# jackroos/VL-BERT

Measured on AMD Instinct MI355X. Metric: samples/sec VL-BERT-base pretrain (seq 64+36 regions) at 1/2/4/8 MI355X, higher is better.
Workload: dtype bf16; 1 GPU; VL-BERT-base 12-layer pretrain step (fwd+bwd+clip+AdamW), 64 text + 36 regions, precomputed 2048-d region features, dropout on; global_batch=256, per_gpu_batch=256, per_gpu_caption_samples=256, per_gpu_text_only_samples=0, module=ResNetVLBERTForPretraining, seq_len=101, parallelism=dp1, hipgraph=False, arch=gfx950:sramecc+:xnack-, cus=256, forced_exchange=False, ranks=1

## Files before the change

include/vlbert_hip.h:

```cpp
#ifndef VLBERT_HIP_H
#define VLBERT_HIP_H

#include <stdint.h>

#ifdef __cplusplus
extern "C" {
#endif

typedef struct ihipStream_t* vlb_stream_t;

const char* vlb_last_error(void);
int vlb_version(void);
int vlb_act_dtype(void);
int vlb_device_info(int device, char* name, int cap);

int vlb_gemm_nt_bf16(const void* A, long lda, const void* B, long ldb, void* C, long ldc, int M, int N, int K,
                     const float* bias, int act, const void* aux, long ldaux, void* pre, long ldpre,
                     const void* res, long ldres, float drop_p, const uint32_t* seed, uint32_t tag,
                     int out_mode, int splitk, vlb_stream_t stream);
int vlb_gemm_nt_bf16_ex(const void* A, long lda, const void* B, long ldb, void* C, long ldc, int M, int N, int K,
                        const float* bias, int act, const void* aux, long ldaux, void* pre, long ldpre,
                        const void* res, long ldres, const float* res_stats, const float* res_gamma, const float* res_beta,
                        int out_f16, float drop_p, const uint32_t* seed, uint32_t tag, int out_mode, int splitk,
                        vlb_stream_t stream);


int vlb_gemm_nt_bf16_splitk(const void* A, long lda, const void* B, long ldb, void* C, long ldc, int M, int N, int K,
                            float* workspace, long workspace_floats, vlb_stream_t stream);
int vlb_gemm_set_option(const char* name, int value);



long vlb_wgrad_workspace_floats(int M, int N, int K);
int vlb_wgrad_nt_bf16(const void* A, long lda, const void* B, long ldb, float* C, long ldc, int M, int N, int K,
                      float* workspace, long workspace_floats, vlb_stream_t stream);

int vlb_wgrad_tn_bf16(const void* A, long lda, const void* B, long ldb, float* C, long ldc, int R, int Mo, int No,
                      float* colsum, float* workspace, long workspace_floats, int accumulate, vlb_stream_t stream);

int vlb_transpose_bf16(const void* in, long ldi, void* out, long ldo, int R, int C, float* colsum, vlb_stream_t stream);
int vlb_transpose_batched_bf16(const int64_t* desc, const int32_t* tile_start, int n, int total_tiles, vlb_stream_t stream);

int vlb_nonfinite_status(int reset);
int vlb_layernorm_fwd(const void* x, long ldx, const float* gamma, const float* beta, void* y, long ldy, float* stats,
                      int rows, int H, float eps, int x_f16, vlb_stream_t stream);
int vlb_layernorm_bwd(const void* dy, long lddy, int dy_f32, const void* x, long ldx, const float* stats,
                      const float* gamma, void* dx, long lddx, void* dx_drop, long lddd, float drop_p,
                      const uint32_t* seed, uint32_t tag, float* dx_acc, long ldacc, float* dgamma, float* dbeta,
                      float* workspace, int rows, int H, int x_f16, vlb_stream_t stream);
long vlb_layernorm_bwd_workspace_floats(int H);
int vlb_layernorm_bwd_deferred(const void* dy, long lddy, int dy_f32, const void* x, long ldx, const float* stats,
                               const float* gamma, void* dx, long lddx, void* dx_drop, long lddd, float drop_p,
                               const uint32_t* seed, uint32_t tag, float* dx_acc, long ldacc, float* dgamma, float* dbeta,
                               float* workspace, int rows, int H, int x_f16, vlb_stream_t stream);
int vlb_layernorm_bwd_slabs(int rows);
int vlb_ln_param_finalize_batch(int n, const float* const* ws, const int* nslab, float* const* dgamma, float* const* dbeta, int H,
                                vlb_stream_t stream);

int vlb_attention_fwd(const void* qkv, const float* mask, void* ctx, float* lse, int B, int S, int H, int nh,
                      float drop_p, const uint32_t* seed, uint32_t tag, vlb_stream_t stream);
int vlb_attention_bwd(const void* qkv, const float* mask, const void* ctx, const float* lse, const void* dctx,
                      void* dqkv, int B, int S, int H, int nh, float drop_p, const uint32_t* seed, uint32_t tag,
                      vlb_stream_t stream);
int vlb_attention_probs(const void* qkv, const float* mask, const float* lse, float* probs, int B, int S, int H, int nh, int n,
                        int ldp, float drop_p, const uint32_t* seed, uint32_t tag, vlb_stream_t stream);

int vlb_seq_layout(const uint8_t* text_mask, const uint8_t* obj_mask, int B, int T, int R, int S, int32_t* code,
                   int32_t* text_len, int32_t* nobj, int32_t* text_rows, int32_t* obj_rows, float* attn_mask,
                   vlb_stream_t stream);
int vlb_obj_prep_fwd(const float* boxes, long ldbox, const float* im_info, long ldinfo, const int64_t* mvrc_ops,
                     const float* mask_emb, void* out, int B, int R, float drop_p, const uint32_t* seed, uint32_t tag,
                     vlb_stream_t stream);
int vlb_zero_padded_rows_bf16(void* x, long ld, const float* boxes, long ldbox, int rows, int H, vlb_stream_t stream);
int vlb_masked_colsum(const void* src, long lds, const int64_t* sel, int rows, int C, float* dst, float drop_p,
                      const uint32_t* seed, uint32_t tag, uint32_t row_elems, uint32_t col_off, vlb_stream_t stream);
int vlb_embed_fwd(const int32_t* code, const int32_t* text_len, const int64_t* text_ids, const int64_t* text_type,
                  const void* word_emb, const void* pos_emb, const void* type_emb, const void* end_emb,
                  const void* text_vis, long tv_sb, long tv_st, const void* obj_vis, long ov_sb, long ov_sr,
                  const void* obj_ling, long ol_sb, long ol_sr, const int64_t* obj_ling_idx, const float* gamma,
                  const float* beta, void* pre, float* stats, void* out, int B, int T, int R, int S, int H, int V,
                  int P, float eps, float drop_p, const uint32_t* seed, uint32_t tag, vlb_stream_t stream);
int vlb_embed_bwd(const void* dy, const void* pre, const float* stats, const float* gamma, const int32_t* code,
                  const int32_t* text_len, const int64_t* text_ids, const int64_t* text_type,
                  const int64_t* obj_ling_idx, float* d_word, float* d_pos, float* d_type, float* d_end,
                  float* d_gamma, float* d_beta, float* d_text_vis, long dtv_sb, long dtv_st, float* d_obj_vis,
                  long dov_sb, long dov_sr, float* d_obj_ling, long dol_sb, long dol_sr, int B, int T, int R, int S,
                  int H, int V, int P, float drop_p, const uint32_t* seed, uint32_t tag, int text_vis_zeroed,
                  vlb_stream_t stream);
int vlb_gather_rows(const void* src, const int32_t* idx, void* out, int n, int H, vlb_stream_t stream);
int vlb_scatter_rows(const void* src, const int32_t* idx, void* out, int n, int H, vlb_stream_t stream);
int vlb_mlm_compact(const int64_t* labels, const int32_t* src_rows, int n, int n_split, int V, int cap, int32_t* sel_pos,
                    int32_t* sel_src, int64_t* labels_c, float* count0, float* count1, int32_t* overflow, vlb_stream_t stream);
int vlb_ce_fwd_bwd_compact(void* logits, long ld, int rows, int V, const int64_t* labels_c, const float* count0, const float* count1,
                           float gscale, float* loss_out0, float* loss_out1, vlb_stream_t stream);
int vlb_head_grad_combine(const void* d_text, const void* d_obj, const int32_t* code, void* dx, int B, int T, int R,
                          int S, int H, vlb_stream_t stream);
int vlb_relu_bwd_cast(const float* g, const void* y, void* out, long n, vlb_stream_t stream);
int vlb_dgelu_mul(const void* dg, const void* u, void* out, long n, vlb_stream_t stream);
int vlb_mul_bf16(const void* a, const void* b, void* out, long n, vlb_stream_t stream);
int vlb_tanh_bwd(const void* dy, const void* y, void* out, long n, vlb_stream_t stream);

int vlb_ce_fwd_bwd(void* logits, long ld, int rows, int V, const int64_t* labels, float* counts, float gscale,
                   float* loss_out, void* logits_copy, long ldcopy, vlb_stream_t stream);
int vlb_soft_ce_fwd_bwd(void* logits, long ld, int rows, int C, const float* target, long ldt, float* tsum,
                        float* counts, float gscale, float* loss_out, void* logits_copy, long ldcopy,
                        vlb_stream_t stream);

int vlb_ce_eval(const void* logits, long ld, int rows, int V, const int64_t* labels, const float* count0, const float* count1,
                float* loss_out0, float* loss_out1, int64_t* acc0, int64_t* acc1, int32_t* pred, vlb_stream_t stream);
int vlb_soft_ce_eval(const void* logits, long ld, int rows, int C, const float* target, long ldt, float* loss_out, int64_t* acc,
                     vlb_stream_t stream);

int vlb_argmax_eval(const float* logits, long ld, int rows, int C, int mode, const void* label, long ldl, int32_t* pred, float* score,
                    float* probs, long ldp, void* sum, int64_t* count, vlb_stream_t stream);
int vlb_binary_cls_eval(const float* logits, long ld, const float* label, long ldl, int rows, int N, int64_t* acc, vlb_stream_t stream);
int vlb_joint_hits(const int32_t* pred_a, const int64_t* label_a, const int32_t* pred_r, const int64_t* label_r, int rows, int64_t* acc,
                   vlb_stream_t stream);

int vlb_bce_logits_fwd_bwd(void* logits, long ld, int rows, int A, const float* label, long ldl, float gscale, float pos_weight,
                           float* loss_out, void* logits_copy, long ldcopy, vlb_stream_t stream);
int vlb_dropout_bf16(const void* x, void* y, long n, float drop_p, const uint32_t* seed, uint32_t tag, vlb_stream_t stream);

int vlb_ground_score_fwd(const void* g, long ldg, int H, const float* w2, const float* b2, float* logits, long ldo, int B, int max_len,
                         int origin_len, float drop_p, const uint32_t* seed, uint32_t tag, vlb_stream_t stream);
int vlb_ground_bce(const float* logits, long ldo, const float* boxes, long sbb, long sbr, const float* label, long ldl, int B, int max_len,
                   float* loss_out, float* dlogit, vlb_stream_t stream);
int vlb_ground_score_bwd(const float* gscale, const float* dlogit, int rows, const void* g, long ldg, const void* dgelu, long ldd, int H,
                         const float* w2, void* du, long lddu, float* dw2, float* db2, float drop_p, const uint32_t* seed, uint32_t tag,
                         vlb_stream_t stream);
int vlb_ground_pick_box(const float* logits, long ldo, int B, int origin_len, const float* boxes, long sbb, long sbr, const float* im_info,
                        long ldi, float* pred_boxes, int64_t* idx, vlb_stream_t stream);

int vlb_scale_f32(float* x, long n, float alpha, vlb_stream_t stream);
int vlb_zero_ranges_f32(float* base, const int64_t* ranges, const int32_t* block_start, int n, int total_blocks, vlb_stream_t stream);
int vlb_copy_ranges_f32(const float* src, float* dst, const int64_t* ranges, const int32_t* block_start, int n, int total_blocks,
                        vlb_stream_t stream);

int vlb_sumsq_f32(const float* g, long n, float* out, vlb_stream_t stream);
int vlb_sumsq_f32_det(const float* g, long n, float* partials, int partials_len, float* out, vlb_stream_t stream);
int vlb_adamw_step(float* p, const float* g, float* m, float* v, void* p_bf16, long n, float* state, float grad_scale,
                   vlb_stream_t stream);
int vlb_sumsq_bf16_det(const void* g_bf16, long n, float* partials, int partials_len, float* out, vlb_stream_t stream);
int vlb_adamw_step_gbf16(float* p, const void* g_bf16, float* m, float* v, void* p_bf16, long n, float* state, float grad_scale,
                         vlb_stream_t stream);
int vlb_sumsq_ranges_det(const void* g, int g_is_bf16, const int64_t* ranges, const int32_t* block_start, int n, int total_blocks, int chunk,
                         float* partials, int partials_len, float* out, vlb_stream_t stream);
int vlb_adamw_step_ranges(float* p, const void* g, int g_is_bf16, float* m, float* v, void* p_bf16_compact, const int64_t* ranges,
                          const int32_t* block_start, int n, int total_blocks, int chunk, float* state, float grad_scale, vlb_stream_t stream);
int vlb_sgd_momentum_step(float* p, const float* g, float* momentum_buf, void* p_bf16, long n, float lr, float momentum,
                          float weight_decay, const float* sumsq, float max_norm, float grad_scale, vlb_stream_t stream);
int vlb_lr_schedule_step(float* state, int kind, float base_lr, float warmup_steps, float t_total, vlb_stream_t stream);

#define VLB_SCALER_FLOATS 9
#define VLB_SCALER_SCALE 0
#define VLB_SCALER_GROWTH_FACTOR 1
#define VLB_SCALER_BACKOFF_FACTOR 2
#define VLB_SCALER_GROWTH_INTERVAL 3
#define VLB_SCALER_UNSKIPPED 4
#define VLB_SCALER_SKIPPED_TOTAL 5
#define VLB_SCALER_SKIPPED_IN_A_ROW 6
#define VLB_SCALER_MIN_SCALE 7
#define VLB_SCALER_MAX_SCALE 8
int vlb_adamw_step_scaled(float* p, const void* g, int g_is_bf16, float* m, float* v, void* p_bf16, long n, float* state, float* scaler,
                          int update_scaler, float grad_scale, vlb_stream_t stream);
int vlb_adamw_step_ranges_scaled(float* p, const void* g, int g_is_bf16, float* m, float* v, void* p_bf16_compact, const int64_t* ranges,
                                 const int32_t* block_start, int n, int total_blocks, int chunk, float* state, float* scaler,
                                 float grad_scale, vlb_stream_t stream);
int vlb_sgd_momentum_step_scaled(float* p, const float* g, float* momentum_buf, void* p_bf16, long n, float lr, float momentum,
                                 float weight_decay, const float* sumsq, float max_norm, float grad_scale, float* scaler, int update_scaler,
                                 vlb_stream_t stream);
int vlb_lr_schedule_step_scaled(float* state, const float* scaler, int kind, float base_lr, float warmup_steps, float t_total,
                                vlb_stream_t stream);
int vlb_ce_fwd_bwd_ds(void* logits, long ld, int rows, int V, const int64_t* labels, float* counts, float gscale, const float* dscale,
                      float* loss_out, void* logits_copy, long ldcopy, vlb_stream_t stream);
int vlb_ce_fwd_bwd_compact_ds(void* logits, long ld, int rows, int V, const int64_t* labels_c, const float* count0, const float* count1,
// ... 98 lines not shown
```

vl-bert_amd/_lib.py:

```python
import ctypes
import os

_HERE = os.path.dirname(os.path.abspath(__file__))
PRECISION = os.environ.get("VLB_PRECISION", "bf16").lower()
if PRECISION in ("fp16", "half", "float16"):
    PRECISION = "f16"
if PRECISION not in ("bf16", "f16"):
    raise ValueError("VLB_PRECISION must be bf16 or f16 (got %r)" % PRECISION)


def _default_path(precision):
    return os.path.join(_HERE, "libvlbert_hip.so" if precision == "bf16" else "libvlbert_hip_f16.so")


LIB_PATH = os.environ.get("VLB_LIB_PATH") or _default_path(PRECISION)

_P, _L, _I, _F, _U = ctypes.c_void_p, ctypes.c_long, ctypes.c_int, ctypes.c_float, ctypes.c_uint32

_SIGS = {
    "vlb_gemm_nt_bf16": "plplpliiipiplplplfpuiis",
    "vlb_transpose_batched_bf16": "ppiis",
    "vlb_gemm_nt_bf16_splitk": "plplpliiipls",
    "vlb_transpose_bf16": "plpliips",
    "vlb_wgrad_nt_bf16": "plplpliiipls",
    "vlb_wgrad_tn_bf16": "plplpliiipplis",
    "vlb_wgrad_tn_group_bf16": "ippppppipppplis",
    "vlb_wgrad_tn_table_launch": "piis",
    "vlb_tn8_set_stamps": "p",
    "vlb_wgrad_tn_table_pack": "i" + "p" * 11 + "ipl",
    "vlb_zero_ranges_f32": "pppiis",
    "vlb_copy_ranges_f32": "ppppiis",
    "vlb_layernorm_fwd": "plppplpiifis",
    "vlb_layernorm_bwd": "pliplppplplfpuplpppiiis",
    "vlb_layernorm_bwd_deferred": "pliplppplplfpuplpppiiis",
    "vlb_ln_param_finalize_batch": "ippppis",
    "vlb_gemm_nt_bf16_ex": "plplpliiipiplplplpppifpuiis",
    "vlb_attention_fwd": "ppppiiiifpus",
    "vlb_attention_bwd": "ppppppiiiifpus",
    "vlb_attention_probs": "ppppiiiiiifpus",
    "vlb_seq_layout": "ppiiiipppppps",
    "vlb_obj_prep_fwd": "plplpppiifpus",
    "vlb_masked_colsum": "plpiipfpuuus",
    "vlb_embed_fwd": "pppp" "pppp" "pll" "pll" "pll" "p" "pp" "ppp" "iiiiiii" "f" "fpu" "s",
    "vlb_embed_bwd": "pppp" "ppppp" "pppppp" "pll" "pll" "pll" "iiiiiii" "fpu" "i" "s",
    "vlb_gather_rows": "pppiis",
    "vlb_scatter_rows": "pppiis",
    "vlb_mlm_compact": "ppiiiipppppps",
    "vlb_ce_fwd_bwd_compact": "pliipppfpps",
    "vlb_head_grad_combine": "ppppiiiiis",
    "vlb_relu_bwd_cast": "pppls",
    "vlb_dgelu_mul": "pppls",
    "vlb_mul_bf16": "pppls",
    "vlb_tanh_bwd": "pppls",
    "vlb_ce_fwd_bwd": "pliippfppls",
    "vlb_soft_ce_fwd_bwd": "pliiplppfppls",
    "vlb_ce_eval": "plii" + "p" * 8 + "s",
    "vlb_soft_ce_eval": "pliiplpps",
    "vlb_argmax_eval": "pliiiplppplpps",
    "vlb_binary_cls_eval": "plpliips",
    "vlb_joint_hits": "ppppips",
    "vlb_sumsq_f32": "plps",
    "vlb_zero_padded_rows_bf16": "plpliis",
    "vlb_bce_logits_fwd_bwd": "pliiplffppls",
    "vlb_dropout_bf16": "pplfpus",
    "vlb_sumsq_f32_det": "plpips",
    "vlb_adamw_step": "ppppplpfs",
    "vlb_adamw_step_gbf16": "ppppplpfs",
    "vlb_sgd_momentum_step": "pppplfffpffs",
    "vlb_sumsq_bf16_det": "plpips",
    "vlb_sumsq_ranges_det": "pippiiipips",
    "vlb_adamw_step_ranges": "ppipppppiiipfs",
    "vlb_lr_schedule_step": "pifffs",
    "vlb_adamw_step_scaled": "ppippplppifs",
    "vlb_adamw_step_ranges_scaled": "ppipppppiiippfs",
    "vlb_sgd_momentum_step_scaled": "pppplfffpffpis",
    "vlb_lr_schedule_step_scaled": "ppifffs",
    "vlb_ce_fwd_bwd_ds": "pliippfpppls",
    "vlb_ce_fwd_bwd_compact_ds": "pliipppfppps",
    "vlb_soft_ce_fwd_bwd_ds": "pliiplppfpppls",
    "vlb_bce_logits_fwd_bwd_ds": "pliiplfpfppls",
    "vlb_conv_weight_prepare": "pppppfppppiiiis",
    "vlb_conv_weight_prepare_batched": "ppiifs",
    "vlb_conv_wgrad_finalize": "pppiiiis",
    "vlb_conv3x3_nhwc_bf16": "piiiiiplplipiplps",
    "vlb_conv3x3_wgrad_tn_bf16": "plpiiiiiplipplis",
    "vlb_wgrad_tn_rowscale_bf16": "plplpliiipplis",
    "vlb_im2col_nhwc_bf16": "ppliiiiiiiiis",
    "vlb_im2col_image_f32": "ppiiiiiiiiis",
    "vlb_mask_image_boxes_f32": "piiiiplips",
    "vlb_maxpool3x3s2_nhwc": "ppiiiis",
    "vlb_subsample2_nhwc": "ppiiiis",
    "vlb_upsample2_zero_nhwc": "ppiiiis",
    "vlb_roi_align_nhwc_fwd": "pplipiiiiiifis",
    "vlb_roi_align_nhwc_bwd": "pplipiiiiiiifis",
    "vlb_roi_align_nhwc_bwd_gather": "pplippppliiiiiifis",
    "vlb_relu_mask_cast": "pppls",
    "vlb_avgpool_rows_fwd": "ppliiiiips",
    "vlb_avgpool_rows_bwd": "plpplpiiifpuuups",
    "vlb_gemm_nt_f32": "plplpliiiiillllllplfiplplplfpuiis",
    "vlb_gemm_tn_f32": "plplpliiiiillllllfiips",
    "vlb_transpose_f32": "plpliiiiillllps",
    "vlb_layernorm_f32_fwd": "plppplpiifs",
    "vlb_layernorm_f32_bwd": "plplppplplfpuppiis",
# ... 117 lines not shown
```

vl-bert_amd/csrc/gemm.hip:

```cpp
#include <math.h>
#include <stdlib.h>

#include <type_traits>

#include "vlb_common.h"

#include "gemm_params.h"


struct EpiStage {
  char* lds;
  int m0, n0;
  int row_l, col_l;
  int tid, nthreads, bn;
};

__device__ __forceinline__ void epi_stage_put(const EpiStage& st, int i, int j, const float (&v)[4]) {
  const int row = st.row_l + i * 16, colb = (st.col_l + j * 16) * 2;
  const int pitch = st.bn * 2, mask = (st.bn >> 3) - 1;
  *(uint2*)(st.lds + row * pitch + ((((colb >> 4) ^ (row & mask)) << 4) | (colb & 15))) =
      make_uint2(pack2bf(v[0], v[1]), pack2bf(v[2], v[3]));
}

__device__ __forceinline__ void epi_copy_out(const EpiStage& st, bf16_t* C, long ldc) {
// ... 145 lines not shown
            for (int r = 0; r < 4 && n + r < p.N; ++r) v[r] += fmaf((h2f(q[r]) - ms.x) * ms.y, p.res_gamma[n + r], p.res_beta[n + r]);
          }
        } else if (full) {
          const uint2 w = *(const uint2*)q;
          v[0] += bflo(w.x); v[1] += bfhi(w.x); v[2] += bflo(w.y); v[3] += bfhi(w.y);
        } else {
          for (int r = 0; r < 4 && n + r < p.N; ++r) v[r] += bf2f(q[r]);
        }
      }
      if (ACT == 7) {
#pragma unroll
        for (int r = 0; r < 4; ++r) v[r] = fmaxf(v[r], 0.f);
      } else if (ACT == 8) {
        const bf16_t* q = aux_row + j * 16;
        if (full) {
          const uint2 w = *(const uint2*)q;
          v[0] = bflo(w.x) > 0.f ? v[0] : 0.f; v[1] = bfhi(w.x) > 0.f ? v[1] : 0.f;
          v[2] = bflo(w.y) > 0.f ? v[2] : 0.f; v[3] = bfhi(w.y) > 0.f ? v[3] : 0.f;
        } else {
          for (int r = 0; r < 4 && n + r < p.N; ++r) v[r] = bf2f(q[r]) > 0.f ? v[r] : 0.f;
        }
      }
      if (OUT == 0) {
        if (STAGED) {
          epi_stage_put(st, i, j, v);
        } else {
          bf16_t* c = (bf16_t*)p.C + offc + j * 16;
          if (full) *(uint2*)c = make_uint2(pack2o(v[0], v[1], f16out), pack2o(v[2], v[3], f16out));
          else for (int r = 0; r < 4 && n + r < p.N; ++r) c[r] = f16out ? f2h(v[r]) : f2bf(v[r]);
        }
      } else if (OUT == 1) {
        float* c = (float*)p.C + offc + j * 16;
        if (full) *(float4*)c = make_float4(v[0], v[1], v[2], v[3]);
        else for (int r = 0; r < 4 && n + r < p.N; ++r) c[r] = v[r];
      } else if (OUT == 2) {
        float* c = (float*)p.C + offc + j * 16;
        for (int r = 0; r < 4 && (INTERIOR || n + r < p.N); ++r) atomicAdd(c + r, v[r]);
      } else {
        float* c = (float*)p.C + offc + j * 16;
        if (full) {
          const float4 o = *(const float4*)c;
          *(float4*)c = make_float4(o.x + v[0], o.y + v[1], o.z + v[2], o.w + v[3]);
        } else {
          for (int r = 0; r < 4 && n + r < p.N; ++r) c[r] += v[r];
        }
      }
    }
  }
  if (STAGED) epi_copy_out(st, (bf16_t*)p.C, p.ldc);
}

template <bool INTERIOR, int FM, int FN>
__device__ __forceinline__ void gemm_epilogue_dispatch(const GemmParams& p, f32x4 (&acc)[FM][FN], int mb, int nb, const EpiStage& st) {
  if (p.out_f32 == 3) gemm_epilogue<0, false, false, 3, INTERIOR, FM, FN, true>(p, acc, mb, nb, st);
  else if (p.out_f32 == 2) gemm_epilogue<0, false, false, 2, INTERIOR, FM, FN, true>(p, acc, mb, nb, st);
  else if (p.out_f32 == 1) gemm_epilogue<0, false, false, 1, INTERIOR, FM, FN, true>(p, acc, mb, nb, st);
  else if (p.act == 1) gemm_epilogue<1, false, false, 0, INTERIOR, FM, FN, true>(p, acc, mb, nb, st);
  else if (p.act == 2) gemm_epilogue<2, false, false, 0, INTERIOR, FM, FN, true>(p, acc, mb, nb, st);
  else if (p.act == 3) gemm_epilogue<3, false, false, 0, INTERIOR, FM, FN, true>(p, acc, mb, nb, st);
  else if (p.act == 4) gemm_epilogue<4, false, false, 0, INTERIOR, FM, FN, true>(p, acc, mb, nb, st);
  else if (p.act == 5) gemm_epilogue<5, false, false, 0, INTERIOR, FM, FN, true>(p, acc, mb, nb, st);
  else if (p.act == 6) gemm_epilogue<6, false, false, 0, INTERIOR, FM, FN, true>(p, acc, mb, nb, st);
  else if (p.act == 7) gemm_epilogue<7, false, true, 0, INTERIOR, FM, FN, true>(p, acc, mb, nb, st);
  else if (p.act == 8) {
    if (p.res) gemm_epilogue<8, false, true, 0, INTERIOR, FM, FN, true>(p, acc, mb, nb, st);
    else gemm_epilogue<8, false, false, 0, INTERIOR, FM, FN, true>(p, acc, mb, nb, st);
  } else if (p.res) {
    if (p.drop_thr) gemm_epilogue<0, true, true, 0, INTERIOR, FM, FN, true>(p, acc, mb, nb, st);
    else gemm_epilogue<0, false, true, 0, INTERIOR, FM, FN, true>(p, acc, mb, nb, st);
  } else if (p.drop_thr) gemm_epilogue<0, true, false, 0, INTERIOR, FM, FN, true>(p, acc, mb, nb, st);
  else gemm_epilogue<0, false, false, 0, INTERIOR, FM, FN, true>(p, acc, mb, nb, st);
}

template <int EPI, bool INTERIOR, int FM, int FN>
__device__ __forceinline__ void gemm_epilogue_select(const GemmParams& p, f32x4 (&acc)[FM][FN], int mb, int nb, const EpiStage& st) {
  if constexpr (EPI < 0) {
    gemm_epilogue_dispatch<INTERIOR, FM, FN>(p, acc, mb, nb, st);
  } else {
    constexpr int ACT = EPI == 1 ? 4 : EPI == 2 ? 5 : EPI == 5 ? 2 : EPI == 6 ? 7 : (EPI == 7 || EPI == 8) ? 8 : 0;
    gemm_epilogue<ACT, EPI == 3, EPI == 3 || EPI == 4 || EPI == 6 || EPI == 7, 0, INTERIOR, FM, FN>(p, acc, mb, nb, st);
  }
}

template <int BM, int BN, int WGM, int WGN, int EPI, bool CONV = false>
__global__ __launch_bounds__(64 * WGM * WGN, (WGM * WGN >= 8) ? 4 : 2) void gemm_nt_bf16_kernel(const GemmParams p) {
  constexpr int BK = 64;
  constexpr int NT = 64 * WGM * WGN;
  constexpr int WM = BM / WGM, WN = BN / WGN;
  constexpr int FM = WM / 16, FN = WN / 16;
  constexpr int NA = BM * 8 / NT, NB = BN * 8 / NT;
  constexpr int A_BYTES = BM * BK * 2, B_BYTES = BN * BK * 2, STAGE = A_BYTES + B_BYTES;
  extern __shared__ __attribute__((aligned(16))) char smem[];

  const int tid = threadIdx.x;
  const int lane = tid & 63;
  const int wave = __builtin_amdgcn_readfirstlane(tid >> 6);
  const int wm = wave / WGN, wn = wave % WGN;
  const int nt = p.ntm * p.ntn;
  const int k_begin = blockIdx.y * p.k_per_split;
  const int k_end = min(p.K, k_begin + p.k_per_split);
  const int ntk = (k_end - k_begin) / BK;
  if ((int)blockIdx.x >= nt || ntk <= 0) return;
  auto tile_of = [&](int w, int& m0, int& n0) {
    int tile_m, tile_n;
    vlb_tile_of(vlb_xcd_order(w, nt), p.ntm, p.ntn, p.tile_group, tile_m, tile_n);
    m0 = tile_m * BM;
    n0 = tile_n * BN;
  };
  auto setup = [&](const bf16_t* (&a_src)[NA], uint32_t (&a_msk)[NA], const bf16_t* (&b_src)[NB], int m0, int n0) {
#pragma unroll
    for (int it = 0; it < NA; ++it) {
      const int P = it * NT + tid, r = P >> 3, kc = (P & 7) ^ ((r >> 1) & 7);
      const int m = min(m0 + r, p.M - 1);
      a_src[it] = p.A + (long)m * p.lda + k_begin + kc * 8;
      if constexpr (CONV) {
        const int ox = m % p.conv_W, oy = (m / p.conv_W) % p.conv_H;
        uint32_t msk = 0;
#pragma unroll
        for (int t = 0; t < 9; ++t) {
          const int iy = oy + (t / 3 - 1) * p.conv_dil, ix = ox + (t % 3 - 1) * p.conv_dil;
          msk |= (uint32_t)(iy >= 0 && iy < p.conv_H && ix >= 0 && ix < p.conv_W) << t;
        }
        a_msk[it] = msk;
      }
    }
#pragma unroll
    for (int it = 0; it < NB; ++it) {
      const int P = it * NT + tid, r = P >> 3, kc = (P & 7) ^ ((r >> 1) & 7);
      b_src[it] = p.B + (long)min(n0 + r, p.N - 1) * p.ldb + k_begin + kc * 8;
    }
  };
  const int conv_cpt = CONV ? p.conv_C / BK : 1;
  auto stage = [&](const bf16_t* (&a_src)[NA], uint32_t (&a_msk)[NA], const bf16_t* (&b_src)[NB], int buf, int kt) {
    char* sa = smem + buf * STAGE;
    char* sb = sa + A_BYTES;
    const int koff = kt * BK;
    if constexpr (CONV) {
      const int t = kt / conv_cpt, cb = kt - t * conv_cpt;
      const long aoff = ((long)(t / 3 - 1) * p.conv_W + (t % 3 - 1)) * p.conv_dil * p.conv_C + cb * BK;
#pragma unroll
      for (int it = 0; it < NA; ++it) {
        const bf16_t* src = ((a_msk[it] >> t) & 1u) ? a_src[it] + aoff : p.zero;
        __builtin_amdgcn_global_load_lds(GLDS_PTR(src), LDS_PTR(sa + (it * NT + wave * 64) * 16), 16, 0, 0);
      }
    } else {
#pragma unroll
      for (int it = 0; it < NA; ++it)
        __builtin_amdgcn_global_load_lds(GLDS_PTR(a_src[it] + koff), LDS_PTR(sa + (it * NT + wave * 64) * 16), 16, 0, 0);
    }
#pragma unroll
    for (int it = 0; it < NB; ++it)
      __builtin_amdgcn_global_load_lds(GLDS_PTR(b_src[it] + koff), LDS_PTR(sb + (it * NT + wave * 64) * 16), 16, 0, 0);
  };

  f32x4 acc[FM][FN];
#pragma unroll
  for (int i = 0; i < FM; ++i)
#pragma unroll
    for (int j = 0; j < FN; ++j) acc[i][j] = (f32x4){0.f, 0.f, 0.f, 0.f};

  const int frow = lane & 15;
  const int c0 = (((lane >> 4) ^ (frow >> 1)) << 4);
  const int a_off = (wm * WM + frow) * 128 + c0;
  const int b_off = (wn * WN + frow) * 128 + c0;

  const bf16_t* a_src[NA];
  const bf16_t* b_src[NB];
  uint32_t a_msk[NA];
  int w = blockIdx.x, m0, n0, buf = 0;
  if (!CONV && p.stagger > 0 && ((blockIdx.x >> 3) & 63) >= 32) {
    for (int i = 0; i < p.stagger; ++i) __builtin_amdgcn_s_sleep(127);
  }
  tile_of(w, m0, n0);
  setup(a_src, a_msk, b_src, m0, n0);
  stage(a_src, a_msk, b_src, 0, 0);
  __syncthreads();
  for (;;) {
    const int w_next = w + gridDim.x;
    const bool has_next = w_next < nt;
    int m0n = 0, n0n = 0;
    const bf16_t* a_nx[NA];
    const bf16_t* b_nx[NB];
    uint32_t m_nx[NA];
    for (int kt = 0; kt < ntk; ++kt) {
      if (kt + 1 < ntk) {
        stage(a_src, a_msk, b_src, buf ^ 1, kt + 1);
      } else if (has_next) {
        tile_of(w_next, m0n, n0n);
// ... 604 lines not shown
                                               float* __restrict__ colsum, int vec, int r0, int c0) {
  __shared__ __attribute__((aligned(16))) bf16_t tile[64 * 64];
  __shared__ float csum[4][64];
  const int tid = threadIdx.x, sub = tid & 7, grp = tid >> 3;
  float cs[8];
#pragma unroll
  for (int k = 0; k < 8; ++k) cs[k] = 0.f;
#pragma unroll
  for (int it = 0; it < 2; ++it) {
    const int rl = grp + 32 * it, r = r0 + rl, c = c0 + sub * 8;
    uint4 v = make_uint4(0, 0, 0, 0);
    if (r < R) {
      if (vec && c + 8 <= C) {
        v = *(const uint4*)(in + (long)r * ldi + c);
      } else {
        bf16_t e[8];
#pragma unroll
        for (int k = 0; k < 8; ++k) e[k] = (c + k < C) ? in[(long)r * ldi + c + k] : (bf16_t)0;
        v = make_uint4(e[0] | (uint32_t)e[1] << 16, e[2] | (uint32_t)e[3] << 16, e[4] | (uint32_t)e[5] << 16, e[6] | (uint32_t)e[7] << 16);
      }
    }
    *(uint4*)(tile + rl * 64 + ((sub ^ (rl >> 3)) << 3)) = v;
    if (colsum) {
      cs[0] += bflo(v.x); cs[1] += bfhi(v.x); cs[2] += bflo(v.y); cs[3] += bfhi(v.y);
      cs[4] += bflo(v.z); cs[5] += bfhi(v.z); cs[6] += bflo(v.w); cs[7] += bfhi(v.w);
    }
  }
  if (colsum) {
#pragma unroll
    for (int k = 0; k < 8; ++k) {
      cs[k] += __shfl_xor(cs[k], 8, 64);
      cs[k] += __shfl_xor(cs[k], 16, 64);
      cs[k] += __shfl_xor(cs[k], 32, 64);
    }
    if ((tid & 63) < 8) {
#pragma unroll
      for (int k = 0; k < 8; ++k) csum[tid >> 6][sub * 8 + k] = cs[k];
    }
  }
  __syncthreads();
#pragma unroll
  for (int it = 0; it < 2; ++it) {
    const int cl = grp + 32 * it, c = c0 + cl, rb = sub * 8;
    bf16_t e[8];
#pragma unroll
    for (int k = 0; k < 8; ++k) e[k] = tile[(rb + k) * 64 + (((cl >> 3) ^ sub) << 3) + (cl & 7)];
    if (c < C) {
      const int r = r0 + rb;
      bf16_t* o = out + (long)c * ldo + r;
      if (vec && r + 8 <= R) {
        *(uint4*)o = make_uint4(e[0] | (uint32_t)e[1] << 16, e[2] | (uint32_t)e[3] << 16, e[4] | (uint32_t)e[5] << 16,
                                e[6] | (uint32_t)e[7] << 16);
      } else {
#pragma unroll
        for (int k = 0; k < 8; ++k)
          if (r + k < R) o[k] = e[k];
      }
    }
  }
  if (colsum && tid < 64 && c0 + tid < C) atomicAdd(colsum + c0 + tid, csum[0][tid] + csum[1][tid] + csum[2][tid] + csum[3][tid]);
}

__global__ __launch_bounds__(256) void transpose_bf16_kernel(const bf16_t* __restrict__ in, long ldi, bf16_t* __restrict__ out,
                                                             long ldo, int R, int C, float* __restrict__ colsum, int vec) {
  transpose_tile(in, ldi, out, ldo, R, C, colsum, vec, blockIdx.y * 64, blockIdx.x * 64);
}

__global__ __launch_bounds__(256) void transpose_batched_kernel(const long* __restrict__ desc, const int* __restrict__ tile_start, int n) {
  int lo = 0, hi = n;
  while (hi - lo > 1) {
    const int mid = (lo + hi) >> 1;
    if ((int)blockIdx.x >= tile_start[mid]) lo = mid; else hi = mid;
  }
  const long* d = desc + 6 * lo;
  const bf16_t* in = (const bf16_t*)d[0];
  bf16_t* out = (bf16_t*)d[2];
  const long ldi = d[1], ldo = d[3];
  const int R = (int)d[4], C = (int)d[5];
  const int t = blockIdx.x - tile_start[lo], tx = (C + 63) >> 6;
  const int vec = ((ldi % 8) == 0 && (ldo % 8) == 0 && ((uintptr_t)in % 16) == 0 && ((uintptr_t)out % 16) == 0) ? 1 : 0;
  transpose_tile(in, ldi, out, ldo, R, C, nullptr, vec, (t / tx) * 64, (t % tx) * 64);
}

template <int BM, int BN, int WGM, int WGN, int EPI>
static int launch_gemm_cfg(GemmParams& p, int splits, hipStream_t stream) {
  int cap = vlb_opt(VLB_OPT_RESIDENT) / splits;
  if (cap < 8) cap = 8;
  return launch_persistent<gemm_nt_bf16_kernel<BM, BN, WGM, WGN, EPI>>(2 * (BM + BN) * 64 * 2, 64 * WGM * WGN, BM, BN, cap & ~7,
                                                                       vlb_opt(VLB_OPT_TILE_GROUP), p, splits, stream, "vlb_gemm_nt_bf16");
}

static int epi_class(const GemmParams& p) {
  if (!vlb_opt(VLB_OPT_EPI_SPECIALISE) || p.out_f32 != 0 || p.res_stats || p.c_f16) return -1;
  if (p.act == 0) return p.res ? (p.drop_thr ? 3 : 4) : (p.drop_thr ? -1 : 0);
  if (p.act == 4) return 1;
  if (p.act == 5) return 2;
  if (p.act == 2) return 5;
  if (p.act == 7) return 6;
  if (p.act == 8) return p.res ? 7 : 8;
  return -1;
}

template <int BM, int BN, int WGM, int WGN>
static int launch_gemm_epi(GemmParams& p, int splits, hipStream_t stream) {
  return dispatch_epi(epi_class(p), std::integer_sequence<int, -1, 0, 1, 2, 3, 4, 5, 6, 7, 8>{}, VLB_ERR_ARG, [&](auto epi) {
    return launch_gemm_cfg<BM, BN, WGM, WGN, decltype(epi)::value>(p, splits, stream);
  });
}

template <int BM, int BN, int WGM, int WGN, int NS>
static int launch_ring_epi(GemmParams& p, hipStream_t stream) {
  constexpr int smem = NS * (BM + BN) * 128;
  return dispatch_epi(epi_class(p), std::integer_sequence<int, -1, 0, 1, 2, 3, 4, 5>{}, 1, [&](auto epi) {
    return launch_persistent<gemm_nt_ring_kernel<BM, BN, WGM, WGN, decltype(epi)::value, NS>>(
        smem, 64 * WGM * WGN, BM, BN, 256 * (163840 / smem), vlb_opt(VLB_OPT_TILE_GROUP), p, 1, stream, "vlb_gemm_nt_bf16(ring)");
  });
}

static int gemm_ring_try(GemmParams& p, int splits, hipStream_t stream) {
  const int ring = vlb_opt(VLB_OPT_NT_RING);
  if (!ring || splits != 1 || p.c_split_stride != 0 || p.k_per_split < p.K) return 1;
  if (ring == 1 && !(p.N <= 1024 && p.M <= 8192 && p.M >= 1024 && p.K >= 512)) return 1;
  const bool narrow = ring == 3 || ring == 1;
  if (narrow) return launch_ring_epi<128, 64, 2, 2, 3>(p, stream);
  return launch_ring_epi<128, 128, 2, 4, 4>(p, stream);
}


template <int BM, int BN>
static int launch_gemm(GemmParams& p, int splits, hipStream_t stream) {
  if (BN == 128) return launch_gemm_epi<BM, 128, 2, 4>(p, splits, stream);
  return launch_gemm_epi<BM, BN, 2, 2>(p, splits, stream);
}

static int gemm_nt_impl(const void* A, long lda, const void* B, long ldb, void* C, long ldc, int M, int N, int K,
                        const float* bias, int act, const void* aux, long ldaux, void* pre, long ldpre,
                        const void* res, long ldres, const float* res_stats, const float* res_gamma, const float* res_beta, int out_f16,
                        float drop_p, const uint32_t* seed, uint32_t tag, int out_mode, int splitk, hipStream_t stream) {
  if (M <= 0 || N <= 0) return VLB_OK;
  VLB_CHECK_ARG(!res_stats || (res && res_gamma && res_beta && act == 0 && out_mode == 0),
                "vlb_gemm_nt_bf16_ex: the LayerNorm residual needs res (fp16 pre-LN rows), gamma, beta, act 0 and a 16-bit output");
  VLB_CHECK_ARG(!out_f16 || out_mode == 0, "vlb_gemm_nt_bf16_ex: out_f16 applies to the 16-bit output mode");
  VLB_CHECK_ARG(K > 0 && (K % 64) == 0, "vlb_gemm_nt_bf16: K=%d must be a positive multiple of 64", K);
  VLB_CHECK_ARG(A && B && C, "vlb_gemm_nt_bf16: null operand");
  VLB_CHECK_ARG((lda % 8) == 0 && (ldb % 8) == 0, "vlb_gemm_nt_bf16: lda/ldb must be multiples of 8 elements");
  VLB_CHECK_ARG((ldc % 4) == 0, "vlb_gemm_nt_bf16: ldc must be a multiple of 4");
  VLB_CHECK_ARG(out_mode >= 0 && out_mode <= 3, "vlb_gemm_nt_bf16: bad out_mode %d", out_mode);
  VLB_CHECK_ARG(act >= 0 && act <= 8, "vlb_gemm_nt_bf16: bad act %d", act);
  VLB_CHECK_ARG((act != 3 && act != 5 && act != 8) || aux, "vlb_gemm_nt_bf16: act=3/5/8 needs aux");
  VLB_CHECK_ARG(act != 7 || res, "vlb_gemm_nt_bf16: act=7 (relu after residual) needs res");
  VLB_CHECK_ARG(act == 0 || act >= 7 || (!(drop_p > 0.f) && !res), "vlb_gemm_nt_bf16: an activation cannot be combined with dropout/residual");
  VLB_CHECK_ARG(act < 7 || !(drop_p > 0.f), "vlb_gemm_nt_bf16: act=7/8 cannot be combined with dropout");
  VLB_CHECK_ARG(out_mode == 0 || (act == 0 && !(drop_p > 0.f) && !res), "vlb_gemm_nt_bf16: fp32 outputs take bias only");
  VLB_CHECK_ARG(!(drop_p > 0.f) || seed, "vlb_gemm_nt_bf16: dropout needs a device seed pointer");
  VLB_CHECK_ARG((long)M * (long)N < (1L << 32) || !(drop_p > 0.f), "vlb_gemm_nt_bf16: dropout index overflow");
  GemmParams p = {};
  p.A = (const bf16_t*)A; p.lda = lda; p.B = (const bf16_t*)B; p.ldb = ldb;
  p.M = M; p.N = N; p.K = K;
  p.bias = bias; p.act = act; p.aux = (const bf16_t*)aux; p.ldaux = ldaux; p.pre = (bf16_t*)pre; p.ldpre = ldpre;
  p.res = (const bf16_t*)res; p.ldres = ldres;
  p.res_stats = res_stats; p.res_gamma = res_gamma; p.res_beta = res_beta; p.c_f16 = out_f16 ? 1 : 0;
  p.drop_thr = vlb_drop_thr(drop_p); p.drop_scale = vlb_drop_scale(p.drop_thr); p.seed = seed; p.tag = tag;
  p.C = C; p.ldc = ldc; p.out_f32 = out_mode; p.c_split_stride = 0;
  p.stagger = vlb_opt(VLB_OPT_NT_STAGGER);
  int splits = 1;
  const int ktiles = K / 64;
  if (out_mode == 2) {
    splits = splitk > 0 ? splitk : 1;
    if (splitk <= 0) {
      const long tiles = (long)vlb_cdiv(M, 128) * vlb_cdiv(N, 128);
      const long slots = 512;
      double best = -1.0;
      for (int sp = 1; sp <= 32 && sp <= ktiles; ++sp) {
        const long blocks = tiles * sp;
        const long rounds = (blocks + slots - 1) / slots;
        const double eff = (double)blocks / (double)(rounds * slots);
        if (eff > best + 0.04) { best = eff; splits = sp; }
      }
    }
    if (splits > ktiles) splits = ktiles;
    if (splits < 1) splits = 1;
  }
  const int per = vlb_cdiv(ktiles, splits);
  splits = vlb_cdiv(ktiles, per);
  p.k_per_split = per * 64;
  if (splits == 1 && out_mode == 0) {
    const int took = vlb_gemm_p8_try(p, stream);
    if (took != 0) return took < 0 ? took : VLB_OK;
  }
  const int use256 = vlb_opt(VLB_OPT_NT_256);
  const long tiles256 = (long)vlb_cdiv(M, 256) * vlb_cdiv(N, 256);
  const bool big_b = (long)N * K * 2 >= (24L << 20) && tiles256 >= 512;
  if (use256 && out_mode == 0 && splits == 1 && act == 0 && !res && !p.drop_thr &&
      (use256 == 1 ? big_b : tiles256 >= use256)) {
    return launch_persistent<gemm_nt_256_kernel>(3 * (256 + 256) * 64, 512, 256, 256, 256, vlb_opt(VLB_OPT_NT_256_GROUP), p, 1, stream,
                                                 "vlb_gemm_nt_bf16(256)");
  }
  const long tiles128 = (long)vlb_cdiv(M, 128) * vlb_cdiv(N, 128) * splits;
  const bool narrow = tiles128 < 384 || N <= 64;
  {
    const int took = gemm_ring_try(p, splits, stream);
    if (took <= 0) return took;
  }
  if (narrow) return launch_gemm<128, 64>(p, splits, stream);
  return launch_gemm<128, 128>(p, splits, stream);
}

extern "C" int vlb_gemm_nt_bf16(const void* A, long lda, const void* B, long ldb, void* C, long ldc, int M, int N, int K,
                                const float* bias, int act, const void* aux, long ldaux, void* pre, long ldpre,
                                const void* res, long ldres, float drop_p, const uint32_t* seed, uint32_t tag,
                                int out_mode, int splitk, hipStream_t stream) {
  return gemm_nt_impl(A, lda, B, ldb, C, ldc, M, N, K, bias, act, aux, ldaux, pre, ldpre, res, ldres, nullptr, nullptr, nullptr, 0,
                      drop_p, seed, tag, out_mode, splitk, stream);
}

extern "C" int vlb_gemm_nt_bf16_ex(const void* A, long lda, const void* B, long ldb, void* C, long ldc, int M, int N, int K,
                                   const float* bias, int act, const void* aux, long ldaux, void* pre, long ldpre,
                                   const void* res, long ldres, const float* res_stats, const float* res_gamma, const float* res_beta,
                                   int out_f16, float drop_p, const uint32_t* seed, uint32_t tag, int out_mode, int splitk,
                                   hipStream_t stream) {
  return gemm_nt_impl(A, lda, B, ldb, C, ldc, M, N, K, bias, act, aux, ldaux, pre, ldpre, res, ldres, res_stats, res_gamma, res_beta,
                      out_f16, drop_p, seed, tag, out_mode, splitk, stream);
}

template <int BN, int WGN>
static int launch_conv(GemmParams& p, hipStream_t stream) {
  return dispatch_epi(p.act == 0 ? 0 : p.act == 2 ? 5 : 8, std::integer_sequence<int, 0, 5, 8>{}, VLB_ERR_ARG, [&](auto epi) {
    return launch_persistent<gemm_nt_bf16_kernel<128, BN, 2, WGN, decltype(epi)::value, true>>(
        2 * (128 + BN) * 64 * 2, 64 * 2 * WGN, 128, BN, 512, vlb_opt(VLB_OPT_TILE_GROUP), p, 1, stream, "vlb_conv3x3_nhwc_bf16");
  });
}

extern "C" int vlb_conv3x3_nhwc_bf16(const void* x, int N, int H, int W, int C, int dil, const void* w, long ldw, void* y, long ldy,
                                     int O, const float* bias, int act, const void* aux, long ldaux, const void* zero16,
                                     hipStream_t stream) {
  if (N <= 0 || O <= 0) return VLB_OK;
  VLB_CHECK_ARG(x && w && y && zero16, "vlb_conv3x3_nhwc_bf16: null argument");
  VLB_CHECK_ARG(C > 0 && (C % 64) == 0, "vlb_conv3x3_nhwc_bf16: C=%d must be a multiple of 64", C);
  VLB_CHECK_ARG(H > 0 && W > 0 && dil >= 1, "vlb_conv3x3_nhwc_bf16: bad geometry");
  VLB_CHECK_ARG((ldw % 8) == 0 && ldw >= 9L * C && (ldy % 4) == 0, "vlb_conv3x3_nhwc_bf16: bad leading dimensions");
  VLB_CHECK_ARG(act == 0 || act == 2 || (act == 8 && aux), "vlb_conv3x3_nhwc_bf16: act must be 0, 2 or 8 (with aux)");
  VLB_CHECK_ARG((long)N * H * W < (1L << 31), "vlb_conv3x3_nhwc_bf16: too many rows");
  GemmParams p = {};
  p.A = (const bf16_t*)x; p.lda = C; p.B = (const bf16_t*)w; p.ldb = ldw;
  p.M = N * H * W; p.N = O; p.K = 9 * C; p.k_per_split = 9 * C;
  p.bias = bias; p.act = act; p.aux = (const bf16_t*)aux; p.ldaux = ldaux; p.pre = nullptr; p.ldpre = 0; p.res = nullptr; p.ldres = 0;
  p.drop_thr = 0; p.drop_scale = 1.f; p.seed = nullptr; p.tag = 0;
  p.C = y; p.ldc = ldy; p.out_f32 = 0; p.c_split_stride = 0;
  p.conv_C = C; p.conv_H = H; p.conv_W = W; p.conv_dil = dil; p.zero = (const bf16_t*)zero16;
  const long tiles128 = (long)vlb_cdiv(p.M, 128) * vlb_cdiv(O, 128);
  const bool narrow = tiles128 < 384 || O <= 64;
  return narrow ? launch_conv<64, 2>(p, stream) : launch_conv<128, 4>(p, stream);
}

__global__ __launch_bounds__(256) void splitk_reduce_kernel(const float* __restrict__ slabs, long slab_stride, int splits,
                                                            float* __restrict__ C, long ldc, int M, int N, int ldw,
                                                            bf16_t* __restrict__ Cb, long ldcb, int accumulate,
                                                            const float* __restrict__ rowscale = nullptr) {
  const int n4 = ldw >> 2;
  const long total = (long)M * n4;
  for (long i = (long)blockIdx.x * 256 + threadIdx.x; i < total; i += (long)gridDim.x * 256) {
    const int m = (int)(i / n4), n = (int)(i % n4) * 4;
    const float* src = slabs + (long)m * ldw + n;
    float4 a = *(const float4*)src;
    for (int sp = 1; sp < splits; ++sp) {
      const float4 b = *(const float4*)(src + sp * slab_stride);
      a.x += b.x; a.y += b.y; a.z += b.z; a.w += b.w;
    }
    if (rowscale) {
      const float sc = rowscale[m];
      a.x *= sc; a.y *= sc; a.z *= sc; a.w *= sc;
    }
    if (Cb) {
      bf16_t* c = Cb + (long)m * ldcb + n;
      if (n + 3 < N) {
        *(uint2*)c = make_uint2(pack2bf(a.x, a.y), pack2bf(a.z, a.w));
      } else {
        const float av[4] = {a.x, a.y, a.z, a.w};
        for (int r = 0; r < 4 && n + r < N; ++r) c[r] = f2bf(av[r]);
      }
      continue;
    }
    float* c = C + (long)m * ldc + n;
    if (n + 3 < N) {
      if (accumulate) {
        const float4 o = *(const float4*)c;
        a.x += o.x; a.y += o.y; a.z += o.z; a.w += o.w;
      }
      *(float4*)c = a;
    } else {
      const float av[4] = {a.x, a.y, a.z, a.w};
      for (int r = 0; r < 4 && n + r < N; ++r) c[r] = accumulate ? c[r] + av[r] : av[r];
    }
  }
}

static int launch_splitk_reduce(const float* workspace, long slab_stride, int splits, float* C, long ldc, int Mo, int No, long ldw,
                                int accumulate, const float* rowscale, hipStream_t stream, const char* name, bf16_t* Cb = nullptr) {
  long blocks = ((long)Mo * (ldw / 4) + 255) / 256;
  if (blocks > 2048) blocks = 2048;
  hipLaunchKernelGGL(splitk_reduce_kernel, dim3((int)blocks), dim3(256), 0, stream, workspace, slab_stride, splits, C, ldc, Mo, No, (int)ldw,
                     Cb, ldc, accumulate, rowscale);
  VLB_CHECK_LAUNCH(name);
  return VLB_OK;
}

static int wgrad_pick_splits(int M, int N, int K, long workspace_floats) {
  const int ktiles = K / 64;
  const long tiles = (long)vlb_cdiv(M, 128) * vlb_cdiv(N, 128);
  const long ldw = (N + 3) / 4 * 4;
  const double t_k = 1.15, t_fix = 4.0, bw = 4.0e6;
  int best = 1;
  double best_t = 1e30;
  for (int sp = 1; sp <= 32 && sp <= ktiles; ++sp) {
    if (sp > 1 && (long)sp * M * ldw > workspace_floats) break;
    const long rounds = (tiles * sp + 511) / 512;
    const double t = rounds * (vlb_cdiv(ktiles, sp) * t_k + t_fix) + (sp > 1 ? 2.0 * sp * M * ldw * 4.0 / bw : 0.0);
    if (t < best_t * 0.97) { best_t = t; best = sp; }
  }
  return best;
}

extern "C" long vlb_wgrad_workspace_floats(int M, int N, int K) {
  if (M <= 0 || N <= 0 || K <= 0) return 0;
  int sp = wgrad_pick_splits(M, N, K, 1L << 40);
  if (K >= 256 && (K % 128) == 0) {
    const int sp8 = vlb_tn8_pick_splits(M, N, K);
    if (sp8 > sp) sp = sp8;
  }
  return sp > 1 ? (long)sp * M * ((N + 3) / 4 * 4) : 0;
}

extern "C" int vlb_wgrad_nt_bf16(const void* A, long lda, const void* B, long ldb, float* C, long ldc, int M, int N, int K,
                                 float* workspace, long workspace_floats, hipStream_t stream) {
  if (M <= 0 || N <= 0) return VLB_OK;
  VLB_CHECK_ARG(K > 0 && (K % 64) == 0, "vlb_wgrad_nt_bf16: K=%d must be a positive multiple of 64", K);
  VLB_CHECK_ARG(A && B && C, "vlb_wgrad_nt_bf16: null operand");
  VLB_CHECK_ARG((lda % 8) == 0 && (ldb % 8) == 0 && (ldc % 4) == 0, "vlb_wgrad_nt_bf16: bad leading dimensions");
  const int splits = wgrad_pick_splits(M, N, K, workspace ? workspace_floats : 0);
  const int ktiles = K / 64;
  const int per = vlb_cdiv(ktiles, splits);
  const int nsp = vlb_cdiv(ktiles, per);
  const long ldw = (N + 3) / 4 * 4;
  GemmParams p = {};
  p.A = (const bf16_t*)A; p.lda = lda; p.B = (const bf16_t*)B; p.ldb = ldb;
  p.M = M; p.N = N; p.K = K; p.k_per_split = per * 64;
  p.bias = nullptr; p.act = 0; p.aux = nullptr; p.ldaux = 0; p.pre = nullptr; p.ldpre = 0; p.res = nullptr; p.ldres = 0;
  p.drop_thr = 0; p.drop_scale = 1.f; p.seed = nullptr; p.tag = 0;
  if (nsp == 1) {
    p.C = C; p.ldc = ldc; p.out_f32 = 3; p.c_split_stride = 0;
  } else {
    p.C = workspace; p.ldc = ldw; p.out_f32 = 1; p.c_split_stride = (long)M * ldw;
  }
  int rc = launch_gemm<128, 128>(p, nsp, stream);
  if (rc) return rc;
  if (nsp > 1) return launch_splitk_reduce(workspace, (long)M * ldw, nsp, C, ldc, M, N, ldw, 1, nullptr, stream, "vlb_wgrad_nt_bf16(reduce)");
  return VLB_OK;
}

extern "C" int vlb_gemm_nt_bf16_splitk(const void* A, long lda, const void* B, long ldb, void* C, long ldc, int M, int N, int K,
                                       float* workspace, long workspace_floats, hipStream_t stream) {
  if (M <= 0 || N <= 0) return VLB_OK;
  VLB_CHECK_ARG(K > 0 && (K % 64) == 0, "vlb_gemm_nt_bf16_splitk: K=%d must be a positive multiple of 64", K);
  VLB_CHECK_ARG(A && B && C, "vlb_gemm_nt_bf16_splitk: null operand");
  VLB_CHECK_ARG((lda % 8) == 0 && (ldb % 8) == 0 && (ldc % 4) == 0, "vlb_gemm_nt_bf16_splitk: bad leading dimensions");
  const int splits = wgrad_pick_splits(M, N, K, workspace ? workspace_floats : 0);
  const int ktiles = K / 64;
  const int per = vlb_cdiv(ktiles, splits);
  const int nsp = vlb_cdiv(ktiles, per);
  if (nsp <= 1)
    return vlb_gemm_nt_bf16(A, lda, B, ldb, C, ldc, M, N, K, nullptr, 0, nullptr, 0, nullptr, 0, nullptr, 0, 0.f, nullptr, 0, 0, 0, stream);
  const long ldw = (N + 3) / 4 * 4;
  GemmParams p = {};
  p.A = (const bf16_t*)A; p.lda = lda; p.B = (const bf16_t*)B; p.ldb = ldb;
  p.M = M; p.N = N; p.K = K; p.k_per_split = per * 64;
  p.bias = nullptr; p.act = 0; p.aux = nullptr; p.ldaux = 0; p.pre = nullptr; p.ldpre = 0; p.res = nullptr; p.ldres = 0;
  p.drop_thr = 0; p.drop_scale = 1.f; p.seed = nullptr; p.tag = 0;
  p.C = workspace; p.ldc = ldw; p.out_f32 = 1; p.c_split_stride = (long)M * ldw;
  int rc = launch_gemm<128, 128>(p, nsp, stream);
  if (rc) return rc;
  return launch_splitk_reduce(workspace, (long)M * ldw, nsp, nullptr, ldc, M, N, ldw, 0, nullptr, stream, "vlb_gemm_nt_bf16_splitk(reduce)",
                              (bf16_t*)C);
}

struct SplitkReduceGroup {
  const float* slabs[4];
  long slab_stride[4];
  float* C[4];
  long ldc[4];
  int splits[4], M[4], N[4], ldw[4];
};

__global__ __launch_bounds__(256) void splitk_reduce_group_kernel(const SplitkReduceGroup g, int accumulate) {
  const int e = blockIdx.y;
  const float* slabs = g.slabs[e];
  const long slab_stride = g.slab_stride[e], ldc = g.ldc[e];
  float* C = g.C[e];
  const int splits = g.splits[e], M = g.M[e], N = g.N[e], ldw = g.ldw[e];
  const int n4 = ldw >> 2;
  const long total = (long)M * n4;
  for (long i = (long)blockIdx.x * 256 + threadIdx.x; i < total; i += (long)gridDim.x * 256) {
    const int m = (int)(i / n4), n = (int)(i % n4) * 4;
    const float* src = slabs + (long)m * ldw + n;
    float4 a = *(const float4*)src;
    for (int sp = 1; sp < splits; ++sp) {
      const float4 b = *(const float4*)(src + sp * slab_stride);
      a.x += b.x; a.y += b.y; a.z += b.z; a.w += b.w;
    }
    float* c = C + (long)m * ldc + n;
    if (n + 3 < N) {
      if (accumulate) {
        const float4 o = *(const float4*)c;
        a.x += o.x; a.y += o.y; a.z += o.z; a.w += o.w;
      }
      vlb_store_nt((float4*)c, a);
    } else {
      const float av[4] = {a.x, a.y, a.z, a.w};
      for (int r = 0; r < 4 && n + r < N; ++r) c[r] = accumulate ? c[r] + av[r] : av[r];
    }
  }
}

template <auto KERNEL>
static void tn128_launch_kernel(dim3 grid, int block, const GemmParams& p, float* colsum, hipStream_t stream) {
  constexpr int smem = 2 * 2 * 64 * 128 * 2;
  static bool attr_set = false;
  if (!attr_set) {
    (void)hipFuncSetAttribute((const void*)KERNEL, hipFuncAttributeMaxDynamicSharedMemorySize, smem);
    attr_set = true;
  }
  hipLaunchKernelGGL(KERNEL, grid, dim3(block), smem, stream, p, colsum);
}

template <bool CONV>
static int tn128_launch(GemmParams& p, float* C, long ldc, int R, int Mo, int No, float* colsum, const float* rowscale, float* workspace,
                        long workspace_floats, int accumulate, hipStream_t stream, const char* name) {
  const int Rp = vlb_cdiv(R, 64) * 64;
  const int splits = wgrad_pick_splits(Mo, No, Rp, workspace ? workspace_floats : 0);
  const int ktiles = Rp / 64;
  const int per = vlb_cdiv(ktiles, splits);
  const int nsp = vlb_cdiv(ktiles, per);
  const long ldw = (No + 3) / 4 * 4;
  const bool slab = nsp > 1 || rowscale != nullptr;
  VLB_CHECK_ARG(!rowscale || (workspace && workspace_floats >= (long)nsp * Mo * ldw), "%s: rowscale needs a workspace of %ld floats", name,
                (long)nsp * Mo * ldw);
  p.M = Mo; p.N = No; p.K = R; p.k_per_split = per * 64;
  p.drop_scale = 1.f;
  if (!slab) {
    p.C = C; p.ldc = ldc; p.out_f32 = accumulate ? 3 : 1; p.c_split_stride = 0;
  } else {
    p.C = workspace; p.ldc = ldw; p.out_f32 = 1; p.c_split_stride = (long)Mo * ldw;
  }
  p.ntm = vlb_cdiv(Mo, 128); p.ntn = vlb_cdiv(No, 128);
  const dim3 grid(p.ntm * p.ntn, nsp);
  if (p.out_f32 == 3) tn128_launch_kernel<gemm_tn_bf16_kernel<4, 3, CONV>>(grid, 512, p, colsum, stream);
  else tn128_launch_kernel<gemm_tn_bf16_kernel<4, 1, CONV>>(grid, 512, p, colsum, stream);
  VLB_CHECK_LAUNCH(name);
  if (slab) return launch_splitk_reduce(workspace, (long)Mo * ldw, nsp, C, ldc, Mo, No, ldw, accumulate, rowscale, stream, name);
  return VLB_OK;
}

static int wgrad_tn_impl(const void* A, long lda, const void* B, long ldb, float* C, long ldc, int R, int Mo, int No, float* colsum,
                         const float* rowscale, float* workspace, long workspace_floats, int accumulate, hipStream_t stream) {
  if (Mo <= 0 || No <= 0 || R <= 0) return VLB_OK;
  VLB_CHECK_ARG(A && B && C, "vlb_wgrad_tn_bf16: null operand");
  VLB_CHECK_ARG((lda % 8) == 0 && (ldb % 8) == 0 && (ldc % 4) == 0 && lda >= 8 && ldb >= 8, "vlb_wgrad_tn_bf16: bad leading dimensions");
  VLB_CHECK_ARG(((uintptr_t)A % 16) == 0 && ((uintptr_t)B % 16) == 0, "vlb_wgrad_tn_bf16: operands must be 16-byte aligned");
  {
    GemmParams q = {};
    q.A = (const bf16_t*)A; q.lda = lda; q.B = (const bf16_t*)B; q.ldb = ldb;
    q.M = Mo; q.N = No; q.K = R;
    const int used = vlb_gemm_tn8_try(q, C, ldc, colsum, workspace, workspace_floats, accumulate, rowscale != nullptr, stream);
    if (used < 0) return used;
    if (used > 0) {
      const long ldw8 = (No + 3) / 4 * 4;
      if (used > 1 || rowscale)
        return launch_splitk_reduce(workspace, (long)Mo * ldw8, used, C, ldc, Mo, No, ldw8, accumulate, rowscale, stream,
                                    "vlb_wgrad_tn_bf16(tn8 reduce)");
      return VLB_OK;
    }
  }
  GemmParams p = {};
  p.A = (const bf16_t*)A; p.lda = lda; p.B = (const bf16_t*)B; p.ldb = ldb;
  const int ntm = vlb_cdiv(Mo, 128), ntn = vlb_cdiv(No, 128), tn_group = vlb_opt(VLB_OPT_TN_GROUP);
  p.tile_group = tn_group > 0 ? (tn_group < ntm ? tn_group : ntm) : vlb_square_tile_group(ntm, ntn);
  return tn128_launch<false>(p, C, ldc, R, Mo, No, colsum, rowscale, workspace, workspace_floats, accumulate, stream, "vlb_wgrad_tn_bf16");
}

extern "C" int vlb_wgrad_tn_bf16(const void* A, long lda, const void* B, long ldb, float* C, long ldc, int R, int Mo, int No,
                                 float* colsum, float* workspace, long workspace_floats, int accumulate, hipStream_t stream) {
  return wgrad_tn_impl(A, lda, B, ldb, C, ldc, R, Mo, No, colsum, nullptr, workspace, workspace_floats, accumulate, stream);
}

extern "C" int vlb_wgrad_tn_group_bf16(int n, const void* const* A, const long* lda, const void* const* B, const long* ldb,
                                       float* const* C, const long* ldc, int R, const int* Mo, const int* No, float* const* colsum,
                                       float* workspace, long workspace_floats, int accumulate, hipStream_t stream) {
  VLB_CHECK_ARG(n >= 1 && n <= 4 && A && lda && B && ldb && C && ldc && Mo && No, "vlb_wgrad_tn_group_bf16: bad arguments (1 <= n <= 4)");
  for (int i = 0; i < n; ++i) VLB_CHECK_ARG(A[i] && B[i] && C[i], "vlb_wgrad_tn_group_bf16: null operand %d", i);
  int slices[4];
  long ws_off[4];
  const int took = vlb_gemm_tn8_group(n, A, lda, B, ldb, C, ldc, R, Mo, No, colsum, workspace, workspace_floats, accumulate, slices, ws_off,
                                      stream);
  if (took < 0) return took;
  if (took == 0) {
    for (int i = 0; i < n; ++i) {
      const int rc = wgrad_tn_impl(A[i], lda[i], B[i], ldb[i], C[i], ldc[i], R, Mo[i], No[i], colsum ? colsum[i] : nullptr, nullptr,
                                   workspace, workspace_floats, accumulate, stream);
      if (rc) return rc;
    }
    return VLB_OK;
  }
  SplitkReduceGroup rg;
  int nr = 0;
  long max_blocks = 1;
  for (int i = 0; i < n; ++i) {
    if (slices[i] <= 1) continue;
    const long ldw = (No[i] + 3) / 4 * 4;
    long blocks = ((long)Mo[i] * (ldw / 4) + 255) / 256;
    if (blocks > 2048) blocks = 2048;
    if (blocks > max_blocks) max_blocks = blocks;
    rg.slabs[nr] = workspace + ws_off[i]; rg.slab_stride[nr] = (long)Mo[i] * ldw; rg.splits[nr] = slices[i];
    rg.C[nr] = C[i]; rg.ldc[nr] = ldc[i]; rg.M[nr] = Mo[i]; rg.N[nr] = No[i]; rg.ldw[nr] = (int)ldw;
    ++nr;
  }
  if (nr) {
    hipLaunchKernelGGL(splitk_reduce_group_kernel, dim3((int)max_blocks, nr), dim3(256), 0, stream, rg, accumulate);
    VLB_CHECK_LAUNCH("vlb_wgrad_tn_group_bf16(reduce)");
  }
  return VLB_OK;
}

extern "C" int vlb_wgrad_tn_rowscale_bf16(const void* A, long lda, const void* B, long ldb, float* C, long ldc, int R, int Mo, int No,
                                          const float* rowscale, float* workspace, long workspace_floats, int accumulate,
                                          hipStream_t stream) {
  VLB_CHECK_ARG(rowscale, "vlb_wgrad_tn_rowscale_bf16: null rowscale");
  return wgrad_tn_impl(A, lda, B, ldb, C, ldc, R, Mo, No, nullptr, rowscale, workspace, workspace_floats, accumulate, stream);
}

extern "C" int vlb_conv3x3_wgrad_tn_bf16(const void* dy, long lddy, const void* x, int N, int H, int W, int C, int dil, float* dW,
                                         long lddw, int O, const float* rowscale, float* workspace, long workspace_floats, int accumulate,
                                         hipStream_t stream) {
  if (N <= 0 || O <= 0) return VLB_OK;
  VLB_CHECK_ARG(dy && x && dW, "vlb_conv3x3_wgrad_tn_bf16: null operand");
  VLB_CHECK_ARG(C > 0 && (C % 128) == 0, "vlb_conv3x3_wgrad_tn_bf16: C=%d must be a multiple of 128", C);
  VLB_CHECK_ARG((lddy % 8) == 0 && lddy >= O && (lddw % 4) == 0 && lddw >= 9L * C, "vlb_conv3x3_wgrad_tn_bf16: bad leading dimensions");
  VLB_CHECK_ARG(H > 0 && W > 0 && dil >= 1 && (long)N * H * W < (1L << 24), "vlb_conv3x3_wgrad_tn_bf16: bad geometry (rows must be < 2^24)");
  const int R = N * H * W, No = 9 * C;
  GemmParams p = {};
  p.A = (const bf16_t*)dy; p.lda = lddy; p.B = (const bf16_t*)x; p.ldb = C;
  p.conv_C = C; p.conv_H = H; p.conv_W = W; p.conv_dil = dil; p.zero = nullptr;
  p.tile_group = vlb_square_tile_group(vlb_cdiv(O, 128), No / 128);
  return tn128_launch<true>(p, dW, lddw, R, O, No, nullptr, rowscale, workspace, workspace_floats, accumulate, stream,
                            "vlb_conv3x3_wgrad_tn_bf16");
}

extern "C" int vlb_transpose_bf16(const void* in, long ldi, void* out, long ldo, int R, int C, float* colsum,
                                  hipStream_t stream) {
  if (R <= 0 || C <= 0) return VLB_OK;
  VLB_CHECK_ARG(in && out && ldo >= R && ldi >= C, "vlb_transpose_bf16: bad arguments");
  dim3 grid(vlb_cdiv(C, 64), vlb_cdiv(R, 64));
  const int vec = ((ldi % 8) == 0 && (ldo % 8) == 0 && ((uintptr_t)in % 16) == 0 && ((uintptr_t)out % 16) == 0) ? 1 : 0;
  hipLaunchKernelGGL(transpose_bf16_kernel, grid, dim3(256), 0, stream, (const bf16_t*)in, ldi, (bf16_t*)out, ldo, R, C,
                     colsum, vec);
  VLB_CHECK_LAUNCH("vlb_transpose_bf16");
  return VLB_OK;
}

extern "C" int vlb_transpose_batched_bf16(const int64_t* desc, const int32_t* tile_start, int n, int total_tiles, hipStream_t stream) {
  if (n <= 0 || total_tiles <= 0) return VLB_OK;
  VLB_CHECK_ARG(desc && tile_start, "vlb_transpose_batched_bf16: null descriptor table");
  hipLaunchKernelGGL(transpose_batched_kernel, dim3(total_tiles), dim3(256), 0, stream, (const long*)desc, (const int*)tile_start, n);
  VLB_CHECK_LAUNCH("vlb_transpose_batched_bf16");
  return VLB_OK;
}
// ... 1 lines not shown
```

vl-bert_amd/csrc/gemm_p8.hip:

```cpp
#include <math.h>
#include <stdlib.h>
#include <string.h>

#include <type_traits>

#include "gemm_params.h"

#ifndef VLB_P8_LN_SB
#define VLB_P8_LN_SB 2
#endif
#ifndef VLB_P8_SIDE_DEPTH
#define VLB_P8_SIDE_DEPTH 1
#endif
#ifndef VLB_P8_WDRAIN
#define VLB_P8_WDRAIN 1
#endif

namespace {

template <int OFF>
__device__ __forceinline__ void p8_lds_read(bf16x8& dst, uint32_t vaddr) {
  asm volatile("ds_read_b128 %0, %1 offset:%2" : "=v"(dst) : "v"(vaddr), "n"(OFF));
}

// ... 303 lines not shown
  auto consts = [&]() {
    if (p.bias && full8) {
      const float4 b0 = *(const float4*)(p.bias + n), b1 = *(const float4*)(p.bias + n + 4);
      b8[0] = b0.x; b8[1] = b0.y; b8[2] = b0.z; b8[3] = b0.w; b8[4] = b1.x; b8[5] = b1.y; b8[6] = b1.z; b8[7] = b1.w;
    }
    if constexpr (LNRES) {
#pragma unroll
      for (int e = 0; e < 8; ++e) g8[e] = be8[e] = 0.f;
      if (full8) {
        const float4 a0 = *(const float4*)(p.res_gamma + n), a1 = *(const float4*)(p.res_gamma + n + 4);
        const float4 c0 = *(const float4*)(p.res_beta + n), c1 = *(const float4*)(p.res_beta + n + 4);
        g8[0] = a0.x; g8[1] = a0.y; g8[2] = a0.z; g8[3] = a0.w; g8[4] = a1.x; g8[5] = a1.y; g8[6] = a1.z; g8[7] = a1.w;
        be8[0] = c0.x; be8[1] = c0.y; be8[2] = c0.z; be8[3] = c0.w; be8[4] = c1.x; be8[5] = c1.y; be8[6] = c1.z; be8[7] = c1.w;
      }
    }
  };
  auto load_side = [&](int u, uint4& sd, float2& ms) {
    if constexpr (SIDE) {
      if (!EDGE || (mw + uoff(u) < p.M && full8)) {
        const uint4* src = (const uint4*)(Sl + uoff(u) * lds_);
        if (EPI == 2 || EPI == 10) sd = vlb_load_nt(src);
        else sd = *src;
        if constexpr (LNRES) ms = *(const float2*)(Ml + 2 * uoff(u));
      }
    }
  };
  auto put = [&](auto u_c) {
    constexpr int u = decltype(u_c)::value, R = u >> 1, hf = u & 1;
    if (upper == (hf != 0)) {
      p8_lds_write_f4<0>(wr[0], acc[R][0]);
      p8_lds_write_f4<0>(wr[1], acc[R][1]);
      p8_lds_write_f4<0>(wr[2], acc[R][2]);
      p8_lds_write_f4<0>(wr[3], acc[R][3]);
    }
  };
  auto finish = [&](int u, const f32x4& x0, const f32x4& x1, const uint4& sd, const float2& ms) {
    const int m = mw + uoff(u);
    if (!EDGE || (m < p.M && n < p.N)) {
      float v[8] = {x0[0], x0[1], x0[2], x0[3], x1[0], x1[1], x1[2], x1[3]};
      if (full8) {
        if constexpr (LNRES) p8_epilogue8<EPI>(p, v, b8, m, n, seed, sd, ms, g8, be8);
        else p8_epilogue8<EPI>(p, v, b8, m, n, seed, sd);
        uint4 o4;
        if (f16out) {
          asm volatile("" ::: "memory");
          o4 = make_uint4(pack2h(v[0], v[1]), pack2h(v[2], v[3]), pack2h(v[4], v[5]), pack2h(v[6], v[7]));
        } else {
          o4 = make_uint4(pack2bf(v[0], v[1]), pack2bf(v[2], v[3]), pack2bf(v[4], v[5]), pack2bf(v[6], v[7]));
        }
        *(uint4*)(Cl + (p.ablate != 2 ? uoff(u) * (long)p.ldc : 0L)) = o4;
      } else {
        for (int e = 0; e < 8 && n + e < p.N; ++e) {
          const float o = p8_epilogue1<EPI>(p, v[e], m, n + e, seed);
          Cl[uoff(u) * (long)p.ldc + e] = f16out ? f2h(o) : f2bf(o);
        }
      }
    }
  };
  constexpr int DEPTH = (EPI == 2 || EPI == 10) ? VLB_P8_SIDE_DEPTH : 1, RING = DEPTH + 1;
  uint4 side[RING];
  float2 mst[RING];
#pragma unroll
  for (int d = 0; d < RING; ++d) {
    side[d] = make_uint4(0, 0, 0, 0);
    mst[d] = make_float2(0.f, 0.f);
  }
  consts();
  p8_static_for<0, (DEPTH < NU ? DEPTH : NU)>([&](auto d_c) {
    constexpr int d = decltype(d_c)::value;
    load_side(d, side[d % RING], mst[d % RING]);
  });
  put(std::integral_constant<int, 0>{});
  p8_static_for<0, NU>([&](auto u_c) {
    constexpr int u = decltype(u_c)::value;
    f32x4 x0, x1;
    p8_stage_read<0>(x0, x1, rd0, rd1);
    if constexpr (u + DEPTH < NU) load_side(u + DEPTH, side[(u + DEPTH) % RING], mst[(u + DEPTH) % RING]);
    if constexpr (u + 1 < NU) put(std::integral_constant<int, u + 1>{});
    finish(u, x0, x1, side[u % RING], mst[u % RING]);
  });
  asm volatile("" ::"v"(b8[0]), "v"(b8[4]));
}

template <int FMH, int EPI, bool KEEPB>
__global__ __launch_bounds__(512, 2) void gemm_nt_p8_kernel(const GemmParams p) {
  constexpr int AH = 32 * FMH;
  constexpr int BM = 2 * AH, BN = 256;
  constexpr int AHB = AH * 128, BHB = 128 * 128;
  constexpr int OFF_A0 = 0, OFF_A1 = AHB, OFF_B0 = 2 * AHB, OFF_B1 = 2 * AHB + BHB;
  constexpr int BUF = 2 * AHB + 2 * BHB;
  constexpr int STG = 2 * BUF;
  constexpr int SR = (163840 - STG) / 1024 >= 32 ? 32 : (163840 - STG) / 1024;
  constexpr int NLA = (AH * 8 + 511) / 512;
  constexpr int VM_AHEAD = (AH * 8) / 512 + 2;
  static_assert(SR == 32 || SR == 16, "staging slab");
  extern __shared__ __attribute__((aligned(16))) char smem[];

  const int tid = threadIdx.x, lane = tid & 63;
  const int wave = __builtin_amdgcn_readfirstlane(tid >> 6);
  const int wm = wave >> 2, wn = wave & 3;
  const int nt = p.ntm * p.ntn;
  const int nk = p.K >> 6;
  if ((int)blockIdx.x >= nt) return;
  unsigned long long* const stamps = (unsigned long long*)(EPI == 1 ? (void*)p.aux : (void*)p.pre);
  const bool stamp = (p.ablate == 4) && stamps;
  unsigned long long t_main = 0, t_epi = 0, t_mark = 0;
  if (stamp && tid == 0) {
    unsigned long long* t = stamps + 8 * blockIdx.x;
    t[0] = __builtin_readcyclecounter();
    t[1] = __builtin_amdgcn_s_memrealtime();
  }

  auto tile_of = [&](int w, int& m0, int& n0) {
    int tile_m, tile_n;
    vlb_tile_of(vlb_xcd_order(w, nt), p.ntm, p.ntn, p.tile_group, tile_m, tile_n);
    m0 = tile_m * BM;
    n0 = tile_n * BN;
  };

  const __amdgpu_buffer_rsrc_t rsA = __builtin_amdgcn_make_buffer_rsrc((void*)p.A, 0, 0x7FFFFFFF, 0x00020000);
  const __amdgpu_buffer_rsrc_t rsB = __builtin_amdgcn_make_buffer_rsrc((void*)p.B, 0, 0x7FFFFFFF, 0x00020000);
  const int ldaB = (int)p.lda * 2, ldbB = (int)p.ldb * 2;
  const int kcb = (((tid & 7) ^ ((tid >> 4) & 7)) << 4);
  const int rowA = (tid >> 3) * ldaB + kcb, maxA = (p.M - 1) * ldaB + kcb;
#if VLB_P8_WDRAIN
  const int rowB = ((tid >> 8) * 64 + ((tid >> 3) & 31)) * ldbB + kcb, maxB = (p.N - 1) * ldbB + kcb;
#else
  const int rowB = (tid >> 3) * ldbB + kcb, maxB = (p.N - 1) * ldbB + kcb;
#endif
  int w_p = blockIdx.x, kt_p = 0, pm0 = 0, pn0 = 0;
  auto setup = [&](int w) { tile_of(w, pm0, pn0); };
  auto stage = [&](auto which_c, auto buf_c) {
    constexpr int WHICH = decltype(which_c)::value, B_ = decltype(buf_c)::value;
    const int koff = kt_p * 128;
    if constexpr (WHICH < 2) {
      char* dst = smem + B_ * BUF + (WHICH == 0 ? OFF_A0 : OFF_A1);
#pragma unroll
      for (int it = 0; it < NLA; ++it) {
        if (it * 512 + 511 < AH * 8 || wave < (AH * 8 - it * 512) / 64) {
          const int vo = min((pm0 + WHICH * AH + it * 64) * ldaB + rowA, maxA);
          __builtin_amdgcn_raw_ptr_buffer_load_lds(rsA, LDS_PTR(dst + (it * 512 + wave * 64) * 16), 16, vo, koff, 0, 0);
        }
      }
    } else {
      char* dst = smem + B_ * BUF + (WHICH == 2 ? OFF_B0 : OFF_B1);
#pragma unroll
      for (int it = 0; it < 2; ++it) {
#if VLB_P8_WDRAIN
        const int vo = min((pn0 + (WHICH - 2) * 32 + it * 128) * ldbB + rowB, maxB);
#else
        const int vo = min((pn0 + (WHICH - 2) * 128 + it * 64) * ldbB + rowB, maxB);
#endif
        __builtin_amdgcn_raw_ptr_buffer_load_lds(rsB, LDS_PTR(dst + (it * 512 + wave * 64) * 16), 16, vo, koff, 0, 0);
      }
    }
  };
  auto advance = [&]() {
    if (++kt_p == nk) {
      if (w_p + (int)gridDim.x < nt) {
        kt_p = 0;
        w_p += gridDim.x;
        setup(w_p);
      } else {
        kt_p = nk - 1;
      }
    }
  };
  constexpr int ORD1 = KEEPB ? 2 : 3, ORD2 = KEEPB ? 3 : 1, ORD3 = KEEPB ? 1 : 2;
  using I0 = std::integral_constant<int, 0>;
  using I1 = std::integral_constant<int, 1>;
  using W0 = std::integral_constant<int, 0>;
  using W1 = std::integral_constant<int, ORD1>;
  using W2 = std::integral_constant<int, ORD2>;
  using W3 = std::integral_constant<int, ORD3>;

  f32x4 acc[2 * FMH][4];
  bf16x8 af[FMH][2], bfr[2][2], bkeep[2][2];
  const int frow = lane & 15;
  const uint32_t c0 = (uint32_t)((((lane >> 4) ^ (frow >> 1)) << 4));
  const uint32_t lds0 = (uint32_t)(uintptr_t)LDS_PTR(smem);
  const uint32_t a_rd = lds0 + (uint32_t)((wm * FMH * 16 + frow) * 128) + c0;
  const uint32_t b_rd = lds0 + (uint32_t)(OFF_B0 + (wn * 32 + frow) * 128) + c0;

  auto read_a = [&](auto buf_c, auto half_c) {
    constexpr int B_ = decltype(buf_c)::value, H_ = decltype(half_c)::value;
    const uint32_t v0 = a_rd + B_ * BUF, v1 = v0 ^ 64u;
    constexpr int O = H_ * AHB;
    p8_lds_read<O + 0 * 2048>(af[0][0], v0); p8_lds_read<O + 0 * 2048>(af[0][1], v1);
    p8_lds_read<O + 1 * 2048>(af[1][0], v0); p8_lds_read<O + 1 * 2048>(af[1][1], v1);
    p8_lds_read<O + 2 * 2048>(af[2][0], v0); p8_lds_read<O + 2 * 2048>(af[2][1], v1);
    if constexpr (FMH >= 4) {
      p8_lds_read<O + 3 * 2048>(af[3][0], v0); p8_lds_read<O + 3 * 2048>(af[3][1], v1);
    }
    if constexpr (FMH == 5) {
      p8_lds_read<O + 4 * 2048>(af[4][0], v0); p8_lds_read<O + 4 * 2048>(af[4][1], v1);
    }
  };
  auto read_b = [&](auto buf_c, auto half_c, bf16x8 (&dst)[2][2]) {
// ... 59 lines not shown
      read_b(I0{}, I1{}, bfr);
      stage(W3{}, I1{});
      p8_barrier();
      compute(I0{}, I1{}, bfr);
      p8_barrier();
      read_a(I0{}, I1{});
      advance();
      stage(W0{}, I0{});
      p8_barrier();
      compute(I1{}, I1{}, bfr);
      p8_barrier();
      if constexpr (!KEEPB) read_b(I0{}, I0{}, bfr);
      stage(W1{}, I0{});
      __builtin_amdgcn_s_waitcnt(0x0F70 | VM_AHEAD);
      p8_barrier();
      if constexpr (KEEPB) compute(I1{}, I0{}, bkeep); else compute(I1{}, I0{}, bfr);
      p8_barrier();
      if constexpr (KEEPB) read_b(I1{}, I0{}, bkeep); else read_b(I1{}, I0{}, bfr);
      __builtin_amdgcn_sched_barrier(0);
      read_a(I1{}, I0{});
      stage(W2{}, I0{});
      p8_barrier();
      if constexpr (KEEPB) compute(I0{}, I0{}, bkeep); else compute(I0{}, I0{}, bfr);
      p8_barrier();
      read_b(I1{}, I1{}, bfr);
      stage(W3{}, I0{});
      p8_barrier();
      compute(I0{}, I1{}, bfr);
      p8_barrier();
      read_a(I1{}, I1{});
      advance();
      stage(W0{}, I1{});
      p8_barrier();
      compute(I1{}, I1{}, bfr);
      p8_barrier();
      if constexpr (!KEEPB) read_b(I1{}, I0{}, bfr);
      stage(W1{}, I1{});
      __builtin_amdgcn_s_waitcnt(0x0F70 | VM_AHEAD);
      p8_barrier();
      if constexpr (KEEPB) compute(I1{}, I0{}, bkeep); else compute(I1{}, I0{}, bfr);
      p8_barrier();
    }
    if (wm == 0) p8_barrier();
    if (stamp) {
      const unsigned long long now = __builtin_readcyclecounter();
      t_main += now - t_mark;
      t_mark = now;
    }

    int m0, n0;
    tile_of(w, m0, n0);
    if (p.ablate == 1) {
#if VLB_P8_WDRAIN
    } else if ((w + (int)gridDim.x < nt || EPI == 0 || (p.p8_flags & 2)) && !(FMH == 5 && (EPI == 6 || EPI == 7))) {
      if (m0 + BM <= p.M && n0 + BN <= p.N) p8_drain_w<FMH, EPI, false>(p, acc, lds0 + STG, m0, n0, wm, wn, tid, seed);
      else p8_drain_w<FMH, EPI, true>(p, acc, lds0 + STG, m0, n0, wm, wn, tid, seed);
#endif
    } else if (w + (int)gridDim.x >= nt) {
      __builtin_amdgcn_s_waitcnt(0x0F70);
      p8_barrier();
      p8_drain<FMH, EPI, (STG >= 131072 ? 4 : 3)>(p, acc, lds0, m0, n0, wm, wn, lane, tid, seed);
    } else {
      p8_drain<FMH, EPI, (SR == 32 ? 1 : 0)>(p, acc, lds0 + STG, m0, n0, wm, wn, lane, tid, seed);
    }
    if (p.p8_flags & 1) __builtin_amdgcn_s_waitcnt(0x0F70);
    p8_barrier();
    if (wm == 1 && w + (int)gridDim.x < nt) p8_barrier();
    if (stamp) t_epi += __builtin_readcyclecounter() - t_mark;
  }
  __builtin_amdgcn_s_waitcnt(0x0F70);
  if (stamp && tid == 0) {
    unsigned long long* t = stamps + 8 * blockIdx.x;
    t[2] = __builtin_readcyclecounter();
    t[3] = __builtin_amdgcn_s_memrealtime();
    t[4] = t_main;
    t[5] = t_epi;
    t[6] = (unsigned long long)((nt - (int)blockIdx.x + (int)gridDim.x - 1) / (int)gridDim.x);
  }
}

template <int FMH, bool KEEPB>
int p8_launch_epi(GemmParams& p, int epi, hipStream_t stream) {
  const int wgs = vlb_opt(VLB_OPT_P8_WGS);
  const int rc = dispatch_epi(epi, std::integer_sequence<int, 0, 1, 2, 3, 4, 5, 6, 7, 8, 10>{}, VLB_ERR_ARG, [&](auto e) {
    return launch_persistent<gemm_nt_p8_kernel<FMH, decltype(e)::value, KEEPB>>(163840, 512, 64 * FMH, 256, (wgs >= 8 && wgs <= 256) ? (wgs & ~7) : 256,
                                                                                vlb_opt(VLB_OPT_P8_GROUP), p, 1, stream, "vlb_gemm_nt_bf16(p8)", true);
  });
  return rc < 0 ? rc : 1;
}

inline bool aligned16(const void* q) { return ((uintptr_t)q & 15) == 0; }

}

int vlb_gemm_p8_try(GemmParams& p, hipStream_t stream) {
  const int mode = vlb_opt(VLB_OPT_P8_MODE), min_tiles = vlb_opt(VLB_OPT_P8_MIN_TILES);
  if (!mode || p.out_f32 != 0 || p.c_split_stride != 0) return 0;
  if ((p.K % 128) != 0 || p.k_per_split < p.K) return 0;
  int epi;
  if (p.act == 0 && p.res && p.res_stats) epi = p.drop_thr ? 6 : 7;
  else if (p.act == 0) epi = p.res ? (p.drop_thr ? 3 : 4) : (p.drop_thr ? -1 : 0);
  else if (p.act == 4) epi = 1;
  else if (p.act == 5) epi = 2;
  else if (p.act == 2) epi = 5;
  else if (p.act == 7 && p.res && !p.drop_thr) epi = 8;
  else if (p.act == 8 && !p.res && !p.drop_thr) epi = 10;
  else epi = -1;
  if (epi < 0) return 0;
  if ((p.ldc % 8) || !aligned16(p.C) || (p.lda % 8) || (p.ldb % 8) || !aligned16(p.A) || !aligned16(p.B)) return 0;
  if (p.res && ((p.ldres % 8) || !aligned16(p.res))) return 0;
  if ((epi == 2 || epi == 10) && ((p.ldaux % 8) || !aligned16(p.aux))) return 0;
  if (epi == 1 && p.pre && ((p.ldpre % 8) || !aligned16(p.pre))) return 0;
  if (p.bias && ((uintptr_t)p.bias & 15)) return 0;
  if (p.res_stats && (((uintptr_t)p.res_gamma & 15) || ((uintptr_t)p.res_beta & 15) || ((uintptr_t)p.res_stats & 7))) return 0;
  if ((long)p.M * p.lda * 2 >= (1L << 31) || (long)p.N * p.ldb * 2 >= (1L << 31)) return 0;
  const long nn = vlb_cdiv(p.N, 256);
  const long t3 = (long)vlb_cdiv(p.M, 192) * nn, t4 = (long)vlb_cdiv(p.M, 256) * nn, t5 = (long)vlb_cdiv(p.M, 320) * nn;
  const double c3 = (double)((t3 + 255) / 256) * 192.0 * 1.15, c4 = (double)((t4 + 255) / 256) * 256.0, c5 = (double)((t5 + 255) / 256) * 320.0;
  const bool ok3 = t3 >= min_tiles, ok4 = t4 >= min_tiles || (t4 >= 128 && p.K >= 1536), ok5 = t5 >= min_tiles;
  int fmh = 0;
  double best = 1e30;
  if (ok4) { fmh = 4; best = c4; }
  if (ok5 && c5 < 0.97 * best) { fmh = 5; best = c5; }
  if (ok3 && vlb_opt(VLB_OPT_P8_TILE192) && c3 < 0.97 * best) { fmh = 3; best = c3; }
  if (mode == 3 || mode == 4 || mode == 5) fmh = mode;
  if (!fmh) return 0;
  p.ablate = vlb_opt(VLB_OPT_P8_ABLATE);
  p.p8_flags = (vlb_opt(VLB_OPT_P8_DRAIN) & 1) | (vlb_opt(VLB_OPT_P8_LASTW) ? 2 : 0);
  if (fmh == 3) return p8_launch_epi<3, true>(p, epi, stream);
  if (fmh == 5) return p8_launch_epi<5, false>(p, epi, stream);
  return vlb_opt(VLB_OPT_P8_KEEPB) ? p8_launch_epi<4, true>(p, epi, stream) : p8_launch_epi<4, false>(p, epi, stream);
}
```

vl-bert_amd/csrc/gemm_params.h:

```cpp
#pragma once
#include <utility>

#include "options.h"
#include "tile_order.h"
#include "vlb_common.h"

struct GemmParams {
  const bf16_t* A; long lda;
  const bf16_t* B; long ldb;
  int M, N, K;
  int k_per_split;
  const float* bias;
  int act;
  const bf16_t* aux; long ldaux;
  bf16_t* pre; long ldpre;
  const bf16_t* res; long ldres;
  const float* res_stats; const float* res_gamma; const float* res_beta;
  int c_f16;
  int ablate;
  int p8_flags;
  int stagger;
  uint32_t drop_thr; float drop_scale; const uint32_t* seed; uint32_t tag;
  void* C; long ldc;
  long c_split_stride;
  int out_f32;
  int ntm, ntn;
  int tile_group;
  int conv_C, conv_H, conv_W, conv_dil;
  const bf16_t* zero;
};

#define GLDS_PTR(p) ((const __attribute__((address_space(1))) void*)(p))
#define LDS_PTR(p) ((__attribute__((address_space(3))) void*)(p))

int vlb_gemm_p8_try(GemmParams& p, hipStream_t stream);

int vlb_gemm_tn8_try(GemmParams& p, float* C, long ldc, float* colsum, float* workspace, long workspace_floats, int accumulate,
                     bool force_slab, hipStream_t stream);
int vlb_tn8_pick_splits(int Mo, int No, int R);
int vlb_gemm_tn8_group(int n, const void* const* A, const long* lda, const void* const* B, const long* ldb, float* const* C,
                       const long* ldc, int R, const int* Mo, const int* No, float* const* colsum, float* workspace,
                       long workspace_floats, int accumulate, int* slices, long* ws_off, hipStream_t stream);

template <auto KERNEL>
static int launch_persistent(int smem, int block, int bm, int bn, int grid_cap, int tile_group, GemmParams& p, int splits,
                             hipStream_t stream, const char* name, bool lds_required = false) {
  static bool attr_set = false;
  if (!attr_set) {
    const hipError_t e = hipFuncSetAttribute((const void*)KERNEL, hipFuncAttributeMaxDynamicSharedMemorySize, smem);
    if (e != hipSuccess && lds_required) {
      vlb_set_error("%s: cannot reserve %d bytes of LDS: %s", name, smem, hipGetErrorString(e));
      return VLB_ERR_HIP;
    }
    attr_set = true;
  }
  p.ntm = vlb_cdiv(p.M, bm);
  p.ntn = vlb_cdiv(p.N, bn);
  p.tile_group = tile_group < 1 ? 1 : tile_group;
  int gx = p.ntm * p.ntn;
  if (gx > grid_cap) gx = grid_cap;
  hipLaunchKernelGGL(KERNEL, dim3(gx, splits), dim3(block), smem, stream, p);
  VLB_CHECK_LAUNCH(name);
  return VLB_OK;
}

template <int... E, typename F>
static int dispatch_epi(int cls, std::integer_sequence<int, E...>, int other, F&& f) {
  int rc = other;
  (void)((cls == E && (rc = f(std::integral_constant<int, E>{}), true)) || ...);
  return rc;
}
```

vl-bert_amd/csrc/gemm_tn8.hip:

```cpp
#include <math.h>
#include <stdlib.h>

#include <type_traits>

#include "gemm_params.h"

namespace {

typedef __attribute__((ext_vector_type(4))) short s16x4;
typedef __attribute__((ext_vector_type(2))) vlb_h16 bf16x2_t;
#ifdef VLB_ACT_F16
#define VLB_FDOT2 __builtin_amdgcn_fdot2
#else
#define VLB_FDOT2 __builtin_amdgcn_fdot2_f32_bf16
#endif

template <int OFF>
__device__ __forceinline__ void tn8_tr_read(s16x4& dst, uint32_t vaddr) {
  asm volatile("ds_read_b64_tr_b16 %0, %1 offset:%2" : "=v"(dst) : "v"(vaddr), "n"(OFF));
}

__device__ __forceinline__ void tn8_barrier() {
  asm volatile("" ::: "memory");
  __builtin_amdgcn_s_barrier();
  asm volatile("" ::: "memory");
}

__device__ __forceinline__ bf16x8 tn8_frag(s16x4 lo, s16x4 hi) {
  typedef __attribute__((ext_vector_type(8))) short s16x8;
  const s16x8 v = __builtin_shufflevector(lo, hi, 0, 1, 2, 3, 4, 5, 6, 7);
  return __builtin_bit_cast(bf16x8, v);
}

struct Tn8Desc {
  const bf16_t* A; const bf16_t* B;
  float* C;
  float* colsum;
  long c_split_stride;
  int lda, ldb, ldc;
  int Mo, No, R;
  int ntm, ntn, tile_group;
  int nsplit, kt_per_split;
  int item0, nitems;
  int accumulate;
  const float* rowscale;
};
constexpr int TN8_MAX_GROUP = 4;
struct Tn8Group {
  Tn8Desc d[TN8_MAX_GROUP];
  int n, nitems;
  unsigned long long* stamps;
};

template <bool TABLE, int ABL = 0>
__global__ __launch_bounds__(512, 2) void gemm_tn8_kernel(const Tn8Group grp, const Tn8Desc* __restrict__ tab) {
  auto D = [&](int gi) -> Tn8Desc {
    if constexpr (TABLE) return tab[gi];
    else return grp.d[gi];
  };
  constexpr int HB = 64 * 256;
  constexpr int OFF_A0 = 0, OFF_A1 = HB, OFF_B0 = 2 * HB, OFF_B1 = 3 * HB;
  constexpr int BUF = 4 * HB;
  extern __shared__ __attribute__((aligned(16))) char smem[];

  const int tid = threadIdx.x, lane = tid & 63;
  const int wave = __builtin_amdgcn_readfirstlane(tid >> 6);
  const int wm = wave >> 2, wn = wave & 3;
  const int nitems = grp.nitems;
  if ((int)blockIdx.x >= nitems) return;
  if (grp.stamps && tid == 0) {
    unsigned long long* t = grp.stamps + 4 * blockIdx.x;
    t[0] = __builtin_readcyclecounter();
    t[1] = __builtin_amdgcn_s_memrealtime();
  }

  auto item_of = [&](int w, int& gi, int& m0, int& n0, int& kt0, int& nk) {
    gi = 0;
    w = vlb_xcd_order(w, nitems);
    if constexpr (TABLE) {
      int lo = 0, hi = grp.n;
      while (hi - lo > 1) {
        const int mid = (lo + hi) >> 1;
        if (w >= tab[mid].item0) lo = mid; else hi = mid;
      }
      gi = lo;
    } else {
#pragma unroll
      for (int q = 1; q < TN8_MAX_GROUP; ++q)
        if (q < grp.n && w >= grp.d[q].item0) gi = q;
    }
    const Tn8Desc d = D(gi);
    const int wl = w - d.item0, ntile = d.ntm * d.ntn;
    const int sp = wl / ntile, t = wl - sp * ntile;
    int tile_m, tile_n;
    vlb_tile_of(t, d.ntm, d.ntn, d.tile_group, tile_m, tile_n);
    m0 = tile_m * 256;
    n0 = tile_n * 256;
    kt0 = sp * d.kt_per_split;
    nk = min((d.R >> 6) - kt0, d.kt_per_split);
  };
  const int step = (int)gridDim.x;

  const int srow = tid >> 4, sc = tid & 15;
  const int sf = (srow & 3) | (((srow >> 3) & 1) << 2);
  const int lc = ((((sc >> 1) ^ sf) << 1) | (sc & 1)) * 8;
  __amdgpu_buffer_rsrc_t rsA, rsB;
  int ldaB = 0, ldbB = 0, clampA = 0, clampB = 0, rowA = 0, rowB = 0;
  int w_p = blockIdx.x, kt_p = 0, nk_p = 0, kt0_p = 0, pm0 = 0, pn0 = 0;
  auto setup = [&](int w) {
    int gi;
    item_of(w, gi, pm0, pn0, kt0_p, nk_p);
    if constexpr ((ABL & 8) != 0) { gi = 0; pm0 = 0; pn0 = 0; kt0_p = 0; }
    const Tn8Desc d = D(gi);
    rsA = __builtin_amdgcn_make_buffer_rsrc((void*)d.A, 0, 0x7FFFFFFF, 0x00020000);
    rsB = __builtin_amdgcn_make_buffer_rsrc((void*)d.B, 0, 0x7FFFFFFF, 0x00020000);
    ldaB = d.lda * 2; ldbB = d.ldb * 2;
    clampA = d.lda - 8; clampB = d.ldb - 8;
    rowA = srow * ldaB; rowB = srow * ldbB;
  };
  auto stage = [&](auto which_c, auto buf_c) {
    constexpr int WHICH = decltype(which_c)::value, B_ = decltype(buf_c)::value;
    if constexpr ((ABL & 1) != 0) return;
    const int kt = kt0_p + kt_p;
    if constexpr (WHICH < 2) {
      char* dst = smem + B_ * BUF + (WHICH == 0 ? OFF_A0 : OFF_A1);
      const int vo = rowA + 2 * min(pm0 + WHICH * 128 + lc, clampA);
#pragma unroll
      for (int it = 0; it < 2; ++it)
        __builtin_amdgcn_raw_ptr_buffer_load_lds(rsA, LDS_PTR(dst + (it * 512 + wave * 64) * 16), 16, vo, (kt * 64 + it * 32) * ldaB, 0, 0);
    } else {
      char* dst = smem + B_ * BUF + (WHICH == 2 ? OFF_B0 : OFF_B1);
      const int vo = rowB + 2 * min(pn0 + (WHICH - 2) * 128 + lc, clampB);
#pragma unroll
      for (int it = 0; it < 2; ++it)
        __builtin_amdgcn_raw_ptr_buffer_load_lds(rsB, LDS_PTR(dst + (it * 512 + wave * 64) * 16), 16, vo, (kt * 64 + it * 32) * ldbB, 0, 0);
    }
  };
  auto advance = [&]() {
    if (++kt_p == nk_p) {
      const int w_next = w_p + step;
      if (w_next < nitems) {
        kt_p = 0;
        w_p = w_next;
        setup(w_p);
      } else {
        kt_p = nk_p - 1;
      }
    }
  };
  using I0 = std::integral_constant<int, 0>;
  using I1 = std::integral_constant<int, 1>;
  using W0 = std::integral_constant<int, 0>;
  using W1 = std::integral_constant<int, 3>;
  using W2 = std::integral_constant<int, 1>;
  using W3 = std::integral_constant<int, 2>;

  constexpr int NI = 4, NJ = 2, KS = 2, KROWS = 32;
  f32x4 acc[2 * NI][2 * NJ];
  s16x4 alo[NI * KS], ahi[NI * KS], blo[NJ * KS], bhi[NJ * KS];
  float csum[2 * NI];
  const int L = lane & 15, g = lane >> 4;
  const int fl = (L >> 2) | ((g & 1) << 2);
  const uint32_t lds0 = (uint32_t)(uintptr_t)LDS_PTR(smem);
  const uint32_t lane_off = lds0 + (uint32_t)((8 * g + (L >> 2)) * 256 + (L & 3) * 8);
  uint32_t a_fo[NI], b_fo[NJ];
#pragma unroll
  for (int i = 0; i < NI; ++i)
    a_fo[i] = lane_off + (uint32_t)(((wm * 4 + i) ^ fl) << 5);
#pragma unroll
  for (int j = 0; j < NJ; ++j)
    b_fo[j] = lane_off + (uint32_t)(OFF_B0 + (((wn * 2 + j) ^ fl) << 5));

  auto read_a = [&](auto buf_c, auto half_c) {
    if constexpr ((ABL & 2) != 0) return;
    constexpr int O = decltype(buf_c)::value * BUF + decltype(half_c)::value * HB;
#pragma unroll
    for (int i = 0; i < NI; ++i) {
      const uint32_t v = a_fo[i] + (uint32_t)O;
      tn8_tr_read<0>(alo[i * KS + 0], v);
      tn8_tr_read<4 * 256>(ahi[i * KS + 0], v);
      tn8_tr_read<KROWS * 256>(alo[i * KS + 1], v);
      tn8_tr_read<KROWS * 256 + 4 * 256>(ahi[i * KS + 1], v);
// ... 188 lines not shown

static unsigned long long* g_tn8_stamps = nullptr;
extern "C" int vlb_tn8_set_stamps(void* dev) {
  g_tn8_stamps = (unsigned long long*)dev;
  return VLB_OK;
}

int vlb_tn8_pick_splits(int Mo, int No, int R) {
  const long tiles = (long)vlb_cdiv(Mo, 256) * vlb_cdiv(No, 256);
  const int pairs = R / 128;
  const long ldw = (No + 3) / 4 * 4;
  double best = -1.0;
  int best_sp = 1;
  for (int sp = 1; sp <= pairs && sp <= 64; ++sp) {
    const long items = tiles * sp;
    const long rounds = (items + 255) / 256;
    const int per = vlb_cdiv(pairs, sp);
    if ((long)vlb_cdiv(pairs, per) != sp) continue;
    const double t = (double)rounds * (per * 2 * 1.6 + 6.0) + (sp > 1 ? 2.0 * sp * Mo * (double)ldw * 4.0 / 4.0e6 : 0.0);
    if (best < 0 || t < best) { best = t; best_sp = sp; }
  }
  return best_sp;
}

static int tile_group_for(int ntm, int ntn) {
  const int group = vlb_opt(VLB_OPT_TN8_GROUP);
  return group > 0 ? (group < ntm ? group : ntm) : vlb_square_tile_group(ntm, ntn);
}

template <bool TABLE, int ABL>
static int tn8_launch_k(Tn8Group& grp, const Tn8Desc* tab, int gx, hipStream_t stream) {
  constexpr int smem = 131072;
  static bool attr_set = false;
  if (!attr_set) {
    hipError_t e = hipFuncSetAttribute((const void*)gemm_tn8_kernel<TABLE, ABL>, hipFuncAttributeMaxDynamicSharedMemorySize, smem);
    if (e != hipSuccess) {
      vlb_set_error("gemm_tn8: cannot reserve %d bytes of LDS: %s", smem, hipGetErrorString(e));
      return VLB_ERR_HIP;
    }
    attr_set = true;
  }
  hipLaunchKernelGGL((gemm_tn8_kernel<TABLE, ABL>), dim3(gx), dim3(512), smem, stream, grp, tab);
  VLB_CHECK_LAUNCH("vlb_wgrad_tn_bf16(tn8)");
  return VLB_OK;
}

template <bool TABLE>
static int tn8_launch_t(Tn8Group& grp, const Tn8Desc* tab, hipStream_t stream) {
  const int wgs = vlb_opt(VLB_OPT_TN8_WGS);
  const int cap = (wgs >= 8 && wgs <= 256) ? wgs : 256;
  const int gx = grp.nitems > cap ? cap : grp.nitems;
  grp.stamps = g_tn8_stamps;
#ifdef VLB_TN8_PROBE
  if (const int ablate = vlb_opt(VLB_OPT_TN8_ABLATE); !TABLE && ablate) {
#define TN8_ABL(A) \
  if ((ablate & 15) == A) return tn8_launch_k<false, A>(grp, tab, gx, stream);
    TN8_ABL(1) TN8_ABL(2) TN8_ABL(3) TN8_ABL(4) TN8_ABL(5) TN8_ABL(6) TN8_ABL(8) TN8_ABL(12) TN8_ABL(14)
#undef TN8_ABL
  }
#endif
  return tn8_launch_k<TABLE, 0>(grp, tab, gx, stream);
}

static int tn8_launch(Tn8Group& grp, hipStream_t stream) { return tn8_launch_t<false>(grp, nullptr, stream); }

static bool tn8_shape_ok(long lda, long ldb, long ldc, int R) {
  if ((R % 128) != 0 || R < 256) return false;
  if ((lda % 8) || (ldb % 8) || lda < 8 || ldb < 8 || (ldc % 4)) return false;
  if ((long)R * lda * 2 >= (1L << 31) || (long)R * ldb * 2 >= (1L << 31)) return false;
  return true;
}

int vlb_gemm_tn8_try(GemmParams& p, float* C, long ldc, float* colsum, float* workspace, long workspace_floats, int accumulate,
                     bool force_slab, hipStream_t stream) {
  if (!vlb_opt(VLB_OPT_TN8_MODE)) return 0;
  const int R = p.K, Mo = p.M, No = p.N;
  if (!tn8_shape_ok(p.lda, p.ldb, ldc, R)) return 0;
  const int ntm = vlb_cdiv(Mo, 256), ntn = vlb_cdiv(No, 256);
  const long tiles = (long)ntm * ntn;
  const int pairs = R / 128;
  const long ldw = (No + 3) / 4 * 4;
  int splits = vlb_tn8_pick_splits(Mo, No, R);
  if (tiles * splits < 128) return 0;
  const int per = vlb_cdiv(pairs, splits);
  splits = vlb_cdiv(pairs, per);
  const bool slab = splits > 1 || force_slab;
  if (slab && (!workspace || workspace_floats < (long)splits * Mo * ldw)) return 0;
  Tn8Group grp = {};
  Tn8Desc& d = grp.d[0];
  d.A = p.A; d.B = p.B; d.colsum = colsum;
  d.lda = (int)p.lda; d.ldb = (int)p.ldb; d.Mo = Mo; d.No = No; d.R = R;
  d.ntm = ntm; d.ntn = ntn; d.tile_group = tile_group_for(ntm, ntn);
  d.nsplit = splits; d.kt_per_split = per * 2; d.item0 = 0; d.nitems = (int)(tiles * splits);
  if (slab) { d.C = workspace; d.ldc = (int)ldw; d.c_split_stride = (long)Mo * ldw; d.accumulate = 0; }
  else { d.C = C; d.ldc = (int)ldc; d.c_split_stride = 0; d.accumulate = accumulate ? 1 : 0; }
  grp.n = 1; grp.nitems = d.nitems;
  const int rc = tn8_launch(grp, stream);
  return rc < 0 ? rc : splits;
}

int vlb_gemm_tn8_group(int n, const void* const* A, const long* lda, const void* const* B, const long* ldb, float* const* C,
                       const long* ldc, int R, const int* Mo, const int* No, float* const* colsum, float* workspace,
                       long workspace_floats, int accumulate, int* slices, long* ws_off, hipStream_t stream) {
  if (!vlb_opt(VLB_OPT_TN8_MODE) || n < 1 || n > TN8_MAX_GROUP) return 0;
  long tiles = 0;
  for (int i = 0; i < n; ++i) {
    if (!tn8_shape_ok(lda[i], ldb[i], ldc[i], R)) return 0;
    tiles += (long)vlb_cdiv(Mo[i], 256) * vlb_cdiv(No[i], 256);
  }
  const int pairs = R / 128;
  int splits = (int)(256 / tiles);
  if (splits < 1) splits = 1;
  if (splits > pairs) splits = pairs;
  if (tiles * splits < 128) return 0;
  const int per = vlb_cdiv(pairs, splits);
  splits = vlb_cdiv(pairs, per);
  Tn8Group grp = {};
  long off = 0;
  int item = 0;
  for (int i = 0; i < n; ++i) {
    Tn8Desc& d = grp.d[i];
    const long ldw = (No[i] + 3) / 4 * 4;
    d.A = (const bf16_t*)A[i]; d.B = (const bf16_t*)B[i]; d.colsum = colsum ? colsum[i] : nullptr;
    d.lda = (int)lda[i]; d.ldb = (int)ldb[i]; d.Mo = Mo[i]; d.No = No[i]; d.R = R;
    d.ntm = vlb_cdiv(Mo[i], 256); d.ntn = vlb_cdiv(No[i], 256); d.tile_group = tile_group_for(d.ntm, d.ntn);
    d.nsplit = splits; d.kt_per_split = per * 2;
    d.item0 = item; d.nitems = d.ntm * d.ntn * splits;
    item += d.nitems;
    if (splits > 1) {
      d.C = workspace + off; d.ldc = (int)ldw; d.c_split_stride = (long)Mo[i] * ldw; d.accumulate = 0;
      ws_off[i] = off;
      off += (long)splits * Mo[i] * ldw;
    } else {
      d.C = C[i]; d.ldc = (int)ldc[i]; d.c_split_stride = 0; d.accumulate = accumulate ? 1 : 0;
      ws_off[i] = 0;
    }
    slices[i] = splits;
  }
  if (splits > 1 && (!workspace || off > workspace_floats)) return 0;
  grp.n = n; grp.nitems = item;
  const int rc = tn8_launch(grp, stream);
  return rc < 0 ? rc : 1;
}


extern "C" long vlb_wgrad_tn_table_desc_bytes(void) { return (long)sizeof(Tn8Desc); }

extern "C" int vlb_wgrad_tn_table_pack(int n, const void* const* A, const long* lda, const void* const* B, const long* ldb, float* const* C,
                                       const long* ldc, const int* R, const int* Mo, const int* No, float* const* colsum,
                                       const float* const* rowscale, int accumulate, void* host_out, long host_bytes) {
  VLB_CHECK_ARG(n >= 1 && A && B && C && lda && ldb && ldc && R && Mo && No && host_out, "vlb_wgrad_tn_table_pack: null argument");
  VLB_CHECK_ARG(host_bytes >= (long)n * (long)sizeof(Tn8Desc), "vlb_wgrad_tn_table_pack: output buffer too small");
  Tn8Desc* out = (Tn8Desc*)host_out;
  int item = 0;
  for (int i = 0; i < n; ++i) {
    if (!A[i] || !B[i] || !C[i] || Mo[i] < 1 || No[i] < 1) {
      vlb_set_error("vlb_wgrad_tn_table_pack: bad product %d", i);
      return VLB_ERR_ARG;
    }
    if (!tn8_shape_ok(lda[i], ldb[i], ldc[i], R[i])) return 0;
    Tn8Desc d = {};
    d.A = (const bf16_t*)A[i]; d.B = (const bf16_t*)B[i]; d.C = C[i]; d.colsum = colsum ? colsum[i] : nullptr;
    d.rowscale = rowscale ? rowscale[i] : nullptr;
    d.lda = (int)lda[i]; d.ldb = (int)ldb[i]; d.ldc = (int)ldc[i]; d.Mo = Mo[i]; d.No = No[i]; d.R = R[i];
    d.ntm = vlb_cdiv(Mo[i], 256); d.ntn = vlb_cdiv(No[i], 256); d.tile_group = tile_group_for(d.ntm, d.ntn);
    d.nsplit = 1; d.kt_per_split = R[i] / 64; d.c_split_stride = 0; d.accumulate = accumulate ? 1 : 0;
    d.item0 = item; d.nitems = d.ntm * d.ntn;
    item += d.nitems;
    out[i] = d;
  }
  return item;
}

extern "C" int vlb_wgrad_tn_table_launch(const void* desc_dev, int n, int nitems, hipStream_t stream) {
  VLB_CHECK_ARG(desc_dev && n >= 1 && nitems >= 1, "vlb_wgrad_tn_table_launch: bad argument");
  Tn8Group grp = {};
  grp.n = n; grp.nitems = nitems;
  return tn8_launch_t<true>(grp, (const Tn8Desc*)desc_dev, stream);
}
// ... 1 lines not shown
```

vl-bert_amd/csrc/loss.hip:

```cpp
#include "vlb_common.h"

__device__ __forceinline__ void online_merge(float& m, float& s, float m2, float s2) {
  const float mn = fmaxf(m, m2);
  if (mn == -INFINITY) return;
  s = s * __expf(m - mn) + s2 * __expf(m2 - mn);
  m = mn;
}

__device__ __forceinline__ void block_online_reduce(float& m, float& s, float* sh) {
#pragma unroll
  for (int o = 32; o > 0; o >>= 1) {
    const float m2 = __shfl_xor(m, o, 64), s2 = __shfl_xor(s, o, 64);
    online_merge(m, s, m2, s2);
  }
  const int wave = threadIdx.x >> 6, lane = threadIdx.x & 63;
  __syncthreads();
  if (lane == 0) {
    sh[wave * 2] = m;
    sh[wave * 2 + 1] = s;
  }
  __syncthreads();
  m = sh[0];
  s = sh[1];
#pragma unroll
// ... 2 lines not shown

__device__ __forceinline__ float block_sum(float v, float* sh) {
  v = wave_sum(v);
  const int wave = threadIdx.x >> 6, lane = threadIdx.x & 63;
  __syncthreads();
  if (lane == 0) sh[wave] = v;
  __syncthreads();
  return sh[0] + sh[1] + sh[2] + sh[3];
}

__global__ void count_labels_kernel(const int64_t* __restrict__ labels, int n, float* __restrict__ counts) {
  int c = 0;
  for (int i = blockIdx.x * 256 + threadIdx.x; i < n; i += gridDim.x * 256) c += (labels[i] >= 0);
  float f = wave_sum((float)c);
  if ((threadIdx.x & 63) == 0 && f != 0.f) atomicAdd(counts, f);
}

template <bool DS = false>
__global__ __launch_bounds__(256) void ce_fwd_bwd_kernel(bf16_t* __restrict__ logits, long ld, int V, const int64_t* __restrict__ labels,
                                                         const float* __restrict__ n_valid, float gscale, float* __restrict__ loss_out,
                                                         bf16_t* __restrict__ logits_copy, long ldcopy,
                                                         const float* __restrict__ n_valid2 = nullptr, float* __restrict__ loss_out2 = nullptr,
                                                         const float* __restrict__ dscale = nullptr) {
  if (DS) gscale = __fmul_rn(gscale, *dscale);
  __shared__ float sh[16];
  const int row = blockIdx.x;
  if (n_valid2 && (float)row >= *n_valid) {
    n_valid = n_valid2;
    loss_out = loss_out2;
  }
  bf16_t* x = logits + (long)row * ld;
  const long label = labels[row];
  const int ldv = (int)ld;
  if (logits_copy) {
    bf16_t* cp = logits_copy + (long)row * ldcopy;
    for (int c = threadIdx.x * 8; c < V; c += 2048) {
      if (c + 8 <= V) *(uint4*)(cp + c) = *(const uint4*)(x + c);
      else for (int k = c; k < V; ++k) cp[k] = x[k];
    }
  }
  if (label < 0 || label >= V) {
    for (int c = threadIdx.x * 8; c < ldv; c += 2048) *(uint4*)(x + c) = make_uint4(0, 0, 0, 0);
    return;
  }
  float m = -INFINITY, s = 0.f;
  for (int c = threadIdx.x * 8; c < V; c += 2048) {
    const uint4 w = *(const uint4*)(x + c);
    const uint32_t ww[4] = {w.x, w.y, w.z, w.w};
#pragma unroll
    for (int k = 0; k < 4; ++k) {
      const float a = bflo(ww[k]), b = bfhi(ww[k]);
      if (c + 2 * k < V) online_merge(m, s, a, 1.f);
      if (c + 2 * k + 1 < V) online_merge(m, s, b, 1.f);
    }
  }
  block_online_reduce(m, s, sh);
  const float lse = m + __logf(s);
  const float nv = fmaxf(*n_valid, 1.f);
  if (threadIdx.x == 0) atomicAdd(loss_out, (lse - bf2f(x[label])) / nv);
  const float sc = gscale / nv;
  __syncthreads();
  for (int c = threadIdx.x * 8; c < ldv; c += 2048) {
    const uint4 w = *(const uint4*)(x + c);
    const uint32_t ww[4] = {w.x, w.y, w.z, w.w};
    uint32_t o[4];
#pragma unroll
    for (int k = 0; k < 4; ++k) {
      const int c0 = c + 2 * k, c1 = c0 + 1;
      float g0 = (c0 < V) ? __expf(bflo(ww[k]) - lse) : 0.f;
      float g1 = (c1 < V) ? __expf(bfhi(ww[k]) - lse) : 0.f;
      if (c0 == label) g0 -= 1.f;
      if (c1 == label) g1 -= 1.f;
      o[k] = pack2bf(g0 * sc, g1 * sc);
    }
    *(uint4*)(x + c) = make_uint4(o[0], o[1], o[2], o[3]);
  }
}

#define MLM_TILE_CHUNKS 16
__global__ __launch_bounds__(1024) void mlm_compact_kernel(const int64_t* __restrict__ labels, const int32_t* __restrict__ src_rows, int n,
                                                           int n_split, int V, int cap, int32_t* __restrict__ sel_pos,
                                                           int32_t* __restrict__ sel_src, int64_t* __restrict__ labels_c,
                                                           float* __restrict__ count0, float* __restrict__ count1,
                                                           int32_t* __restrict__ overflow) {
  __shared__ int wsum[16], wsum0[16];
  const int tid = threadIdx.x, lane = tid & 63, wave = tid >> 6;
  const unsigned long long below = (1ull << lane) - 1ull;
  int total = 0, n0 = 0;
  for (int tile0 = 0; tile0 < n; tile0 += 1024 * MLM_TILE_CHUNKS) {
    const int first = tile0 + wave * MLM_TILE_CHUNKS * 64;
    int lab[MLM_TILE_CHUNKS];
    unsigned long long bal[MLM_TILE_CHUNKS];
    int wtot = 0, wtot0 = 0;
#pragma unroll
    for (int i = 0; i < MLM_TILE_CHUNKS; ++i) {
      const int idx = first + i * 64 + lane;
      const int64_t l = (idx < n) ? labels[idx] : (int64_t)-1;
      lab[i] = (int)l;
      bal[i] = __ballot(l >= 0 && l < V);
    }
#pragma unroll
    for (int i = 0; i < MLM_TILE_CHUNKS; ++i) {
      const int d = n_split - (first + i * 64);
      const unsigned long long front = d <= 0 ? 0ull : (d >= 64 ? ~0ull : (1ull << d) - 1ull);
      wtot += __popcll(bal[i]);
      wtot0 += __popcll(bal[i] & front);
    }
    __syncthreads();
    if (lane == 0) {
      wsum[wave] = wtot;
      wsum0[wave] = wtot0;
    }
    __syncthreads();
    int k = total;
#pragma unroll
    for (int w = 0; w < 16; ++w) {
      if (w < wave) k += wsum[w];
      total += wsum[w];
      n0 += wsum0[w];
    }
#pragma unroll
    for (int i = 0; i < MLM_TILE_CHUNKS; ++i) {
      if ((bal[i] >> lane) & 1ull) {
        const int kk = k + __popcll(bal[i] & below), idx = first + i * 64 + lane;
        if (kk < cap) {
          sel_pos[kk] = idx;
          sel_src[kk] = src_rows[idx];
          labels_c[kk] = (int64_t)lab[i];
        }
      }
      k += __popcll(bal[i]);
    }
  }
  for (int q = total + tid; q < cap; q += 1024) {
    sel_pos[q] = -1;
    sel_src[q] = -1;
    labels_c[q] = -1;
  }
  if (tid == 0) {
    const int kept = min(total, cap);
    n0 = min(n0, kept);
    *count0 = (float)n0;
    *count1 = (float)(kept - n0);
    if (total > cap) *overflow = 1;
  }
}

extern "C" int vlb_mlm_compact(const int64_t* labels, const int32_t* src_rows, int n, int n_split, int V, int cap, int32_t* sel_pos,
                               int32_t* sel_src, int64_t* labels_c, float* count0, float* count1, int32_t* overflow, hipStream_t stream) {
  VLB_CHECK_ARG(labels && src_rows && sel_pos && sel_src && labels_c && count0 && count1 && overflow, "vlb_mlm_compact: null argument");
  VLB_CHECK_ARG(n > 0 && cap > 0 && n_split >= 0 && n_split <= n, "vlb_mlm_compact: bad sizes");
  hipLaunchKernelGGL(mlm_compact_kernel, dim3(1), dim3(1024), 0, stream, labels, src_rows, n, n_split, V, cap, sel_pos, sel_src, labels_c,
                     count0, count1, overflow);
  VLB_CHECK_LAUNCH("vlb_mlm_compact");
  return VLB_OK;
}

static int ce_fwd_bwd_compact(void* logits, long ld, int rows, int V, const int64_t* labels_c, const float* count0, const float* count1,
                              float gscale, const float* dscale, float* loss_out0, float* loss_out1, hipStream_t stream) {
  if (rows <= 0) return VLB_OK;
  VLB_CHECK_ARG(logits && labels_c && count0 && count1 && loss_out0 && loss_out1, "vlb_ce_fwd_bwd_compact: null argument");
  VLB_CHECK_ARG(ld >= V && (ld % 8) == 0, "vlb_ce_fwd_bwd_compact: ld=%ld must be >= V=%d and a multiple of 8", ld, V);
  if (dscale)
    hipLaunchKernelGGL(ce_fwd_bwd_kernel<true>, dim3(rows), dim3(256), 0, stream, (bf16_t*)logits, ld, V, labels_c, count0, gscale, loss_out0,
                       (bf16_t*)nullptr, 0L, count1, loss_out1, dscale);
  else
    hipLaunchKernelGGL(ce_fwd_bwd_kernel<false>, dim3(rows), dim3(256), 0, stream, (bf16_t*)logits, ld, V, labels_c, count0, gscale, loss_out0,
                       (bf16_t*)nullptr, 0L, count1, loss_out1, (const float*)nullptr);
  VLB_CHECK_LAUNCH("vlb_ce_fwd_bwd_compact");
  return VLB_OK;
}

extern "C" int vlb_ce_fwd_bwd_compact(void* logits, long ld, int rows, int V, const int64_t* labels_c, const float* count0,
                                      const float* count1, float gscale, float* loss_out0, float* loss_out1, hipStream_t stream) {
  return ce_fwd_bwd_compact(logits, ld, rows, V, labels_c, count0, count1, gscale, nullptr, loss_out0, loss_out1, stream);
}

extern "C" int vlb_ce_fwd_bwd_compact_ds(void* logits, long ld, int rows, int V, const int64_t* labels_c, const float* count0,
                                         const float* count1, float gscale, const float* dscale, float* loss_out0, float* loss_out1,
                                         hipStream_t stream) {
  return ce_fwd_bwd_compact(logits, ld, rows, V, labels_c, count0, count1, gscale, dscale, loss_out0, loss_out1, stream);
}

__global__ __launch_bounds__(256) void soft_valid_kernel(const float* __restrict__ target, long ldt, int C, int rows, float* __restrict__ tsum,
                                                         float* __restrict__ counts) {
  const int row = blockIdx.x * 4 + (threadIdx.x >> 6), lane = threadIdx.x & 63;
  if (row >= rows) return;
  const float* t = target + (long)row * ldt;
  float s = 0.f;
  for (int c = lane; c < C; c += 512) {
    float v[8];
#pragma unroll
    for (int u = 0; u < 8; ++u) v[u] = (c + 64 * u < C) ? t[c + 64 * u] : 0.f;
#pragma unroll
    for (int u = 0; u < 8; ++u)
      if (c + 64 * u < C) s += v[u];
  }
  s = wave_sum(s);
  if (lane == 0) {
    tsum[row] = s;
    if (fabsf(s - 1.f) < 0.1f) atomicAdd(counts, 1.f);
  }
}

template <bool DS = false>
__global__ __launch_bounds__(256) void soft_ce_fwd_bwd_kernel(bf16_t* __restrict__ logits, long ld, int C, const float* __restrict__ target,
                                                              long ldt, const float* __restrict__ tsum, const float* __restrict__ n_valid,
                                                              float gscale, float* __restrict__ loss_out, bf16_t* __restrict__ logits_copy,
                                                              long ldcopy, const float* __restrict__ dscale = nullptr) {
  __shared__ float sh[16];
  if (DS) gscale = __fmul_rn(gscale, *dscale);
  const int row = blockIdx.x;
  bf16_t* x = logits + (long)row * ld;
  const float* t = target + (long)row * ldt;
  const int ldv = (int)ld;
  if (logits_copy) {
    bf16_t* cp = logits_copy + (long)row * ldcopy;
    for (int c = threadIdx.x; c < C; c += 256) cp[c] = x[c];
  }
  const float ts = tsum[row];
  if (!(fabsf(ts - 1.f) < 0.1f)) {
    for (int c = threadIdx.x; c < ldv; c += 256) x[c] = 0;
    return;
  }
  float m = -INFINITY, s = 0.f, dot = 0.f;
  for (int c = threadIdx.x; c < C; c += 256) {
    const float v = bf2f(x[c]);
    online_merge(m, s, v, 1.f);
    dot += t[c] * v;
  }
  block_online_reduce(m, s, sh);
  dot = block_sum(dot, sh + 8);
  const float lse = m + __logf(s);
  const float nv = fmaxf(*n_valid, 1.f);
  if (threadIdx.x == 0) atomicAdd(loss_out, (lse * ts - dot) / nv);
  const float sc = gscale / nv;
  for (int c = threadIdx.x; c < ldv; c += 256) {
    float g = 0.f;
// ... 140 lines not shown
```

vl-bert_amd/csrc/options.h:

```cpp
#pragma once

#define VLB_OPTIONS(X)                                                                                                                  \
                                                                                 \
                                \
  X(P8_MODE, "p8_mode", "VLB_GEMM_P8", 1)                                                                                               \
                         \
  X(P8_KEEPB, "p8_keepb", "VLB_GEMM_P8_KEEPB", 1)                                                                                       \
                                                                                             \
  X(P8_GROUP, "p8_group", "VLB_GEMM_P8_GROUP", 2)                                                                                       \
                       \
  X(P8_MIN_TILES, "p8_min_tiles", "VLB_GEMM_P8_MIN_TILES", 160)                                                                         \
              \
  X(P8_WGS, "p8_wgs", "VLB_GEMM_P8_WGS", 256)                                                                                           \
                                         \
  X(P8_ABLATE, "p8_ablate", nullptr, 0)                                                                                                 \
                                                                                       \
  X(P8_TILE192, "p8_tile192", "VLB_GEMM_P8_192", 1)                                                                                     \
                                                    \
  X(P8_DRAIN, "p8_drain", "VLB_GEMM_P8_DRAIN", 0)                                                                                       \
                                         \
  X(P8_LASTW, "p8_lastw", "VLB_GEMM_P8_LASTW", 0)                                                                                       \
                                                                                                    \
                                                                   \
  X(NT_RING, "nt_ring", "VLB_GEMM_NT_RING", 1)                                                                                          \
                                                         \
  X(NT_STAGGER, "nt_stagger", "VLB_GEMM_NT_STAGGER", 0)                                                                                 \
                                                     \
  X(TILE_GROUP, "tile_group", "VLB_GEMM_TILE_GROUP", 4)                                                                                 \
                 \
  X(RESIDENT, "resident", "VLB_GEMM_RESIDENT", 512)                                                                                     \
               \
  X(EPI_SPECIALISE, "epi_specialise", "VLB_GEMM_EPI_SPECIALISE", 1)                                                                     \
   \
  X(NT_256, "nt_256", "VLB_GEMM_256", 1)                                                                                                \
                                                                                      \
  X(NT_256_GROUP, "nt_256_group", "VLB_GEMM_256_GROUP", 2)                                                                              \
                                                                           \
                                                                \
  X(TN_GROUP, "tn_group", "VLB_GEMM_TN_GROUP", -1)                                                                                      \
                                                                           \
                                                                                                     \
  X(TN8_MODE, "tn8_mode", "VLB_GEMM_TN8", 1)                                                                                            \
                                                                  \
  X(TN8_WGS, "tn8_wgs", "VLB_GEMM_TN8_WGS", 256)                                                                                        \
                                                         \
  X(TN8_ABLATE, "tn8_ablate", nullptr, 0)                                                                                               \
                                                                \
  X(TN8_GROUP, "tn8_group", "VLB_GEMM_TN8_GROUP", 0)                                                                                    \
                                                                     \
                        \
  X(LN_FWD_ROWS, "ln_fwd_rows", "VLB_LN_FWD_ROWS", 0)                                                                                   \
                    \
  X(LN_BWD4, "ln_bwd4", "VLB_LN_BWD4", 1)

enum VlbOpt {
#define VLB_OPT_ID(id, name, env, dflt) VLB_OPT_##id,
  VLB_OPTIONS(VLB_OPT_ID)
#undef VLB_OPT_ID
  VLB_OPT_COUNT
};

int vlb_opt(VlbOpt o);
bool vlb_opt_set(const char* name, int value);
```

vl-bert_amd/engine.py:

```python
import math
import os
from collections import OrderedDict
from dataclasses import dataclass
from types import SimpleNamespace

import torch

from . import ops
from .side_streams import SideStreams

F32 = torch.float32
MAX_SEQ = 512
VIS_DIM = 2048
TAG_EMBED, TAG_DOWNSAMPLE = 1000, 1001


def _ru(x, m):
    return (x + m - 1) // m * m


@dataclass
class ModelConfig:
    hidden_size: int = 768
    num_hidden_layers: int = 12
# ... 200 lines not shown
        self.wT["vlbert.mlm_head.predictions.transform.dense.weight"] = zb(H, H)
        self.wT["vlbert.word_embeddings.weight"] = zb(H, self.Vp)
        self.wT["vlbert.mvrc_head.transform.dense.weight"] = zb(H, H)
        self.wT["vlbert.mvrc_head.region_cls_pred.weight"] = zb(H, self.Cp)
        self.wT["image_feature_extractor.obj_downsample.1.weight"] = zb(2 * VIS_DIM, H)
        if cfg.with_pooler:
            self.wT["vlbert.pooler.dense.weight"] = zb(H, H)
        if cfg.with_rel_loss:
            self.wT["vlbert.relationsip_head.caption_image_relationship.weight"] = zb(H, 64)

        self.layer = [self._layer_record(l) for l in range(L)]

        self.seed = torch.tensor([((seed * 2 + 1) & 0x7FFFFFFF)], dtype=torch.int32, device=d)
        self._seed_prev = torch.zeros_like(self.seed)
        self._last_p_a, self._seed_moved = None, False
        self.adam = torch.tensor([lr, betas[0], betas[1], eps, weight_decay, 0.0, max_grad_norm, 0.0], dtype=F32, device=d)
        self.hyper = dict(betas=(float(betas[0]), float(betas[1])), eps=float(eps), weight_decay=float(weight_decay))
        if self._scaler_spec is not None:
            self.scaler = LS.LossScaler(self._scaler_spec, d)
        self.sumsq_ws = zf(2048)
        self.losses = zf(4)
        self.counts = zf(4)
        self.metric_acc = torch.zeros((4, 2), dtype=torch.int64, device=d)

        self.in_boxes = zf(B, R, 4 + VIS_DIM)
        self.in_im_info = zf(B, 5)
        Bt = self.Bt
        self.in_text = torch.zeros((Bt, T), dtype=torch.int64, device=d)
        self.in_mlm_labels = torch.full((Bt, T), -1, dtype=torch.int64, device=d)
        self.in_mvrc_ops = torch.zeros((B, R), dtype=torch.int64, device=d)
        self.in_mvrc_labels = zf(B, R, C)
        self.in_rel_label = torch.zeros((B,), dtype=torch.int64, device=d)
        self.text_mask = torch.zeros((Bt, T), dtype=torch.uint8, device=d)
        self.box_mask = torch.zeros((Bt, R), dtype=torch.uint8, device=d)
        i32 = lambda *s: torch.zeros(s, dtype=torch.int32, device=d)
        self.lay = dict(code=i32(Bt, self.S), text_len=i32(Bt), nobj=i32(Bt), text_rows=i32(Bt, T), obj_rows=i32(Bt, R),
                        attn_mask=zf(Bt, self.S))

        M, BT, BR, S, nh = self.M, self.BT, self.BR, self.S, cfg.num_attention_heads
        self.Mp128 = _ru(M, 128)
        self._row_padded = {}

        def zbm(cols):
            full = zb(self.Mp128, cols)
            view = full[:M]
            self._row_padded[view.data_ptr()] = full
            return view
        self.a_ds = zb(BR, 2 * VIS_DIM)
        self.obj_reps = zb(BR, H)
        self.objvis, self.st_objvis = zb(BR, H), zf(BR, 2)
        self.textvis, self.st_textvis = zb(Bt, H), zf(Bt, 2)
        self.emb_pre, self.st_emb = zb(M, H), zf(M, 2)
        self.X = [zbm(H) for _ in range(L + 1)]
        self.QKV = [zb(M, 3 * H) for _ in range(L)]
        self.CTX = [zbm(H) for _ in range(L)]
        self.LSE = [zf(Bt, nh, S) for _ in range(L)]
        self.hp_res = os.environ.get("VLB_RESIDUAL_STREAM", "f16ln") != "bf16"
        zdt = torch.float16 if self.hp_res else ops.BF16
        zz = lambda *s: torch.zeros(s, dtype=zdt, device=d)
        self.Z1, self.ST1, self.Y1 = [zz(M, H) for _ in range(L)], [zf(M, 2) for _ in range(L)], [zbm(H) for _ in range(L)]
        self.U, self.G = [zb(M, I) for _ in range(L)], [zbm(I) for _ in range(L)]
        self.Z2, self.ST2 = [zz(M, H) for _ in range(L)], [zf(M, 2) for _ in range(L)]
        self.text_out, self.obj_out = zb(BT, H), zb(BR, H)
        self.mlm_u, self.mlm_g, self.mlm_h, self.st_mlm = zb(BT, H), zb(BT, H), zb(BT, H), zf(BT, 2)
        self.mlm_logits = zb(BT, self.Vp)
        self.mvrc_u, self.mvrc_g = zb(BR, H), zb(BR, H)
        self.mvrc_logits = zb(BR, self.Cp)
        self.mvrc_tsum = zf(BR)
        if cfg.with_pooler:
            self.pooled, self.d_pooled, self.d_pool_pre = zb(B, H), zb(B, H), zb(B, H)
        if cfg.with_rel_loss:
            self.rel_logits = zb(B, 64)
            self.rel_logits_copy = zb(B, 64) if keep_logits else None
        self.mlm_logits_copy = zb(BT, self.Vp) if keep_logits else None
        cap = min(self.BTp, max(256, _ru(int(math.ceil(0.20 * BT)), 256)))
        want = os.environ.get("VLB_MLM_COMPACT", "1") != "0" and not keep_logits and not core and cap < BT
        self.mlm_cap = cap if want else None
        self._mlm_compact_now = want
        if want:
            self.sel_pos = torch.full((cap,), -1, dtype=torch.int32, device=d)
            self.sel_src = torch.full((cap,), -1, dtype=torch.int32, device=d)
            self.labels_c = torch.full((cap,), -1, dtype=torch.int64, device=d)
            self.mlm_overflow = torch.zeros((1,), dtype=torch.int32, device=d)
            self.d_text_out_c = zb(cap, H)
        self.mvrc_logits_copy = zb(BR, self.Cp) if keep_logits else None

        self.dXa, self.dXb = zb(M, H), zb(M, H)
        self.dZ = zb(M, H)
        self._pairs = os.environ.get("VLB_WGRAD_PAIRS", "1") != "0"
        self._pair_tables = {}
        nset = 4 if self._pairs else 2
        self.dD2, self.dD1 = [zbm(H) for _ in range(nset)], [zbm(H) for _ in range(nset)]
        self.dU2 = [zbm(I) for _ in range(nset)]
        self.dQKV2 = [zbm(3 * H) for _ in range(nset)]
        self.dCTX = zb(M, H)
        self.d_mlm_h, self.d_mlm_g, self.d_mlm_u = zb(BT, H), zb(BT, H), zb(BT, H)
        self.d_text_out, self.d_obj_out = zb(BT, H), zb(BR, H)
        self.d_mvrc_u = zb(BR, H)
        self.d_textvis, self.d_objvis = zf(Bt, H), zf(BR, H)
        self.d_obj_reps = zf(BR, H)
        self.d_yds = zb(BR, H)
        self.d_afeat = zb(BR, VIS_DIM)
        if core:
            self.in_text_type = torch.zeros((Bt, T), dtype=torch.int64, device=d)
            self.tv_in, self.ovl_in = zb(BT, H), zb(BR, 2 * H)
            self.tv_n, self.st_tv = zb(BT, H), zf(BT, 2)
            self.d_tv_n, self.d_ol = zf(BT, H), zf(BR, H)
            self.d_tv_in, self.d_ovl_in = zb(BT, H), zb(BR, 2 * H)
        need = [ops.wgrad_workspace_floats(n, k, rp) for n, k, rp in
                ((3 * H, H, self.Mp), (H, H, self.Mp), (I, H, self.Mp), (H, I, self.Mp), (V, H, self.BTp), (H, H, self.BTp),
                 (C, H, self.BRp), (H, H, self.BRp), (H, 2 * VIS_DIM, self.BRp))]
        need_dec = ops.wgrad_workspace_floats(self.BT, H, self.Vp)
        need.append(need_dec)
        need.append(3 * (3 * H * H + H * H + 2 * I * H) + 64)
        self.wg_ws = zf(max(max(need), 4))
        self.side = torch.cuda.Stream(device=d) if (d.type == "cuda" and os.environ.get("VLB_WGRAD_STREAM", "1") != "0") else None
        self.wg_ws_main = zf(max(need_dec, 4)) if self.side is not None else self.wg_ws
        self._hazards = SideStreams()
        self.ln_ws = zf(ops.ln_bwd_workspace_floats(H))
        self._ln_slices = list(zf(min(2 * L + 1, 32), ops.ln_bwd_workspace_floats(H)).unbind(0))
        self._ln_pending = []
        self.graph = None
        self._weights_dirty = True
        self.buckets = None
        self._wT_stale = self._gather_pending = self._vision_stale = False
        self._dp_hook = None
        from .parallel import force_exchange
        if (world > 1 or force_exchange()) and self._own_flat:
            from .parallel import GradBuckets
            vstart = min((o for n, o in self.P.offsets.items() if n.startswith("image_feature_extractor.") and
                          not n.startswith("image_feature_extractor.obj_downsample")), default=None)
            self.buckets = GradBuckets(self.P.grad, self.P.offsets, self.P.numel, L, group=process_group, vision_start=vstart,
                                       wire_dtype=dp_wire, mode=dp_mode)
            if self.buckets.sharded:
                self.shard_tbl = ops.ShardRanges(self.buckets.owned_rows(), d)
                self.wshard = torch.zeros(self.P.numel // world, dtype=ops.BF16, device=d)
                self.buckets.set_replicated_fp32(self._fp32_read_ranges())
        self.enc32 = None
        if encoder_fp32:
            if self.buckets is not None and self.buckets.sharded:
                raise ValueError("encoder_fp32 reads the fp32 master weights on every rank: use dp_mode='allreduce' (the sharded optimizer "
                                 "keeps them authoritative on the owner only)")
            from .encoder_f32 import EncoderF32
            self.enc32 = EncoderF32(self)

    def _layer_record(self, l):
        P, H, p = self.P, self.cfg.hidden_size, "vlbert.encoder.layer.%d." % l
        q = p + "attention.self.query."
        rec = SimpleNamespace(qkv=SimpleNamespace(
            w=P.view(P.w16, q + "weight", (3 * H, H), span=3), b=P.view(P.master, q + "bias", (3 * H,), span=3),
            gw=P.view(P.grad, q + "weight", (3 * H, H), span=3), gb=P.view(P.grad, q + "bias", (3 * H,), span=3), wT=self.wT[p + "qkv"]))
        for k, n in (("ao", "attention.output.dense."), ("f1", "intermediate.dense."), ("f2", "output.dense.")):
            setattr(rec, k, SimpleNamespace(w=self.w16[p + n + "weight"], b=self.w32[p + n + "bias"], gw=self.g32[p + n + "weight"],
                                            gb=self.g32[p + n + "bias"], wT=self.wT[p + n + "weight"]))
        for k, n in (("ln1", "attention.output.LayerNorm."), ("ln2", "output.LayerNorm.")):
            setattr(rec, k, SimpleNamespace(g=self.w32[p + n + "weight"], b=self.w32[p + n + "bias"], gg=self.g32[p + n + "weight"],
                                            gb=self.g32[p + n + "bias"]))
        return rec

    def load_state_dict(self, sd):
        vis = self._vision_names()
        for name in self.P.shapes:
            if name in vis:
                continue
            if name not in sd:
                raise KeyError("missing parameter %s" % name)
# ... 150 lines not shown
        self.metric_acc.zero_()

    def metric_counts(self):
        a = self.metric_acc.cpu()
        return {k: (int(a[i, 0]), int(a[i, 1])) for i, k in enumerate(self.METRIC_ROWS)}

    def _front_core_fwd(self, p_h):
        cfg, T, R, S, Bt = self.cfg, self.T, self.R, self.S, self.Bt
        H = cfg.hidden_size
        w16, w32, seed = self.w16, self.w32, self.seed
        ops.layernorm_fwd(self.tv_in, w32["vlbert.visual_ln_text.weight"], w32["vlbert.visual_ln_text.bias"], self.tv_n, self.st_tv)
        ops.layernorm_fwd(self.ovl_in[:, :H], w32["vlbert.visual_ln_object.weight"], w32["vlbert.visual_ln_object.bias"], self.objvis,
                          self.st_objvis)
        ops.embed_fwd(self.lay, self.in_text, self.in_text_type, w16["vlbert.word_embeddings.weight"],
                      w16["vlbert.position_embeddings.weight"], w16["vlbert.token_type_embeddings.weight"],
                      w16["vlbert.end_embedding.weight"], self.tv_n, (T * H, H), self.objvis, (R * H, H),
                      self.ovl_in[:, H:], (R * 2 * H, 2 * H), None, w32["vlbert.embedding_LayerNorm.weight"],
                      w32["vlbert.embedding_LayerNorm.bias"], self.emb_pre, self.st_emb, self.X[0], Bt, T, R, S, H, drop_p=p_h,
                      seed=seed, tag=TAG_EMBED)

    def _front_pretrain_fwd(self, p_h, p_ds):
        cfg, B, T, R, S, Bt, Ba = self.cfg, self.B, self.T, self.R, self.S, self.Bt, self.Ba
        H = cfg.hidden_size
        w16, w32, seed = self.w16, self.w32, self.seed
        e2e = self.vision is not None
        if e2e:
            self.vision.forward(self.in_image, self.in_boxes)
        ops.obj_prep_fwd(self.in_boxes, self.in_im_info, None if e2e else self.in_mvrc_ops.view(-1),
                         w32["object_mask_visual_embedding.weight"], self.a_ds, drop_p=p_ds, seed=seed, tag=TAG_DOWNSAMPLE)
        ops.gemm_nt(self.a_ds, w16["image_feature_extractor.obj_downsample.1.weight"], self.obj_reps,
                    bias=w32["image_feature_extractor.obj_downsample.1.bias"], act=ops.ACT_RELU)
        ops.zero_padded_rows(self.obj_reps, self.in_boxes)
        ops.layernorm_fwd(self.obj_reps, w32["vlbert.visual_ln_object.weight"], w32["vlbert.visual_ln_object.bias"], self.objvis,
                          self.st_objvis)
        reps0 = self.obj_reps.view(B, R * H)[:, :H]
        ops.layernorm_fwd(reps0, w32["vlbert.visual_ln_text.weight"], w32["vlbert.visual_ln_text.bias"], self.textvis[:B],
                          self.st_textvis[:B])
        if Ba:
            ops.layernorm_fwd(w16["aux_text_visual_embedding.weight"], w32["vlbert.visual_ln_text.weight"],
                              w32["vlbert.visual_ln_text.bias"], self.textvis[B:], self.st_textvis[B:], rows=Ba, ldx=0)
        ops.embed_fwd(self.lay, self.in_text, None, w16["vlbert.word_embeddings.weight"], w16["vlbert.position_embeddings.weight"],
                      w16["vlbert.token_type_embeddings.weight"], w16["vlbert.end_embedding.weight"], self.textvis, (H, 0),
                      self.objvis, (R * H, H), w16["object_linguistic_embeddings.weight"], (0, 0), self.in_mvrc_ops,
                      w32["vlbert.embedding_LayerNorm.weight"], w32["vlbert.embedding_LayerNorm.bias"], self.emb_pre, self.st_emb,
                      self.X[0], Bt, T, R, S, H, drop_p=p_h, seed=seed, tag=TAG_EMBED)

    def _encoder_heads_fwd(self, p_h, p_a):
        cfg, S, Bt = self.cfg, self.S, self.Bt
        H, V, C, L, nh = cfg.hidden_size, cfg.vocab_size, cfg.visual_region_classes, cfg.num_hidden_layers, cfg.num_attention_heads
        w16, w32, seed = self.w16, self.w32, self.seed
        mask = self.lay["attn_mask"]
        stale = self._gather_pending
        self._last_p_a, self._seed_moved = p_a, False
        if self.enc32 is not None:
            self.enc32.forward(p_h, p_a)
        for l in range(L if self.enc32 is None else 0):
            r, x = self.layer[l], self.X[l]
            if stale:
                self.buckets.wait_params(l)
            ops.gemm_nt(x, r.qkv.w, self.QKV[l], bias=r.qkv.b)
            ops.attention_fwd(self.QKV[l], mask, self.CTX[l], self.LSE[l], Bt, S, H, nh, drop_p=p_a, seed=seed, tag=l * 8 + 0)
            if self.hp_res and l > 0:
                ln = self.layer[l - 1].ln2
                res_kw = dict(res=self.Z2[l - 1], res_ln=(self.ST2[l - 1], ln.g, ln.b))
            else:
                res_kw = dict(res=x)
            ops.gemm_nt(self.CTX[l], r.ao.w, self.Z1[l], bias=r.ao.b, drop_p=p_h, seed=seed, tag=l * 8 + 1, **res_kw)
            ops.layernorm_fwd(self.Z1[l], r.ln1.g, r.ln1.b, self.Y1[l], self.ST1[l])
            ops.gemm_nt(self.Y1[l], r.f1.w, self.G[l], bias=r.f1.b, act=ops.ACT_GELU_D, pre=self.U[l])
            if self.hp_res:
                res_kw = dict(res=self.Z1[l], res_ln=(self.ST1[l], r.ln1.g, r.ln1.b))
            else:
                res_kw = dict(res=self.Y1[l])
            ops.gemm_nt(self.G[l], r.f2.w, self.Z2[l], bias=r.f2.b, drop_p=p_h, seed=seed, tag=l * 8 + 2, **res_kw)
            ops.layernorm_fwd(self.Z2[l], r.ln2.g, r.ln2.b, self.X[l + 1], self.ST2[l])
        if stale:
            self.buckets.wait_params("heads")
            self._gather_pending = False
        xl = self.X[L]
        compact = self._mlm_compact_now and self.with_heads
        nr = self.mlm_cap if compact else self.BT
        if compact:
            ops.mlm_compact(self.in_mlm_labels.view(-1), self.lay["text_rows"].view(-1), self.B * self.T, V, self.sel_pos, self.sel_src,
                            self.labels_c, self.counts[0:1], self.counts[2:3], self.mlm_overflow)
            ops.gather_rows(xl, self.sel_src, self.text_out[:nr])
        else:
            ops.gather_rows(xl, self.lay["text_rows"].view(-1), self.text_out)
        ops.gather_rows(xl, self.lay["obj_rows"].view(-1)[:self.BR], self.obj_out)
        if cfg.with_pooler:
            x0 = xl.view(Bt, S * H)[:self.B, :H]
            ops.gemm_nt(x0, w16["vlbert.pooler.dense.weight"], self.pooled, bias=w32["vlbert.pooler.dense.bias"], act=ops.ACT_TANH)
        if not self.with_heads:
            return
        if cfg.with_rel_loss:
            pr = "vlbert.relationsip_head.caption_image_relationship."
            ops.gemm_nt(self.pooled, w16[pr + "weight"], self.rel_logits[:, :2], bias=w32[pr + "bias"])
        pm = "vlbert.mlm_head.predictions."
        ops.gemm_nt(self.text_out[:nr], w16[pm + "transform.dense.weight"], self.mlm_g[:nr], bias=w32[pm + "transform.dense.bias"],
                    act=ops.ACT_GELU_D, pre=self.mlm_u[:nr])
        ops.layernorm_fwd(self.mlm_g[:nr], w32[pm + "transform.LayerNorm.weight"], w32[pm + "transform.LayerNorm.bias"], self.mlm_h[:nr],
                          self.st_mlm[:nr])
        ops.gemm_nt(self.mlm_h[:nr], w16["vlbert.word_embeddings.weight"], self.mlm_logits[:nr, :V], bias=w32[pm + "bias"])
        ops.gemm_nt(self.obj_out, w16["vlbert.mvrc_head.transform.dense.weight"], self.mvrc_g,
                    bias=w32["vlbert.mvrc_head.transform.dense.bias"], act=ops.ACT_GELU_D, pre=self.mvrc_u)
        ops.gemm_nt(self.mvrc_g, w16["vlbert.mvrc_head.region_cls_pred.weight"], self.mvrc_logits[:, :C],
                    bias=w32["vlbert.mvrc_head.region_cls_pred.bias"])

    def _losses_fwd_bwd(self, gscale, keep):
        B, T, Ba, V, C = self.B, self.T, self.Ba, self.cfg.vocab_size, self.cfg.visual_region_classes
        if keep:
            losses, mcopy, vcopy = self.losses, self.mlm_logits_copy, self.mvrc_logits_copy
        else:
            self.mlm_logits.copy_(self.mlm_logits_copy)
            self.mvrc_logits.copy_(self.mvrc_logits_copy)
            losses, mcopy, vcopy = torch.zeros_like(self.losses), None, None
        nw = B * T
        ds = self.scaler.scale if self.scaler is not None else None
        if self._mlm_compact_now:
            ops.ce_fwd_bwd_compact(self.mlm_logits[:self.mlm_cap], V, self.labels_c, self.counts[0:1], self.counts[2:3], losses[0:1],
                                   losses[2:3], gscale=gscale, dscale=ds)
        else:
            ops.ce_fwd_bwd(self.mlm_logits[:nw], V, self.in_mlm_labels.view(-1)[:nw], self.counts[0:1], losses[0:1], gscale=gscale,
                           logits_copy=mcopy[:nw] if mcopy is not None else None, dscale=ds)
            if Ba:
                ops.ce_fwd_bwd(self.mlm_logits[nw:], V, self.in_mlm_labels.view(-1)[nw:], self.counts[2:3], losses[2:3],
                               gscale=gscale, logits_copy=mcopy[nw:] if mcopy is not None else None, dscale=ds)
        ops.soft_ce_fwd_bwd(self.mvrc_logits, C, self.in_mvrc_labels.view(self.BR, C), self.mvrc_tsum, self.counts[1:2],
                            losses[1:2], gscale=gscale, logits_copy=vcopy, dscale=ds)
        if self.cfg.with_rel_loss:
            if not keep:
                self.rel_logits.copy_(self.rel_logits_copy)
            ops.ce_fwd_bwd(self.rel_logits, 2, self.in_rel_label, self.counts[3:4], losses[3:4], gscale=gscale,
                           logits_copy=self.rel_logits_copy if keep else None, dscale=ds)

    def _on_side(self, launch, items):
        self._hazards.run(self.side, launch, [dy for dy, _, _, _ in items], writes=[g for _, _, gw, gb in items for g in (gw, gb)])

    def _wgrad(self, dy, x, gw, gb):
        acc = not self._fresh_grads
        self._on_side(lambda: ops.wgrad_tn(dy, x, gw, colsum=gb, workspace=self.wg_ws, accumulate=acc), [(dy, x, gw, gb)])

    def _padded(self, items):
        pad = self._row_padded
        return [(pad.get(dy.data_ptr(), dy), pad.get(x.data_ptr(), x), gw, gb) for dy, x, gw, gb in items]

    def _wgrad_group(self, items):
        acc = not self._fresh_grads
        items = self._padded(items)
        if len({t.shape[0] for it in items for t in it[:2]}) != 1:
            items = [(dy[:self.M], x[:self.M], gw, gb) for dy, x, gw, gb in items]
        self._on_side(lambda: ops.wgrad_tn_group(items, workspace=self.wg_ws, accumulate=acc), items)

    def _wgrad_pair(self, items):
        acc = not self._fresh_grads
        items = self._padded(items)
        key = (acc,) + tuple(t.data_ptr() for it in items for t in it)
        tab = self._pair_tables.get(key)
        if tab is None:
            if self.dev.type == "cuda" and torch.cuda.is_current_stream_capturing():
                return False
            if len({t.shape[0] for it in items for t in it[:2]}) != 1:
                return False
            tab = ops.WgradTable([(dy, x, gw, gb, None) for dy, x, gw, gb in items], self.dev, accumulate=acc)
            self._pair_tables[key] = tab
        if not tab.ok:
            return False
        self._on_side(lambda: tab.run(), items)
        return True

    def _before_write(self, *bufs):
        self._hazards.before_write(*bufs)

    def _join_side(self):
        if self.side is not None:
            self._hazards.join([self.side])

    def _ln_bwd(self, dy, x, stats, gamma, dgamma, dbeta, **kw):
        if len(self._ln_pending) == len(self._ln_slices):
            self._flush_ln()
        ws = self._ln_slices[len(self._ln_pending)]
        slabs = ops.layernorm_bwd(dy, x, stats, gamma, dgamma=dgamma, dbeta=dbeta, workspace=ws, defer=True, **kw)
        if slabs:
            self._ln_pending.append((ws, slabs, dgamma, dbeta))

    def _flush_ln(self):
        if self._ln_pending:
            ops.ln_param_finalize_batch(self._ln_pending, self.cfg.hidden_size)
            self._ln_pending = []

    def backward(self, train=None, on_layer_done=None):
        will_launch = None
        if on_layer_done is None and self._dp_hook is not None:
            on_layer_done = self._dp_hook
        if on_layer_done is not None:
            user_hook = on_layer_done
            will_launch = getattr(getattr(user_hook, "__self__", None), "will_launch", None)

            def on_layer_done(what):
                self._flush_ln()
                user_hook(what)
        train = self.train if train is None else train
        cfg, B, T, R, S, Bt, Ba = self.cfg, self.B, self.T, self.R, self.S, self.Bt, self.Ba
        H, I, V, C, L, nh = cfg.hidden_size, cfg.intermediate_size, cfg.vocab_size, cfg.visual_region_classes, \
            cfg.num_hidden_layers, cfg.num_attention_heads
        p_h, p_a, p_ds = self._p(train)
        w16, w32, g32, wT, seed = self.w16, self.w32, self.g32, self.wT, self.seed
        if self._wT_stale:
            self.buckets.wait_params("all")
            self._refresh_transposes()
            self._wT_stale = False
        if self.buckets is not None and on_layer_done is None:
            self.buckets.invalidate()
        if self.with_heads:
            pm = "vlbert.mlm_head.predictions."
            compact = self._mlm_compact_now and not self.core
            nr = self.mlm_cap if compact else self.BT
            dlog = self.mlm_logits[:nr]
            self._wgrad(dlog[:, :V], self.mlm_h[:nr], g32["vlbert.word_embeddings.weight"], g32[pm + "bias"])
            ops.gemm_nt_splitk(dlog, wT["vlbert.word_embeddings.weight"], self.d_mlm_h[:nr], workspace=self.wg_ws_main)
            self._ln_bwd(self.d_mlm_h[:nr], self.mlm_g[:nr], self.st_mlm[:nr], w32[pm + "transform.LayerNorm.weight"],
                         g32[pm + "transform.LayerNorm.weight"], g32[pm + "transform.LayerNorm.bias"], dx=self.d_mlm_g[:nr])
            ops.mul_bf16(self.d_mlm_g[:nr], self.mlm_u[:nr], self.d_mlm_u[:nr])
            self._wgrad(self.d_mlm_u[:nr], self.text_out[:nr], g32[pm + "transform.dense.weight"], g32[pm + "transform.dense.bias"])
            if compact:
                ops.gemm_nt(self.d_mlm_u[:nr], wT[pm + "transform.dense.weight"], self.d_text_out_c)
                self.d_text_out.zero_()
                ops.scatter_rows(self.d_text_out_c, self.sel_pos, self.d_text_out)
            else:
                ops.gemm_nt(self.d_mlm_u, wT[pm + "transform.dense.weight"], self.d_text_out)
            dlog2 = self.mvrc_logits
            self._wgrad(dlog2[:, :C], self.mvrc_g, g32["vlbert.mvrc_head.region_cls_pred.weight"],
                        g32["vlbert.mvrc_head.region_cls_pred.bias"])
            ops.gemm_nt(dlog2, wT["vlbert.mvrc_head.region_cls_pred.weight"], self.d_mvrc_u, act=ops.ACT_MULAUX, aux=self.mvrc_u)
            self._wgrad(self.d_mvrc_u, self.obj_out, g32["vlbert.mvrc_head.transform.dense.weight"],
                        g32["vlbert.mvrc_head.transform.dense.bias"])
            ops.gemm_nt(self.d_mvrc_u, wT["vlbert.mvrc_head.transform.dense.weight"], self.d_obj_out)
            if cfg.with_rel_loss:
                pr = "vlbert.relationsip_head.caption_image_relationship."
                self._wgrad(self.rel_logits[:, :2], self.pooled, g32[pr + "weight"], g32[pr + "bias"])
                ops.gemm_nt(self.rel_logits, wT[pr + "weight"], self.d_pooled)
        dx = self.dXa
        if not self.seq_out:
            ops.head_grad_combine(self.d_text_out, self.d_obj_out, self.lay["code"], dx, Bt, T, R, S, H)
        if cfg.with_pooler and (cfg.with_rel_loss or not self.with_heads):
            ops.tanh_bwd(self.d_pooled, self.pooled, self.d_pool_pre)
            x0 = self.X[L].view(Bt, S * H)[:self.B, :H]
            self._wgrad(self.d_pool_pre, x0, g32["vlbert.pooler.dense.weight"], g32["vlbert.pooler.dense.bias"])
            dx0 = dx.view(Bt, S * H)[:self.B, :H]
            ops.gemm_nt(self.d_pool_pre, wT["vlbert.pooler.dense.weight"], dx0, res=dx0)
        if on_layer_done:
            self._join_side()
            on_layer_done("heads")
        mask = self.lay["attn_mask"]
        if self.enc32 is not None:
            dx = self.enc32.backward(dx, p_h, p_a, on_layer_done, will_launch)
        held = None
        for l in reversed(range(L if self.enc32 is None else 0)):
            r = self.layer[l]
            dx_next = self.dXb if dx is self.dXa else self.dXa
            par = l & (len(self.dD2) - 1)
            dD2, dD1, dU, dQKV = self.dD2[par], self.dD1[par], self.dU2[par], self.dQKV2[par]
            self._before_write(self.dZ, dD2)
            self._ln_bwd(dx, self.Z2[l], self.ST2[l], r.ln2.g, r.ln2.gg, r.ln2.gb, dx=self.dZ, dx_drop=dD2, drop_p=p_h, seed=seed,
                         tag=l * 8 + 2)
            self._before_write(dU)
            ops.gemm_nt(dD2, r.f2.wT, dU, act=ops.ACT_MULAUX, aux=self.U[l])
            ops.gemm_nt(dU, r.f1.wT, dx_next, res=self.dZ)
            self._before_write(self.dZ, dD1)
            self._ln_bwd(dx_next, self.Z1[l], self.ST1[l], r.ln1.g, r.ln1.gg, r.ln1.gb, dx=self.dZ, dx_drop=dD1, drop_p=p_h, seed=seed,
                         tag=l * 8 + 1)
            ops.gemm_nt(dD1, r.ao.wT, self.dCTX)
            self._before_write(dQKV)
            ops.attention_bwd(self.QKV[l], mask, self.CTX[l], self.LSE[l], self.dCTX, dQKV, Bt, S, H, nh, drop_p=p_a,
                              seed=seed, tag=l * 8 + 0)
            ops.gemm_nt(dQKV, r.qkv.wT, dx_next, res=self.dZ)
            wg = [(dD2, self.G[l], r.f2.gw, r.f2.gb), (dU, self.Y1[l], r.f1.gw, r.f1.gb), (dD1, self.CTX[l], r.ao.gw, r.ao.gb),
                  (dQKV, self.X[l], r.qkv.gw, r.qkv.gb)]
            dx = dx_next
            if self._pairs and (l & 1):
                held = (l, wg)
                continue
            finished = [l]
            if held is not None:
                if not self._wgrad_pair(held[1] + wg):
                    self._wgrad_group(held[1])
                    self._wgrad_group(wg)
                finished = [held[0], l]
                held = None
            else:
                self._wgrad_group(wg)
            for lf in finished:
                if on_layer_done and (will_launch is None or will_launch(lf)):
                    self._join_side()
                    on_layer_done(lf)
        if on_layer_done:
            self._join_side()
        else:
            self._hazards.before_accumulate(*self._front_grads())
        if self.core:
            self._front_core_bwd(dx, p_h)
        else:
            self._front_pretrain_bwd(dx, p_h, p_ds, on_layer_done)
# ... 456 lines not shown
```

vl-bert_amd/ops.py:

```python
import torch

from . import _lib

BF16 = _lib.act_torch_dtype()
ACT_NONE, ACT_GELU, ACT_RELU, ACT_DGELU, ACT_GELU_D, ACT_MULAUX, ACT_TANH = 0, 1, 2, 3, 4, 5, 6
OUT_BF16, OUT_F32, OUT_F32_ATOMIC = 0, 1, 2


_raw_stream = getattr(torch._C, "_cuda_getCurrentRawStream", None)


def _stream():
    if _raw_stream is not None:
        return _raw_stream(torch.cuda.current_device())
    return torch.cuda.current_stream().cuda_stream


def _p(t, dtype=None):
    if t is None:
        return None
    if not t.is_cuda:
        raise RuntimeError("vl-bert_amd ops need GPU tensors (got %s); there is no CPU path" % t.device)
    if dtype is not None and t.dtype != dtype:
        raise RuntimeError("expected dtype %s, got %s" % (dtype, t.dtype))
    return t.data_ptr()


def _ld(t):
    if t is None:
        return 0
    assert t.dim() == 2 and t.stride(1) == 1, "expected a 2-D tensor with unit inner stride"
    return t.stride(0) if t.shape[0] > 1 else max(t.stride(0), t.shape[1])


F16 = torch.float16


def gemm_nt(A, B, C, bias=None, act=ACT_NONE, aux=None, pre=None, res=None, drop_p=0.0, seed=None, tag=0,
            out_mode=OUT_BF16, splitk=0, K=None, res_ln=None):
    M, N = C.shape
    K = A.shape[1] if K is None else K
    assert A.shape[0] == M and B.shape[0] == N and B.shape[1] >= K and A.shape[1] >= K
    if res_ln is not None or C.dtype == F16:
        assert out_mode == OUT_BF16
        st, g, b = res_ln if res_ln is not None else (None, None, None)
        if res_ln is not None:
            assert res is not None and res.dtype == F16 and st.shape[0] >= M
        _lib.call("vlb_gemm_nt_bf16_ex", _p(A, BF16), _ld(A), _p(B, BF16), _ld(B), _p(C), _ld(C), M, N, K,
                  _p(bias, torch.float32), act, _p(aux, BF16), _ld(aux), _p(pre, BF16), _ld(pre), _p(res), _ld(res),
                  _p(st, torch.float32), _p(g, torch.float32), _p(b, torch.float32), 1 if C.dtype == F16 else 0,
                  float(drop_p), _p(seed), int(tag), out_mode, splitk, _stream())
        return C
    cdt = BF16 if out_mode == OUT_BF16 else torch.float32
    _lib.call("vlb_gemm_nt_bf16", _p(A, BF16), _ld(A), _p(B, BF16), _ld(B), _p(C, cdt), _ld(C), M, N, K,
              _p(bias, torch.float32), act, _p(aux, BF16), _ld(aux), _p(pre, BF16), _ld(pre), _p(res, BF16), _ld(res),
              float(drop_p), _p(seed), int(tag), out_mode, splitk, _stream())
    return C


def wgrad_nt(A, B, C, workspace=None):
    M, N = C.shape
    K = A.shape[1]
    assert A.shape[0] == M and B.shape[0] == N and B.shape[1] == K
    _lib.call("vlb_wgrad_nt_bf16", _p(A, BF16), _ld(A), _p(B, BF16), _ld(B), _p(C, torch.float32), _ld(C), M, N, K,
              _p(workspace, torch.float32), workspace.numel() if workspace is not None else 0, _stream())
    return C


def wgrad_tn(dy, x, C, colsum=None, workspace=None, accumulate=True):
    Mo, No = C.shape
    R = dy.shape[0]
    assert dy.shape[1] == Mo and x.shape[1] == No and x.shape[0] == R
    _lib.call("vlb_wgrad_tn_bf16", _p(dy, BF16), _ld(dy), _p(x, BF16), _ld(x), _p(C, torch.float32), _ld(C), R, Mo, No,
              _p(colsum, torch.float32), _p(workspace, torch.float32), workspace.numel() if workspace is not None else 0,
              int(bool(accumulate)), _stream())
    return C


class ZeroRanges:

    def __init__(self, base, ranges):
        self.base = base
        rows, starts, total = [], [0], 0
        for lo, hi in ranges:
            if hi <= lo:
                continue
            rows.append([lo, hi - lo])
            total += (hi - lo + 1023) // 1024
            starts.append(total)
        self.n, self.total = len(rows), total
        self.ranges = torch.tensor(rows, dtype=torch.int64).to(base.device) if rows else None
        self.starts = torch.tensor(starts, dtype=torch.int32).to(base.device)

    def run(self):
        if self.n:
            _lib.call("vlb_zero_ranges_f32", _p(self.base, torch.float32), self.ranges.data_ptr(), self.starts.data_ptr(), self.n,
                      self.total, _stream())


class CopyRanges:

    def __init__(self, rows, device):
        rows = [[int(a), int(b), int(n)] for a, b, n in rows if n > 0]
        starts, total = [0], 0
        for _, _, n in rows:
            total += (n + 1023) // 1024
            starts.append(total)
        self.rows, self.n, self.total = rows, len(rows), total
        self.ranges = torch.tensor(rows, dtype=torch.int64).reshape(-1, 3).to(device) if rows else None
        self.starts = torch.tensor(starts, dtype=torch.int32).to(device)

    def run(self, src, dst):
        if self.n:
            _lib.call("vlb_copy_ranges_f32", _p(src, torch.float32), _p(dst, torch.float32), self.ranges.data_ptr(), self.starts.data_ptr(),
                      self.n, self.total, _stream())


def wgrad_tn_group(items, workspace=None, accumulate=True):
    import ctypes
    n = len(items)
    R = items[0][0].shape[0]
    P, Lg, I = ctypes.c_void_p * n, ctypes.c_long * n, ctypes.c_int * n
    for dy, x, C, cs in items:
        assert dy.shape[0] == R and x.shape[0] == R and C.shape == (dy.shape[1], x.shape[1])
    A = P(*[_p(t[0], BF16) for t in items]); lda = Lg(*[_ld(t[0]) for t in items])
    B = P(*[_p(t[1], BF16) for t in items]); ldb = Lg(*[_ld(t[1]) for t in items])
    Cs = P(*[_p(t[2], torch.float32) for t in items]); ldc = Lg(*[_ld(t[2]) for t in items])
    Mo = I(*[t[0].shape[1] for t in items]); No = I(*[t[1].shape[1] for t in items])
    cs = P(*[_p(t[3], torch.float32) for t in items])
    _lib.call("vlb_wgrad_tn_group_bf16", n, A, lda, B, ldb, Cs, ldc, R, Mo, No, cs, _p(workspace, torch.float32),
              workspace.numel() if workspace is not None else 0, 1 if accumulate else 0, _stream())


class WgradTable:

    def __init__(self, items, device, accumulate=True):
        import ctypes
        lib = _lib.load()
        n = len(items)
        self.keep = list(items)
        P, Lg, I = ctypes.c_void_p * n, ctypes.c_long * n, ctypes.c_int * n
        for dy, x, C, cs, rs in items:
            assert dy.shape[0] == x.shape[0] and C.shape == (dy.shape[1], x.shape[1]) and dy.dtype == BF16 and x.dtype == BF16
        A = P(*[_p(t[0], BF16) for t in items]); lda = Lg(*[_ld(t[0]) for t in items])
        B = P(*[_p(t[1], BF16) for t in items]); ldb = Lg(*[_ld(t[1]) for t in items])
        Cs = P(*[_p(t[2], torch.float32) for t in items]); ldc = Lg(*[_ld(t[2]) for t in items])
        R = I(*[t[0].shape[0] for t in items])
        Mo = I(*[t[0].shape[1] for t in items]); No = I(*[t[1].shape[1] for t in items])
        cs = P(*[_p(t[3], torch.float32) for t in items]); rs = P(*[_p(t[4], torch.float32) for t in items])
        nbytes = int(lib.vlb_wgrad_tn_table_desc_bytes()) * n
        host = ctypes.create_string_buffer(nbytes)
        rc = lib.vlb_wgrad_tn_table_pack(n, A, lda, B, ldb, Cs, ldc, R, Mo, No, cs, rs, 1 if accumulate else 0, host, nbytes)
        if rc < 0:
            raise RuntimeError("vlb_wgrad_tn_table_pack failed (%d): %s" % (rc, lib.vlb_last_error().decode()))
        self.ok, self.n, self.nitems = rc > 0, n, rc
        self.flops = sum(2.0 * t[0].shape[0] * t[0].shape[1] * t[1].shape[1] for t in items)
        self.nbytes = sum(t[0].numel() * 2 + t[1].numel() * 2 + t[2].numel() * 4 for t in items)
        self.desc = torch.frombuffer(bytearray(host.raw), dtype=torch.uint8).to(device) if self.ok else None

    def run(self):
        if not self.ok:
            raise RuntimeError("WgradTable: a product is outside what the table kernel covers (row counts must be multiples of 128)")
        _lib.call("vlb_wgrad_tn_table_launch", self.desc.data_ptr(), self.n, self.nitems, _stream())


def gemm_nt_splitk(A, B, C, workspace=None):
    M, K = A.shape
    N = B.shape[0]
    _lib.call("vlb_gemm_nt_bf16_splitk", _p(A, BF16), _ld(A), _p(B, BF16), _ld(B), _p(C, BF16), _ld(C), M, N, K,
              _p(workspace, torch.float32), workspace.numel() if workspace is not None else 0, _stream())
    return C


class TransposeBatch:

    def __init__(self, pairs, device):
        desc, starts, total = [], [0], 0
        self.keep = list(pairs)
        for src, dst in pairs:
            R, C = src.shape
            assert dst.shape[0] == C and dst.shape[1] >= R and src.dtype == BF16 and dst.dtype == BF16
            desc.append([src.data_ptr(), _ld(src), dst.data_ptr(), _ld(dst), R, C])
            total += ((R + 63) // 64) * ((C + 63) // 64)
            starts.append(total)
        self.n, self.total = len(desc), total
        self.desc = torch.tensor(desc, dtype=torch.int64).to(device)
        self.starts = torch.tensor(starts, dtype=torch.int32).to(device)

    def run(self):
        _lib.call("vlb_transpose_batched_bf16", self.desc.data_ptr(), self.starts.data_ptr(), self.n, self.total, _stream())


def ln_bwd_workspace_floats(H):
    return int(_lib.load().vlb_layernorm_bwd_workspace_floats(H))


def wgrad_workspace_floats(M, N, K):
    return int(_lib.load().vlb_wgrad_workspace_floats(M, N, K))


def transpose(x, out, colsum=None):
    R, Cc = x.shape
    _lib.call("vlb_transpose_bf16", _p(x, BF16), _ld(x), _p(out, BF16), _ld(out), R, Cc, _p(colsum, torch.float32), _stream())
    return out


def layernorm_fwd(x, gamma, beta, y, stats=None, eps=1e-12, rows=None, ldx=None):
    H = x.shape[1]
    rows = x.shape[0] if rows is None else rows
    assert x.dtype in (BF16, F16)
    _lib.call("vlb_layernorm_fwd", _p(x), _ld(x) if ldx is None else ldx, _p(gamma, torch.float32), _p(beta, torch.float32), _p(y, BF16),
              _ld(y), _p(stats, torch.float32), rows, H, float(eps), 1 if x.dtype == F16 else 0, _stream())
    return y


def layernorm_bwd(dy, x, stats, gamma, dx=None, dx_drop=None, drop_p=0.0, seed=None, tag=0, dx_acc=None, dgamma=None,
                  dbeta=None, rows=None, ldx=None, ldacc=None, workspace=None, defer=False):
    H = x.shape[1]
    rows = x.shape[0] if rows is None else rows
    dy_f32 = 1 if dy.dtype == torch.float32 else 0
    assert x.dtype in (BF16, F16)
    _lib.call("vlb_layernorm_bwd_deferred" if defer else "vlb_layernorm_bwd", _p(dy), _ld(dy), dy_f32, _p(x),
              _ld(x) if ldx is None else ldx, _p(stats, torch.float32),
              _p(gamma, torch.float32), _p(dx, BF16), _ld(dx), _p(dx_drop, BF16), _ld(dx_drop), float(drop_p), _p(seed),
              int(tag), _p(dx_acc, torch.float32), _ld(dx_acc) if ldacc is None else ldacc, _p(dgamma, torch.float32),
              _p(dbeta, torch.float32), _p(workspace, torch.float32), rows, H, 1 if x.dtype == F16 else 0, _stream())
    return int(_lib.load().vlb_layernorm_bwd_slabs(rows)) if defer else None


def ln_param_finalize_batch(entries, H):
    import ctypes
    n = len(entries)
    if not n:
        return
    P, I = ctypes.c_void_p * n, ctypes.c_int * n
    _lib.call("vlb_ln_param_finalize_batch", n, P(*[_p(e[0], torch.float32) for e in entries]), I(*[int(e[1]) for e in entries]),
              P(*[_p(e[2], torch.float32) for e in entries]), P(*[_p(e[3], torch.float32) for e in entries]), int(H), _stream())


def attention_fwd(qkv, mask, ctx, lse, B, S, H, nh, drop_p=0.0, seed=None, tag=0):
    _lib.call("vlb_attention_fwd", _p(qkv, BF16), _p(mask, torch.float32), _p(ctx, BF16), _p(lse, torch.float32), B, S, H, nh,
              float(drop_p), _p(seed), int(tag), _stream())
    return ctx


def attention_bwd(qkv, mask, ctx, lse, dctx, dqkv, B, S, H, nh, drop_p=0.0, seed=None, tag=0):
    _lib.call("vlb_attention_bwd", _p(qkv, BF16), _p(mask, torch.float32), _p(ctx, BF16), _p(lse, torch.float32),
              _p(dctx, BF16), _p(dqkv, BF16), B, S, H, nh, float(drop_p), _p(seed), int(tag), _stream())
    return dqkv


# ... 35 lines not shown
              _p(mask_emb, torch.float32), _p(out, BF16), B, R, float(drop_p), _p(seed), int(tag), _stream())
    return out


def zero_padded_rows(x, boxes):
    B, R, ldb = boxes.shape
    _lib.call("vlb_zero_padded_rows_bf16", _p(x, BF16), _ld(x), _p(boxes, torch.float32), ldb, B * R, x.shape[1], _stream())
    return x


def masked_colsum(src, sel, dst, drop_p=0.0, seed=None, tag=0, row_elems=0, col_off=0):
    rows, C = src.shape
    _lib.call("vlb_masked_colsum", _p(src, BF16), _ld(src), _p(sel, torch.int64), rows, C, _p(dst, torch.float32), float(drop_p),
              _p(seed), int(tag), int(row_elems), int(col_off), _stream())


def embed_fwd(lay, text_ids, text_type, word_emb, pos_emb, type_emb, end_emb, text_vis, tv_strides, obj_vis, ov_strides,
              obj_ling, ol_strides, obj_ling_idx, gamma, beta, pre, stats, out, B, T, R, S, H, eps=1e-12, drop_p=0.0,
              seed=None, tag=0):
    _lib.call("vlb_embed_fwd", _p(lay["code"]), _p(lay["text_len"]), _p(text_ids, torch.int64), _p(text_type, torch.int64),
              _p(word_emb, BF16), _p(pos_emb, BF16), _p(type_emb, BF16), _p(end_emb, BF16),
              _p(text_vis, BF16), tv_strides[0], tv_strides[1], _p(obj_vis, BF16), ov_strides[0], ov_strides[1],
              _p(obj_ling, BF16), ol_strides[0], ol_strides[1], _p(obj_ling_idx, torch.int64),
              _p(gamma, torch.float32), _p(beta, torch.float32), _p(pre, BF16), _p(stats, torch.float32), _p(out, BF16),
              B, T, R, S, H, word_emb.shape[0], pos_emb.shape[0], float(eps), float(drop_p), _p(seed), int(tag), _stream())
    return out


def embed_bwd(dy, pre, stats, gamma, lay, text_ids, text_type, obj_ling_idx, d_word, d_pos, d_type, d_end, d_gamma, d_beta,
              d_text_vis, dtv_strides, d_obj_vis, dov_strides, d_obj_ling, dol_strides, B, T, R, S, H, drop_p=0.0, seed=None,
              tag=0, text_vis_zeroed=False):
    _lib.call("vlb_embed_bwd", _p(dy, BF16), _p(pre, BF16), _p(stats, torch.float32), _p(gamma, torch.float32), _p(lay["code"]),
              _p(lay["text_len"]), _p(text_ids, torch.int64), _p(text_type, torch.int64), _p(obj_ling_idx, torch.int64),
              _p(d_word, torch.float32), _p(d_pos, torch.float32), _p(d_type, torch.float32), _p(d_end, torch.float32),
              _p(d_gamma, torch.float32), _p(d_beta, torch.float32),
              _p(d_text_vis, torch.float32), dtv_strides[0], dtv_strides[1], _p(d_obj_vis, torch.float32), dov_strides[0],
              dov_strides[1], _p(d_obj_ling, torch.float32), dol_strides[0], dol_strides[1],
              B, T, R, S, H, d_word.shape[0], d_pos.shape[0], float(drop_p), _p(seed), int(tag), int(bool(text_vis_zeroed)),
              _stream())


def gather_rows(src, idx, out):
    n, H = out.shape
    _lib.call("vlb_gather_rows", _p(src, BF16), _p(idx, torch.int32), _p(out, BF16), n, H, _stream())
    return out


def head_grad_combine(d_text, d_obj, code, dx, B, T, R, S, H):
    _lib.call("vlb_head_grad_combine", _p(d_text, BF16), _p(d_obj, BF16), _p(code, torch.int32), _p(dx, BF16), B, T, R, S, H,
              _stream())
    return dx


def relu_bwd_cast(g, y, out):
    _lib.call("vlb_relu_bwd_cast", _p(g, torch.float32), _p(y, BF16), _p(out, BF16), g.numel(), _stream())
    return out


def dgelu_mul(dg, u, out):
    _lib.call("vlb_dgelu_mul", _p(dg, BF16), _p(u, BF16), _p(out, BF16), dg.numel(), _stream())
    return out


def tanh_bwd(dy, y, out):
    _lib.call("vlb_tanh_bwd", _p(dy, BF16), _p(y, BF16), _p(out, BF16), dy.numel(), _stream())
    return out


def mul_bf16(a, b, out):
    _lib.call("vlb_mul_bf16", _p(a, BF16), _p(b, BF16), _p(out, BF16), a.numel(), _stream())
    return out


def ce_fwd_bwd(logits, V, labels, counts, loss_out, gscale=1.0, logits_copy=None, dscale=None):
    rows = logits.shape[0]
    if dscale is not None:
        _lib.call("vlb_ce_fwd_bwd_ds", _p(logits, BF16), _ld(logits), rows, V, _p(labels, torch.int64), _p(counts, torch.float32),
                  float(gscale), _p(dscale, torch.float32), _p(loss_out, torch.float32), _p(logits_copy, BF16), _ld(logits_copy), _stream())
        return
    _lib.call("vlb_ce_fwd_bwd", _p(logits, BF16), _ld(logits), rows, V, _p(labels, torch.int64), _p(counts, torch.float32),
              float(gscale), _p(loss_out, torch.float32), _p(logits_copy, BF16), _ld(logits_copy), _stream())


def mlm_compact(labels, src_rows, n_split, V, sel_pos, sel_src, labels_c, count0, count1, overflow):
    _lib.call("vlb_mlm_compact", _p(labels, torch.int64), _p(src_rows, torch.int32), labels.numel(), int(n_split), int(V), sel_pos.numel(),
              _p(sel_pos, torch.int32), _p(sel_src, torch.int32), _p(labels_c, torch.int64), _p(count0, torch.float32),
              _p(count1, torch.float32), _p(overflow, torch.int32), _stream())


def ce_fwd_bwd_compact(logits, V, labels_c, count0, count1, loss_out0, loss_out1, gscale=1.0, dscale=None):
    if dscale is not None:
        _lib.call("vlb_ce_fwd_bwd_compact_ds", _p(logits, BF16), _ld(logits), logits.shape[0], V, _p(labels_c, torch.int64),
                  _p(count0, torch.float32), _p(count1, torch.float32), float(gscale), _p(dscale, torch.float32),
                  _p(loss_out0, torch.float32), _p(loss_out1, torch.float32), _stream())
        return
    _lib.call("vlb_ce_fwd_bwd_compact", _p(logits, BF16), _ld(logits), logits.shape[0], V, _p(labels_c, torch.int64),
              _p(count0, torch.float32), _p(count1, torch.float32), float(gscale), _p(loss_out0, torch.float32),
              _p(loss_out1, torch.float32), _stream())


def scatter_rows(src, idx, out):
    _lib.call("vlb_scatter_rows", _p(src, BF16), _p(idx, torch.int32), _p(out, BF16), idx.numel(), src.shape[1], _stream())
    return out


def soft_ce_fwd_bwd(logits, C, target, tsum, counts, loss_out, gscale=1.0, logits_copy=None, dscale=None):
    rows = logits.shape[0]
    if dscale is not None:
        _lib.call("vlb_soft_ce_fwd_bwd_ds", _p(logits, BF16), _ld(logits), rows, C, _p(target, torch.float32), _ld(target),
                  _p(tsum, torch.float32), _p(counts, torch.float32), float(gscale), _p(dscale, torch.float32),
                  _p(loss_out, torch.float32), _p(logits_copy, BF16), _ld(logits_copy), _stream())
        return
    _lib.call("vlb_soft_ce_fwd_bwd", _p(logits, BF16), _ld(logits), rows, C, _p(target, torch.float32), _ld(target),
              _p(tsum, torch.float32), _p(counts, torch.float32), float(gscale), _p(loss_out, torch.float32),
              _p(logits_copy, BF16), _ld(logits_copy), _stream())


def ce_eval(logits, V, labels, loss_out, acc, count0=None, count1=None, loss_out1=None, acc1=None, pred=None):
    _lib.call("vlb_ce_eval", _p(logits, BF16), _ld(logits), logits.shape[0], int(V), _p(labels, torch.int64), _p(count0, torch.float32),
              _p(count1, torch.float32), _p(loss_out, torch.float32), _p(loss_out1, torch.float32), _p(acc, torch.int64),
              _p(acc1, torch.int64), _p(pred, torch.int32), _stream())


def soft_ce_eval(logits, C, target, loss_out, acc):
    _lib.call("vlb_soft_ce_eval", _p(logits, BF16), _ld(logits), logits.shape[0], int(C), _p(target, torch.float32), _ld(target),
              _p(loss_out, torch.float32), _p(acc, torch.int64), _stream())


ARGMAX_PREDICT, ARGMAX_HARD, ARGMAX_GATHER, ARGMAX_GATHER_GT = 0, 1, 2, 3


def argmax_eval(logits, mode=ARGMAX_PREDICT, label=None, pred=None, score=None, probs=None, sum=None, count=None, C=None):
    rows = logits.shape[0]
    C = logits.shape[1] if C is None else int(C)
    if mode == ARGMAX_HARD:
        lp, ldl = _p(label, torch.int64), 0
        assert label.dim() == 1 and label.shape[0] == rows and label.is_contiguous()
    elif mode != ARGMAX_PREDICT:
        lp, ldl = _p(label, torch.float32), _ld(label)
        assert label.shape[0] == rows
    else:
        lp, ldl = None, 0
    for t in (pred, score):
        assert t is None or (t.is_contiguous() and t.numel() >= rows)
    _lib.call("vlb_argmax_eval", _p(logits, torch.float32), _ld(logits), rows, C, int(mode), lp, ldl, _p(pred, torch.int32),
              _p(score, torch.float32), _p(probs, torch.float32), _ld(probs),
              _p(sum, torch.float64 if mode == ARGMAX_GATHER else torch.int64), _p(count, torch.int64), _stream())


def binary_cls_eval(logits, label, acc, N=None):
    N = logits.shape[1] if N is None else int(N)
    assert label.shape[0] == logits.shape[0] and acc.numel() >= 4 and acc.is_contiguous()
    _lib.call("vlb_binary_cls_eval", _p(logits, torch.float32), _ld(logits), _p(label, torch.float32), _ld(label), logits.shape[0], N,
              _p(acc, torch.int64), _stream())


def joint_hits(pred_a, label_a, pred_r, label_r, acc):
    rows = pred_a.shape[0]
    for t in (pred_a, label_a, pred_r, label_r):
        assert t.dim() == 1 and t.shape[0] == rows and t.is_contiguous()
    _lib.call("vlb_joint_hits", _p(pred_a, torch.int32), _p(label_a, torch.int64), _p(pred_r, torch.int32), _p(label_r, torch.int64), rows,
              _p(acc, torch.int64), _stream())


def bce_logits_fwd_bwd(logits, A, label, loss_out, gscale=1.0, logits_copy=None, pos_weight=1.0, dscale=None):
    rows = logits.shape[0]
    if dscale is not None:
# ... 376 lines not shown
```

Before: 13950 samples/s.

## Limit MLM head GEMMs to device-counted kept rows after compaction

The MLM compaction kernel now writes the number of kept masked rows to a device counter. The vocab logits GEMM, its weight-gradient GEMM and the split-K dgrad GEMM read this counter inside their persistent kernels and skip row tiles past it, and the split-K reduce writes zeros there. Before, these GEMMs always processed the full compaction capacity, including padding rows. The change disables the ring and 256-tile fast paths and restricts epilogues when a row limit is given. It also relies on padding rows never being consumed downstream.

```diff
diff --git a/include/vlbert_hip.h b/include/vlbert_hip.h
--- a/include/vlbert_hip.h
+++ b/include/vlbert_hip.h
@@ -27,6 +27,15 @@
 
 int vlb_gemm_nt_bf16_splitk(const void* A, long lda, const void* B, long ldb, void* C, long ldc, int M, int N, int K,
                             float* workspace, long workspace_floats, vlb_stream_t stream);
+int vlb_gemm_nt_bf16_rows(const void* A, long lda, const void* B, long ldb, void* C, long ldc, int M, int N, int K,
+                          const float* bias, int act, const void* aux, long ldaux, void* pre, long ldpre,
+                          const void* res, long ldres, float drop_p, const uint32_t* seed, uint32_t tag,
+                          int out_mode, int splitk, const int32_t* row_limit, vlb_stream_t stream);
+int vlb_gemm_nt_bf16_splitk_rows(const void* A, long lda, const void* B, long ldb, void* C, long ldc, int M, int N, int K,
+                                 float* workspace, long workspace_floats, const int32_t* row_limit, vlb_stream_t stream);
+int vlb_wgrad_tn_bf16_rows(const void* A, long lda, const void* B, long ldb, float* C, long ldc, int R, int Mo, int No,
+                           float* colsum, float* workspace, long workspace_floats, int accumulate, const int32_t* row_limit,
+                           vlb_stream_t stream);
 int vlb_gemm_set_option(const char* name, int value);
 
 
@@ -91,6 +100,9 @@
 int vlb_scatter_rows(const void* src, const int32_t* idx, void* out, int n, int H, vlb_stream_t stream);
 int vlb_mlm_compact(const int64_t* labels, const int32_t* src_rows, int n, int n_split, int V, int cap, int32_t* sel_pos,
                     int32_t* sel_src, int64_t* labels_c, float* count0, float* count1, int32_t* overflow, vlb_stream_t stream);
+int vlb_mlm_compact_rows(const int64_t* labels, const int32_t* src_rows, int n, int n_split, int V, int cap, int32_t* sel_pos,
+                         int32_t* sel_src, int64_t* labels_c, float* count0, float* count1, int32_t* overflow, int32_t* kept,
+                         vlb_stream_t stream);
 int vlb_ce_fwd_bwd_compact(void* logits, long ld, int rows, int V, const int64_t* labels_c, const float* count0, const float* count1,
                            float gscale, float* loss_out0, float* loss_out1, vlb_stream_t stream);
 int vlb_head_grad_combine(const void* d_text, const void* d_obj, const int32_t* code, void* dx, int B, int T, int R,
diff --git a/vl-bert_amd/_lib.py b/vl-bert_amd/_lib.py
--- a/vl-bert_amd/_lib.py
+++ b/vl-bert_amd/_lib.py
@@ -19,6 +19,10 @@
 
 _SIGS = {
     "vlb_gemm_nt_bf16": "plplpliiipiplplplfpuiis",
+    "vlb_gemm_nt_bf16_rows": "plplpliiipiplplplfpuiips",
+    "vlb_gemm_nt_bf16_splitk_rows": "plplpliiiplps",
+    "vlb_wgrad_tn_bf16_rows": "plplpliiipplips",
+    "vlb_mlm_compact_rows": "ppiiiippppppps",
     "vlb_transpose_batched_bf16": "ppiis",
     "vlb_gemm_nt_bf16_splitk": "plplpliiipls",
     "vlb_transpose_bf16": "plpliips",
diff --git a/vl-bert_amd/csrc/gemm.hip b/vl-bert_amd/csrc/gemm.hip
--- a/vl-bert_amd/csrc/gemm.hip
+++ b/vl-bert_amd/csrc/gemm.hip
@@ -251,7 +251,7 @@
   }
 }
 
-template <int BM, int BN, int WGM, int WGN, int EPI, bool CONV = false>
+template <int BM, int BN, int WGM, int WGN, int EPI, bool CONV = false, bool ROWS = false>
 __global__ __launch_bounds__(64 * WGM * WGN, (WGM * WGN >= 8) ? 4 : 2) void gemm_nt_bf16_kernel(const GemmParams p) {
   constexpr int BK = 64;
   constexpr int NT = 64 * WGM * WGN;
@@ -265,14 +265,15 @@
   const int lane = tid & 63;
   const int wave = __builtin_amdgcn_readfirstlane(tid >> 6);
   const int wm = wave / WGN, wn = wave % WGN;
-  const int nt = p.ntm * p.ntn;
+  const int ntm = ROWS ? vlb_limited_tile_rows(p.row_limit, p.ntm, BM) : p.ntm;
+  const int nt = ntm * p.ntn;
   const int k_begin = blockIdx.y * p.k_per_split;
   const int k_end = min(p.K, k_begin + p.k_per_split);
   const int ntk = (k_end - k_begin) / BK;
   if ((int)blockIdx.x >= nt || ntk <= 0) return;
   auto tile_of = [&](int w, int& m0, int& n0) {
     int tile_m, tile_n;
-    vlb_tile_of(vlb_xcd_order(w, nt), p.ntm, p.ntn, p.tile_group, tile_m, tile_n);
+    vlb_tile_of(vlb_xcd_order(w, nt), ntm, p.ntn, p.tile_group, tile_m, tile_n);
     m0 = tile_m * BM;
     n0 = tile_n * BN;
   };
@@ -1043,11 +1044,11 @@
   transpose_tile(in, ldi, out, ldo, R, C, nullptr, vec, (t / tx) * 64, (t % tx) * 64);
 }
 
-template <int BM, int BN, int WGM, int WGN, int EPI>
+template <int BM, int BN, int WGM, int WGN, int EPI, bool ROWS = false>
 static int launch_gemm_cfg(GemmParams& p, int splits, hipStream_t stream) {
   int cap = vlb_opt(VLB_OPT_RESIDENT) / splits;
   if (cap < 8) cap = 8;
-  return launch_persistent<gemm_nt_bf16_kernel<BM, BN, WGM, WGN, EPI>>(2 * (BM + BN) * 64 * 2, 64 * WGM * WGN, BM, BN, cap & ~7,
+  return launch_persistent<gemm_nt_bf16_kernel<BM, BN, WGM, WGN, EPI, false, ROWS>>(2 * (BM + BN) * 64 * 2, 64 * WGM * WGN, BM, BN, cap & ~7,
                                                                        vlb_opt(VLB_OPT_TILE_GROUP), p, splits, stream, "vlb_gemm_nt_bf16");
 }
 
@@ -1064,6 +1065,10 @@
 
 template <int BM, int BN, int WGM, int WGN>
 static int launch_gemm_epi(GemmParams& p, int splits, hipStream_t stream) {
+  if (p.row_limit)
+    return dispatch_epi(epi_class(p) == 0 ? 0 : -1, std::integer_sequence<int, -1, 0>{}, VLB_ERR_ARG, [&](auto epi) {
+      return launch_gemm_cfg<BM, BN, WGM, WGN, decltype(epi)::value, true>(p, splits, stream);
+    });
   return dispatch_epi(epi_class(p), std::integer_sequence<int, -1, 0, 1, 2, 3, 4, 5, 6, 7, 8>{}, VLB_ERR_ARG, [&](auto epi) {
     return launch_gemm_cfg<BM, BN, WGM, WGN, decltype(epi)::value>(p, splits, stream);
   });
@@ -1097,7 +1102,8 @@
 static int gemm_nt_impl(const void* A, long lda, const void* B, long ldb, void* C, long ldc, int M, int N, int K,
                         const float* bias, int act, const void* aux, long ldaux, void* pre, long ldpre,
                         const void* res, long ldres, const float* res_stats, const float* res_gamma, const float* res_beta, int out_f16,
-                        float drop_p, const uint32_t* seed, uint32_t tag, int out_mode, int splitk, hipStream_t stream) {
+                        float drop_p, const uint32_t* seed, uint32_t tag, int out_mode, int splitk, hipStream_t stream,
+                        const int32_t* row_limit = nullptr) {
   if (M <= 0 || N <= 0) return VLB_OK;
   VLB_CHECK_ARG(!res_stats || (res && res_gamma && res_beta && act == 0 && out_mode == 0),
                 "vlb_gemm_nt_bf16_ex: the LayerNorm residual needs res (fp16 pre-LN rows), gamma, beta, act 0 and a 16-bit output");
@@ -1124,6 +1130,7 @@
   p.drop_thr = vlb_drop_thr(drop_p); p.drop_scale = vlb_drop_scale(p.drop_thr); p.seed = seed; p.tag = tag;
   p.C = C; p.ldc = ldc; p.out_f32 = out_mode; p.c_split_stride = 0;
   p.stagger = vlb_opt(VLB_OPT_NT_STAGGER);
+  p.row_limit = row_limit;
   int splits = 1;
   const int ktiles = K / 64;
   if (out_mode == 2) {
@@ -1152,14 +1159,14 @@
   const int use256 = vlb_opt(VLB_OPT_NT_256);
   const long tiles256 = (long)vlb_cdiv(M, 256) * vlb_cdiv(N, 256);
   const bool big_b = (long)N * K * 2 >= (24L << 20) && tiles256 >= 512;
-  if (use256 && out_mode == 0 && splits == 1 && act == 0 && !res && !p.drop_thr &&
+  if (use256 && !row_limit && out_mode == 0 && splits == 1 && act == 0 && !res && !p.drop_thr &&
       (use256 == 1 ? big_b : tiles256 >= use256)) {
     return launch_persistent<gemm_nt_256_kernel>(3 * (256 + 256) * 64, 512, 256, 256, 256, vlb_opt(VLB_OPT_NT_256_GROUP), p, 1, stream,
                                                  "vlb_gemm_nt_bf16(256)");
   }
   const long tiles128 = (long)vlb_cdiv(M, 128) * vlb_cdiv(N, 128) * splits;
   const bool narrow = tiles128 < 384 || N <= 64;
-  {
+  if (!row_limit) {
     const int took = gemm_ring_try(p, splits, stream);
     if (took <= 0) return took;
   }
@@ -1173,6 +1180,15 @@
                                 int out_mode, int splitk, hipStream_t stream) {
   return gemm_nt_impl(A, lda, B, ldb, C, ldc, M, N, K, bias, act, aux, ldaux, pre, ldpre, res, ldres, nullptr, nullptr, nullptr, 0,
                       drop_p, seed, tag, out_mode, splitk, stream);
+}
+
+extern "C" int vlb_gemm_nt_bf16_rows(const void* A, long lda, const void* B, long ldb, void* C, long ldc, int M, int N, int K,
+                                     const float* bias, int act, const void* aux, long ldaux, void* pre, long ldpre,
+                                     const void* res, long ldres, float drop_p, const uint32_t* seed, uint32_t tag,
+                                     int out_mode, int splitk, const int32_t* row_limit, hipStream_t stream) {
+  if (!vlb_opt(VLB_OPT_MLM_ROW_LIMIT)) row_limit = nullptr;
+  return gemm_nt_impl(A, lda, B, ldb, C, ldc, M, N, K, bias, act, aux, ldaux, pre, ldpre, res, ldres, nullptr, nullptr, nullptr, 0,
+                      drop_p, seed, tag, out_mode, splitk, stream, row_limit);
 }
 
 extern "C" int vlb_gemm_nt_bf16_ex(const void* A, long lda, const void* B, long ldb, void* C, long ldc, int M, int N, int K,
@@ -1217,16 +1233,21 @@
 __global__ __launch_bounds__(256) void splitk_reduce_kernel(const float* __restrict__ slabs, long slab_stride, int splits,
                                                             float* __restrict__ C, long ldc, int M, int N, int ldw,
                                                             bf16_t* __restrict__ Cb, long ldcb, int accumulate,
-                                                            const float* __restrict__ rowscale = nullptr) {
+                                                            const float* __restrict__ rowscale = nullptr,
+                                                            const int32_t* __restrict__ row_limit = nullptr) {
   const int n4 = ldw >> 2;
   const long total = (long)M * n4;
+  const int m_have = vlb_limited_tile_rows(row_limit, (M + 127) / 128, 128) * 128;
   for (long i = (long)blockIdx.x * 256 + threadIdx.x; i < total; i += (long)gridDim.x * 256) {
     const int m = (int)(i / n4), n = (int)(i % n4) * 4;
     const float* src = slabs + (long)m * ldw + n;
-    float4 a = *(const float4*)src;
-    for (int sp = 1; sp < splits; ++sp) {
-      const float4 b = *(const float4*)(src + sp * slab_stride);
-      a.x += b.x; a.y += b.y; a.z += b.z; a.w += b.w;
+    float4 a = make_float4(0.f, 0.f, 0.f, 0.f);
+    if (m < m_have) {
+      a = *(const float4*)src;
+      for (int sp = 1; sp < splits; ++sp) {
+        const float4 b = *(const float4*)(src + sp * slab_stride);
+        a.x += b.x; a.y += b.y; a.z += b.z; a.w += b.w;
+      }
     }
     if (rowscale) {
       const float sc = rowscale[m];
@@ -1257,11 +1278,12 @@
 }
 
 static int launch_splitk_reduce(const float* workspace, long slab_stride, int splits, float* C, long ldc, int Mo, int No, long ldw,
-                                int accumulate, const float* rowscale, hipStream_t stream, const char* name, bf16_t* Cb = nullptr) {
+                                int accumulate, const float* rowscale, hipStream_t stream, const char* name, bf16_t* Cb = nullptr,
+                                const int32_t* row_limit = nullptr) {
   long blocks = ((long)Mo * (ldw / 4) + 255) / 256;
   if (blocks > 2048) blocks = 2048;
   hipLaunchKernelGGL(splitk_reduce_kernel, dim3((int)blocks), dim3(256), 0, stream, workspace, slab_stride, splits, C, ldc, Mo, No, (int)ldw,
-                     Cb, ldc, accumulate, rowscale);
+                     Cb, ldc, accumulate, rowscale, row_limit);
   VLB_CHECK_LAUNCH(name);
   return VLB_OK;
 }
@@ -1319,8 +1341,8 @@
   return VLB_OK;
 }
 
-extern "C" int vlb_gemm_nt_bf16_splitk(const void* A, long lda, const void* B, long ldb, void* C, long ldc, int M, int N, int K,
-                                       float* workspace, long workspace_floats, hipStream_t stream) {
+static int gemm_nt_splitk_impl(const void* A, long lda, const void* B, long ldb, void* C, long ldc, int M, int N, int K, float* workspace,
+                              long workspace_floats, const int32_t* row_limit, hipStream_t stream) {
   if (M <= 0 || N <= 0) return VLB_OK;
   VLB_CHECK_ARG(K > 0 && (K % 64) == 0, "vlb_gemm_nt_bf16_splitk: K=%d must be a positive multiple of 64", K);
   VLB_CHECK_ARG(A && B && C, "vlb_gemm_nt_bf16_splitk: null operand");
@@ -1338,10 +1360,22 @@
   p.bias = nullptr; p.act = 0; p.aux = nullptr; p.ldaux = 0; p.pre = nullptr; p.ldpre = 0; p.res = nullptr; p.ldres = 0;
   p.drop_thr = 0; p.drop_scale = 1.f; p.seed = nullptr; p.tag = 0;
   p.C = workspace; p.ldc = ldw; p.out_f32 = 1; p.c_split_stride = (long)M * ldw;
+  p.row_limit = row_limit;
   int rc = launch_gemm<128, 128>(p, nsp, stream);
   if (rc) return rc;
   return launch_splitk_reduce(workspace, (long)M * ldw, nsp, nullptr, ldc, M, N, ldw, 0, nullptr, stream, "vlb_gemm_nt_bf16_splitk(reduce)",
-                              (bf16_t*)C);
+                              (bf16_t*)C, row_limit);
+}
+
+extern "C" int vlb_gemm_nt_bf16_splitk(const void* A, long lda, const void* B, long ldb, void* C, long ldc, int M, int N, int K,
+                                       float* workspace, long workspace_floats, hipStream_t stream) {
+  return gemm_nt_splitk_impl(A, lda, B, ldb, C, ldc, M, N, K, workspace, workspace_floats, nullptr, stream);
+}
+
+extern "C" int vlb_gemm_nt_bf16_splitk_rows(const void* A, long lda, const void* B, long ldb, void* C, long ldc, int M, int N, int K,
+                                            float* workspace, long workspace_floats, const int32_t* row_limit, hipStream_t stream) {
+  if (!vlb_opt(VLB_OPT_MLM_ROW_LIMIT)) row_limit = nullptr;
+  return gemm_nt_splitk_impl(A, lda, B, ldb, C, ldc, M, N, K, workspace, workspace_floats, row_limit, stream);
 }
 
 struct SplitkReduceGroup {
@@ -1422,7 +1456,8 @@
 }
 
 static int wgrad_tn_impl(const void* A, long lda, const void* B, long ldb, float* C, long ldc, int R, int Mo, int No, float* colsum,
-                         const float* rowscale, float* workspace, long workspace_floats, int accumulate, hipStream_t stream) {
+                         const float* rowscale, float* workspace, long workspace_floats, int accumulate, hipStream_t stream,
+                         const int32_t* row_limit = nullptr) {
   if (Mo <= 0 || No <= 0 || R <= 0) return VLB_OK;
   VLB_CHECK_ARG(A && B && C, "vlb_wgrad_tn_bf16: null operand");
   VLB_CHECK_ARG((lda % 8) == 0 && (ldb % 8) == 0 && (ldc % 4) == 0 && lda >= 8 && ldb >= 8, "vlb_wgrad_tn_bf16: bad leading dimensions");
@@ -1431,6 +1466,7 @@
     GemmParams q = {};
     q.A = (const bf16_t*)A; q.lda = lda; q.B = (const bf16_t*)B; q.ldb = ldb;
     q.M = Mo; q.N = No; q.K = R;
+    q.row_limit = row_limit;
     const int used = vlb_gemm_tn8_try(q, C, ldc, colsum, workspace, workspace_floats, accumulate, rowscale != nullptr, stream);
     if (used < 0) return used;
     if (used > 0) {
@@ -1451,6 +1487,13 @@
 extern "C" int vlb_wgrad_tn_bf16(const void* A, long lda, const void* B, long ldb, float* C, long ldc, int R, int Mo, int No,
                                  float* colsum, float* workspace, long workspace_floats, int accumulate, hipStream_t stream) {
   return wgrad_tn_impl(A, lda, B, ldb, C, ldc, R, Mo, No, colsum, nullptr, workspace, workspace_floats, accumulate, stream);
+}
+
+extern "C" int vlb_wgrad_tn_bf16_rows(const void* A, long lda, const void* B, long ldb, float* C, long ldc, int R, int Mo, int No,
+                                      float* colsum, float* workspace, long workspace_floats, int accumulate, const int32_t* row_limit,
+                                      hipStream_t stream) {
+  if (!vlb_opt(VLB_OPT_MLM_ROW_LIMIT)) row_limit = nullptr;
+  return wgrad_tn_impl(A, lda, B, ldb, C, ldc, R, Mo, No, colsum, nullptr, workspace, workspace_floats, accumulate, stream, row_limit);
 }
 
 extern "C" int vlb_wgrad_tn_group_bf16(int n, const void* const* A, const long* lda, const void* const* B, const long* ldb,
diff --git a/vl-bert_amd/csrc/gemm_p8.hip b/vl-bert_amd/csrc/gemm_p8.hip
--- a/vl-bert_amd/csrc/gemm_p8.hip
+++ b/vl-bert_amd/csrc/gemm_p8.hip
@@ -409,7 +409,7 @@
   asm volatile("" ::"v"(b8[0]), "v"(b8[4]));
 }
 
-template <int FMH, int EPI, bool KEEPB>
+template <int FMH, int EPI, bool KEEPB, bool ROWS = false>
 __global__ __launch_bounds__(512, 2) void gemm_nt_p8_kernel(const GemmParams p) {
   constexpr int AH = 32 * FMH;
   constexpr int BM = 2 * AH, BN = 256;
@@ -426,7 +426,8 @@
   const int tid = threadIdx.x, lane = tid & 63;
   const int wave = __builtin_amdgcn_readfirstlane(tid >> 6);
   const int wm = wave >> 2, wn = wave & 3;
-  const int nt = p.ntm * p.ntn;
+  const int ntm = ROWS ? vlb_limited_tile_rows(p.row_limit, p.ntm, BM) : p.ntm;
+  const int nt = ntm * p.ntn;
   const int nk = p.K >> 6;
   if ((int)blockIdx.x >= nt) return;
   unsigned long long* const stamps = (unsigned long long*)(EPI == 1 ? (void*)p.aux : (void*)p.pre);
@@ -440,7 +441,7 @@
 
   auto tile_of = [&](int w, int& m0, int& n0) {
     int tile_m, tile_n;
-    vlb_tile_of(vlb_xcd_order(w, nt), p.ntm, p.ntn, p.tile_group, tile_m, tile_n);
+    vlb_tile_of(vlb_xcd_order(w, nt), ntm, p.ntn, p.tile_group, tile_m, tile_n);
     m0 = tile_m * BM;
     n0 = tile_n * BN;
   };
@@ -666,6 +667,12 @@
 template <int FMH, bool KEEPB>
 int p8_launch_epi(GemmParams& p, int epi, hipStream_t stream) {
   const int wgs = vlb_opt(VLB_OPT_P8_WGS);
+  if (p.row_limit) {
+    if (epi != 0) return 0;
+    const int rc = launch_persistent<gemm_nt_p8_kernel<FMH, 0, KEEPB, true>>(163840, 512, 64 * FMH, 256, (wgs >= 8 && wgs <= 256) ? (wgs & ~7) : 256,
+                                                                           vlb_opt(VLB_OPT_P8_GROUP), p, 1, stream, "vlb_gemm_nt_bf16(p8 rows)", true);
+    return rc < 0 ? rc : 1;
+  }
   const int rc = dispatch_epi(epi, std::integer_sequence<int, 0, 1, 2, 3, 4, 5, 6, 7, 8, 10>{}, VLB_ERR_ARG, [&](auto e) {
     return launch_persistent<gemm_nt_p8_kernel<FMH, decltype(e)::value, KEEPB>>(163840, 512, 64 * FMH, 256, (wgs >= 8 && wgs <= 256) ? (wgs & ~7) : 256,
                                                                                 vlb_opt(VLB_OPT_P8_GROUP), p, 1, stream, "vlb_gemm_nt_bf16(p8)", true);
diff --git a/vl-bert_amd/csrc/gemm_params.h b/vl-bert_amd/csrc/gemm_params.h
--- a/vl-bert_amd/csrc/gemm_params.h
+++ b/vl-bert_amd/csrc/gemm_params.h
@@ -28,7 +28,14 @@
   int tile_group;
   int conv_C, conv_H, conv_W, conv_dil;
   const bf16_t* zero;
+  const int32_t* row_limit;
 };
+
+__device__ __forceinline__ int vlb_limited_tile_rows(const int32_t* row_limit, int ntm, int bm) {
+  if (!row_limit) return ntm;
+  const int lim = min(max(*row_limit, 0), ntm * bm);
+  return (lim + bm - 1) / bm;
+}
 
 #define GLDS_PTR(p) ((const __attribute__((address_space(1))) void*)(p))
 #define LDS_PTR(p) ((__attribute__((address_space(3))) void*)(p))
diff --git a/vl-bert_amd/csrc/gemm_tn8.hip b/vl-bert_amd/csrc/gemm_tn8.hip
--- a/vl-bert_amd/csrc/gemm_tn8.hip
+++ b/vl-bert_amd/csrc/gemm_tn8.hip
@@ -50,6 +50,7 @@
   Tn8Desc d[TN8_MAX_GROUP];
   int n, nitems;
   unsigned long long* stamps;
+  const int32_t* row_limit;
 };
 
 template <bool TABLE, int ABL = 0>
@@ -68,6 +69,9 @@
   const int wm = wave >> 2, wn = wave & 3;
   const int nitems = grp.nitems;
   if ((int)blockIdx.x >= nitems) return;
+  int r_max = 0x7FFFFFFF;
+  if constexpr (!TABLE)
+    if (grp.row_limit) r_max = (min(max(*grp.row_limit, 128), 0x7FFFFF00) + 127) & ~127;
   if (grp.stamps && tid == 0) {
     unsigned long long* t = grp.stamps + 4 * blockIdx.x;
     t[0] = __builtin_readcyclecounter();
@@ -97,7 +101,7 @@
     m0 = tile_m * 256;
     n0 = tile_n * 256;
     kt0 = sp * d.kt_per_split;
-    nk = min((d.R >> 6) - kt0, d.kt_per_split);
+    nk = min((min(d.R, r_max) >> 6) - kt0, d.kt_per_split);
   };
   const int step = (int)gridDim.x;
 
@@ -452,6 +456,7 @@
   const long ldw = (No + 3) / 4 * 4;
   int splits = vlb_tn8_pick_splits(Mo, No, R);
   if (tiles * splits < 128) return 0;
+  const int32_t* const row_limit = (splits == 1 && !force_slab) ? p.row_limit : nullptr;
   const int per = vlb_cdiv(pairs, splits);
   splits = vlb_cdiv(pairs, per);
   const bool slab = splits > 1 || force_slab;
@@ -465,6 +470,7 @@
   if (slab) { d.C = workspace; d.ldc = (int)ldw; d.c_split_stride = (long)Mo * ldw; d.accumulate = 0; }
   else { d.C = C; d.ldc = (int)ldc; d.c_split_stride = 0; d.accumulate = accumulate ? 1 : 0; }
   grp.n = 1; grp.nitems = d.nitems;
+  grp.row_limit = row_limit;
   const int rc = tn8_launch(grp, stream);
   return rc < 0 ? rc : splits;
 }
diff --git a/vl-bert_amd/csrc/loss.hip b/vl-bert_amd/csrc/loss.hip
--- a/vl-bert_amd/csrc/loss.hip
+++ b/vl-bert_amd/csrc/loss.hip
@@ -108,7 +108,7 @@
                                                            int n_split, int V, int cap, int32_t* __restrict__ sel_pos,
                                                            int32_t* __restrict__ sel_src, int64_t* __restrict__ labels_c,
                                                            float* __restrict__ count0, float* __restrict__ count1,
-                                                           int32_t* __restrict__ overflow) {
+                                                           int32_t* __restrict__ overflow, int32_t* __restrict__ kept_out) {
   __shared__ int wsum[16], wsum0[16];
   const int tid = threadIdx.x, lane = tid & 63, wave = tid >> 6;
   const unsigned long long below = (1ull << lane) - 1ull;
@@ -169,17 +169,31 @@
     *count0 = (float)n0;
     *count1 = (float)(kept - n0);
     if (total > cap) *overflow = 1;
-  }
-}
-
-extern "C" int vlb_mlm_compact(const int64_t* labels, const int32_t* src_rows, int n, int n_split, int V, int cap, int32_t* sel_pos,
-                               int32_t* sel_src, int64_t* labels_c, float* count0, float* count1, int32_t* overflow, hipStream_t stream) {
+    if (kept_out) *kept_out = kept;
+  }
+}
+
+static int mlm_compact(const int64_t* labels, const int32_t* src_rows, int n, int n_split, int V, int cap, int32_t* sel_pos,
+                       int32_t* sel_src, int64_t* labels_c, float* count0, float* count1, int32_t* overflow, int32_t* kept,
+                       hipStream_t stream) {
   VLB_CHECK_ARG(labels && src_rows && sel_pos && sel_src && labels_c && count0 && count1 && overflow, "vlb_mlm_compact: null argument");
   VLB_CHECK_ARG(n > 0 && cap > 0 && n_split >= 0 && n_split <= n, "vlb_mlm_compact: bad sizes");
   hipLaunchKernelGGL(mlm_compact_kernel, dim3(1), dim3(1024), 0, stream, labels, src_rows, n, n_split, V, cap, sel_pos, sel_src, labels_c,
-                     count0, count1, overflow);
+                     count0, count1, overflow, kept);
   VLB_CHECK_LAUNCH("vlb_mlm_compact");
   return VLB_OK;
+}
+
+extern "C" int vlb_mlm_compact(const int64_t* labels, const int32_t* src_rows, int n, int n_split, int V, int cap, int32_t* sel_pos,
+                               int32_t* sel_src, int64_t* labels_c, float* count0, float* count1, int32_t* overflow, hipStream_t stream) {
+  return mlm_compact(labels, src_rows, n, n_split, V, cap, sel_pos, sel_src, labels_c, count0, count1, overflow, nullptr, stream);
+}
+
+extern "C" int vlb_mlm_compact_rows(const int64_t* labels, const int32_t* src_rows, int n, int n_split, int V, int cap, int32_t* sel_pos,
+                                    int32_t* sel_src, int64_t* labels_c, float* count0, float* count1, int32_t* overflow, int32_t* kept,
+                                    hipStream_t stream) {
+  VLB_CHECK_ARG(kept, "vlb_mlm_compact_rows: null argument");
+  return mlm_compact(labels, src_rows, n, n_split, V, cap, sel_pos, sel_src, labels_c, count0, count1, overflow, kept, stream);
 }
 
 static int ce_fwd_bwd_compact(void* logits, long ld, int rows, int V, const int64_t* labels_c, const float* count0, const float* count1,
diff --git a/vl-bert_amd/csrc/options.h b/vl-bert_amd/csrc/options.h
--- a/vl-bert_amd/csrc/options.h
+++ b/vl-bert_amd/csrc/options.h
@@ -51,7 +51,9 @@
                         \
   X(LN_FWD_ROWS, "ln_fwd_rows", "VLB_LN_FWD_ROWS", 0)                                                                                   \
                     \
-  X(LN_BWD4, "ln_bwd4", "VLB_LN_BWD4", 1)
+  X(LN_BWD4, "ln_bwd4", "VLB_LN_BWD4", 1)                                                                                               \
+   \
+  X(MLM_ROW_LIMIT, "mlm_row_limit", "VLB_MLM_ROW_LIMIT", 1)
 
 enum VlbOpt {
 #define VLB_OPT_ID(id, name, env, dflt) VLB_OPT_##id,
diff --git a/vl-bert_amd/engine.py b/vl-bert_amd/engine.py
--- a/vl-bert_amd/engine.py
+++ b/vl-bert_amd/engine.py
@@ -306,6 +306,7 @@
             self.sel_src = torch.full((cap,), -1, dtype=torch.int32, device=d)
             self.labels_c = torch.full((cap,), -1, dtype=torch.int64, device=d)
             self.mlm_overflow = torch.zeros((1,), dtype=torch.int32, device=d)
+            self.mlm_kept = torch.zeros((1,), dtype=torch.int32, device=d)
             self.d_text_out_c = zb(cap, H)
         self.mvrc_logits_copy = zb(BR, self.Cp) if keep_logits else None
 
@@ -622,7 +623,7 @@
         nr = self.mlm_cap if compact else self.BT
         if compact:
             ops.mlm_compact(self.in_mlm_labels.view(-1), self.lay["text_rows"].view(-1), self.B * self.T, V, self.sel_pos, self.sel_src,
-                            self.labels_c, self.counts[0:1], self.counts[2:3], self.mlm_overflow)
+                            self.labels_c, self.counts[0:1], self.counts[2:3], self.mlm_overflow, kept=self.mlm_kept)
             ops.gather_rows(xl, self.sel_src, self.text_out[:nr])
         else:
             ops.gather_rows(xl, self.lay["text_rows"].view(-1), self.text_out)
@@ -640,7 +641,8 @@
                     act=ops.ACT_GELU_D, pre=self.mlm_u[:nr])
         ops.layernorm_fwd(self.mlm_g[:nr], w32[pm + "transform.LayerNorm.weight"], w32[pm + "transform.LayerNorm.bias"], self.mlm_h[:nr],
                           self.st_mlm[:nr])
-        ops.gemm_nt(self.mlm_h[:nr], w16["vlbert.word_embeddings.weight"], self.mlm_logits[:nr, :V], bias=w32[pm + "bias"])
+        ops.gemm_nt(self.mlm_h[:nr], w16["vlbert.word_embeddings.weight"], self.mlm_logits[:nr, :V], bias=w32[pm + "bias"],
+                    row_limit=self.mlm_kept if compact else None)
         ops.gemm_nt(self.obj_out, w16["vlbert.mvrc_head.transform.dense.weight"], self.mvrc_g,
                     bias=w32["vlbert.mvrc_head.transform.dense.bias"], act=ops.ACT_GELU_D, pre=self.mvrc_u)
         ops.gemm_nt(self.mvrc_g, w16["vlbert.mvrc_head.region_cls_pred.weight"], self.mvrc_logits[:, :C],
@@ -676,9 +678,10 @@
     def _on_side(self, launch, items):
         self._hazards.run(self.side, launch, [dy for dy, _, _, _ in items], writes=[g for _, _, gw, gb in items for g in (gw, gb)])
 
-    def _wgrad(self, dy, x, gw, gb):
+    def _wgrad(self, dy, x, gw, gb, row_limit=None):
         acc = not self._fresh_grads
-        self._on_side(lambda: ops.wgrad_tn(dy, x, gw, colsum=gb, workspace=self.wg_ws, accumulate=acc), [(dy, x, gw, gb)])
+        self._on_side(lambda: ops.wgrad_tn(dy, x, gw, colsum=gb, workspace=self.wg_ws, accumulate=acc, row_limit=row_limit),
+                      [(dy, x, gw, gb)])
 
     def _padded(self, items):
         pad = self._row_padded
@@ -756,8 +759,9 @@
             compact = self._mlm_compact_now and not self.core
             nr = self.mlm_cap if compact else self.BT
             dlog = self.mlm_logits[:nr]
-            self._wgrad(dlog[:, :V], self.mlm_h[:nr], g32["vlbert.word_embeddings.weight"], g32[pm + "bias"])
-            ops.gemm_nt_splitk(dlog, wT["vlbert.word_embeddings.weight"], self.d_mlm_h[:nr], workspace=self.wg_ws_main)
+            kept = self.mlm_kept if compact else None
+            self._wgrad(dlog[:, :V], self.mlm_h[:nr], g32["vlbert.word_embeddings.weight"], g32[pm + "bias"], row_limit=kept)
+            ops.gemm_nt_splitk(dlog, wT["vlbert.word_embeddings.weight"], self.d_mlm_h[:nr], workspace=self.wg_ws_main, row_limit=kept)
             self._ln_bwd(self.d_mlm_h[:nr], self.mlm_g[:nr], self.st_mlm[:nr], w32[pm + "transform.LayerNorm.weight"],
                          g32[pm + "transform.LayerNorm.weight"], g32[pm + "transform.LayerNorm.bias"], dx=self.d_mlm_g[:nr])
             ops.mul_bf16(self.d_mlm_g[:nr], self.mlm_u[:nr], self.d_mlm_u[:nr])
diff --git a/vl-bert_amd/ops.py b/vl-bert_amd/ops.py
--- a/vl-bert_amd/ops.py
+++ b/vl-bert_amd/ops.py
@@ -37,10 +37,17 @@
 
 
 def gemm_nt(A, B, C, bias=None, act=ACT_NONE, aux=None, pre=None, res=None, drop_p=0.0, seed=None, tag=0,
-            out_mode=OUT_BF16, splitk=0, K=None, res_ln=None):
+            out_mode=OUT_BF16, splitk=0, K=None, res_ln=None, row_limit=None):
     M, N = C.shape
     K = A.shape[1] if K is None else K
     assert A.shape[0] == M and B.shape[0] == N and B.shape[1] >= K and A.shape[1] >= K
+    cdt = BF16 if out_mode == OUT_BF16 else torch.float32
+    if row_limit is not None:
+        assert res_ln is None
+        _lib.call("vlb_gemm_nt_bf16_rows", _p(A, BF16), _ld(A), _p(B, BF16), _ld(B), _p(C, cdt), _ld(C), M, N, K,
+                  _p(bias, torch.float32), act, _p(aux, BF16), _ld(aux), _p(pre, BF16), _ld(pre), _p(res, BF16), _ld(res),
+                  float(drop_p), _p(seed), int(tag), out_mode, splitk, _p(row_limit, torch.int32), _stream())
+        return C
     if res_ln is not None or C.dtype == F16:
         assert out_mode == OUT_BF16
         st, g, b = res_ln if res_ln is not None else (None, None, None)
@@ -51,7 +58,6 @@
                   _p(st, torch.float32), _p(g, torch.float32), _p(b, torch.float32), 1 if C.dtype == F16 else 0,
                   float(drop_p), _p(seed), int(tag), out_mode, splitk, _stream())
         return C
-    cdt = BF16 if out_mode == OUT_BF16 else torch.float32
     _lib.call("vlb_gemm_nt_bf16", _p(A, BF16), _ld(A), _p(B, BF16), _ld(B), _p(C, cdt), _ld(C), M, N, K,
               _p(bias, torch.float32), act, _p(aux, BF16), _ld(aux), _p(pre, BF16), _ld(pre), _p(res, BF16), _ld(res),
               float(drop_p), _p(seed), int(tag), out_mode, splitk, _stream())
@@ -67,10 +73,15 @@
     return C
 
 
-def wgrad_tn(dy, x, C, colsum=None, workspace=None, accumulate=True):
+def wgrad_tn(dy, x, C, colsum=None, workspace=None, accumulate=True, row_limit=None):
     Mo, No = C.shape
     R = dy.shape[0]
     assert dy.shape[1] == Mo and x.shape[1] == No and x.shape[0] == R
+    if row_limit is not None:
+        _lib.call("vlb_wgrad_tn_bf16_rows", _p(dy, BF16), _ld(dy), _p(x, BF16), _ld(x), _p(C, torch.float32), _ld(C), R, Mo, No,
+                  _p(colsum, torch.float32), _p(workspace, torch.float32), workspace.numel() if workspace is not None else 0,
+                  int(bool(accumulate)), _p(row_limit, torch.int32), _stream())
+        return C
     _lib.call("vlb_wgrad_tn_bf16", _p(dy, BF16), _ld(dy), _p(x, BF16), _ld(x), _p(C, torch.float32), _ld(C), R, Mo, No,
               _p(colsum, torch.float32), _p(workspace, torch.float32), workspace.numel() if workspace is not None else 0,
               int(bool(accumulate)), _stream())
@@ -164,9 +175,13 @@
         _lib.call("vlb_wgrad_tn_table_launch", self.desc.data_ptr(), self.n, self.nitems, _stream())
 
 
-def gemm_nt_splitk(A, B, C, workspace=None):
+def gemm_nt_splitk(A, B, C, workspace=None, row_limit=None):
     M, K = A.shape
     N = B.shape[0]
+    if row_limit is not None:
+        _lib.call("vlb_gemm_nt_bf16_splitk_rows", _p(A, BF16), _ld(A), _p(B, BF16), _ld(B), _p(C, BF16), _ld(C), M, N, K,
+                  _p(workspace, torch.float32), workspace.numel() if workspace is not None else 0, _p(row_limit, torch.int32), _stream())
+        return C
     _lib.call("vlb_gemm_nt_bf16_splitk", _p(A, BF16), _ld(A), _p(B, BF16), _ld(B), _p(C, BF16), _ld(C), M, N, K,
               _p(workspace, torch.float32), workspace.numel() if workspace is not None else 0, _stream())
     return C
@@ -368,7 +383,12 @@
               float(gscale), _p(loss_out, torch.float32), _p(logits_copy, BF16), _ld(logits_copy), _stream())
 
 
-def mlm_compact(labels, src_rows, n_split, V, sel_pos, sel_src, labels_c, count0, count1, overflow):
+def mlm_compact(labels, src_rows, n_split, V, sel_pos, sel_src, labels_c, count0, count1, overflow, kept=None):
+    if kept is not None:
+        _lib.call("vlb_mlm_compact_rows", _p(labels, torch.int64), _p(src_rows, torch.int32), labels.numel(), int(n_split), int(V),
+                  sel_pos.numel(), _p(sel_pos, torch.int32), _p(sel_src, torch.int32), _p(labels_c, torch.int64),
+                  _p(count0, torch.float32), _p(count1, torch.float32), _p(overflow, torch.int32), _p(kept, torch.int32), _stream())
+        return
     _lib.call("vlb_mlm_compact", _p(labels, torch.int64), _p(src_rows, torch.int32), labels.numel(), int(n_split), int(V), sel_pos.numel(),
               _p(sel_pos, torch.int32), _p(sel_src, torch.int32), _p(labels_c, torch.int64), _p(count0, torch.float32),
               _p(count1, torch.float32), _p(overflow, torch.int32), _stream())
```

Measured after the change: 13990 samples/s (median of 6 runs). Within noise of the previous version (+0.3%).
